# ViacheslavTimofeev/tpu_superresolution

Hardware: AMD Instinct MI355X
Metric: HR pixels/sec, SwinIR x4 train step, 64x64 LR, bs=32/GPU (higher is better)
Workload: dtype bf16; 1 GPU; BASELINE cfg3: SwinIR classical x4 (dim 180, 6x6 blocks, window 8) train step = fwd + L1 + bwd + clip 1.0 + AdamW, 64x64 LR patches -> 256x256 HR, random-init weights, drop_path 0.1; every step starts from the seeded weights and fresh AdamW state; batch_per_gpu=32, global_batch=32, parallelism=dp1

## Files before the change

include/srk.h:

```cpp
#ifndef SRK_H_
#define SRK_H_

#include <stddef.h>
#include <stdint.h>

#ifdef __cplusplus
extern "C" {
#endif

#define SRK_OK 0
#define SRK_E_SHAPE (-1)
#define SRK_E_NULL (-2)
#define SRK_E_UNSUPPORTED (-3)
#define SRK_E_LAUNCH (-4)
#define SRK_E_ALIGN (-5)
#define SRK_E_STATE (-6)

typedef void* srk_stream_t;

const char* srk_version(void);
const char* srk_last_error(void);

int srk_window_partition(const void* x, void* out, int B, int H, int W, int C, int ws, int elem_bytes, srk_stream_t stream);
int srk_window_reverse(const void* windows, void* out, int B, int H, int W, int C, int ws, int elem_bytes, srk_stream_t stream);
int srk_roll2d(const void* x, void* out, int B, int H, int W, int C, int sh, int sw, int elem_bytes, srk_stream_t stream);
int srk_pixel_shuffle(const void* x, void* out, int B, int C, int H, int W, int r, int elem_bytes, srk_stream_t stream);
int srk_shift_mask(float* mask, int H, int W, int ws, int shift, srk_stream_t stream);
int srk_relative_position_index(int64_t* out, int ws, srk_stream_t stream);

typedef struct {
  int H, W;
  int shift;
} srk_win_geom;

int srk_layernorm_fwd(const float* x, const float* gamma, const float* beta, uint16_t* y_bf16, float* y_f32,
                      float* mean, float* rstd, int rows, int C, int CP, const srk_win_geom* geom, srk_stream_t stream);
int srk_window_attention_fwd(const uint16_t* qkv, const float* bias_dense, uint16_t* out, int64_t B_, int nH,
                             const srk_win_geom* geom, srk_stream_t stream);
int srk_window_attention_bwd(const uint16_t* qkv, const float* bias_dense, const uint16_t* d_out, uint16_t* d_qkv,
                             float* d_table, void* slab, int64_t B_, int nH, float scale, const srk_win_geom* geom,
                             srk_stream_t stream);
size_t srk_window_attention_bwd_scratch(int64_t B_, int nH);
int srk_window_attention_bwd_fused(const uint16_t* xn, int lda, const uint16_t* w_qkv, const float* b_qkv, float scale,
                                   const uint16_t* d_x1, int ldg, const uint16_t* w_proj_t, const float* bias_dense, uint16_t* d_qkv,
                                   float* d_table, void* slab, int64_t B_, int nH, const srk_win_geom* geom, srk_stream_t stream);
size_t srk_window_attention_bwd_fused_scratch(int64_t B_, int nH);
int srk_rel_pos_bias_expand(const float* table, float* bias_dense, int nH, srk_stream_t stream);
int srk_linear_bf16(const uint16_t* a, const uint16_t* w, const float* bias, uint16_t* y, int M, int N, int K, srk_stream_t stream);
int srk_linear_wgrad_bf16(const uint16_t* y, const uint16_t* x, float* dw, float* db, int M, int N, int K, srk_stream_t stream);
typedef struct {
  const void* y; int ldy;
  const void* x; int ldx;
  float* dw; float* db;
  int N, K;
} srk_wgrad_problem;
int srk_linear_wgrad_multi_bf16(const srk_wgrad_problem* problems, int count, int M, srk_stream_t stream);
int srk_conv3x3_bf16(const uint16_t* x, const uint16_t* w, const float* bias, uint16_t* y, int B, int H, int W, int CinP, int N,
                     srk_stream_t stream);
int srk_conv3x3_wgrad_bf16(const uint16_t* y, const uint16_t* x, float* dw, float* db, int B, int H, int W, int CinP, int N,
                           srk_stream_t stream);
int srk_cast_f32_bf16(const float* x, uint16_t* y, int64_t n, srk_stream_t stream);
int srk_probe_trread(const uint16_t* in, uint16_t* out, srk_stream_t stream);

int srk_probe_begin(int family, int capacity);
int srk_probe_end(double* total_ms, double* flops, double* bytes, int* launches);

int srk_set_option(const char* name, int value);
int srk_get_option(const char* name, int* value);

int srk_l1_loss_fwd_bwd(const float* pred, const float* target, float* d_pred, float* loss, uint32_t* nonfinite,
                        int64_t n, float grad_scale, srk_stream_t stream);
#define SRK_LOSS_L1 0
#define SRK_LOSS_MSE 1
#define SRK_LOSS_CHARBONNIER 2
int64_t srk_pixel_loss_workspace(int64_t n);
int srk_pixel_loss_fwd_bwd(const float* pred, const float* target, float* d_pred, float* loss, uint32_t* nonfinite, int64_t n, int kind,
                           float eps, float grad_scale, int accumulate, void* workspace, srk_stream_t stream);
int64_t srk_ssim_loss_workspace(int B, int C, int H, int W);
int srk_ssim_loss_fwd_bwd(const float* x, const float* y, void* workspace, int B, int C, int H, int W, float data_range, float alpha,
                          float* d_x, int accumulate, float* ssim_mean, float* loss, srk_stream_t stream);
int64_t srk_wgrad_workspace_bytes(void);
int srk_set_wgrad_workspace(void* workspace, int64_t bytes);

int srk_paired_crop_u8(const uint8_t* pool, const int64_t* lr_desc, const int64_t* hr_desc, float* lr_out, float* hr_out, int B,
                       int lr_patch, int scale, srk_stream_t stream);
int srk_dihedral_f32(const float* in, float* out, const int32_t* ops, int op_all, int B, int C, int H, int W, float alpha,
                     int accumulate, srk_stream_t stream);
int64_t srk_batch_psnr_workspace(int64_t per_image, int B);
int srk_batch_psnr(const float* pred, const float* target, void* workspace, int B, int64_t per_image, float max_val, float* psnr,
                   float* psnr_sum, float* abs_sum, srk_stream_t stream);
int64_t srk_eval_psnr_workspace(int64_t per_image, int B);
int srk_eval_psnr(const float* x, const float* y, void* workspace, int B, int64_t per_image, float max_val, float* psnr, float* mean,
                  srk_stream_t stream);
int64_t srk_ssim_workspace(int B, int C, int H, int W);
int srk_ssim(const float* x, const float* y, void* workspace, int B, int C, int H, int W, float data_range, float* per_image, float* mean,
             srk_stream_t stream);
int srk_grad_sumsq(const float* grads, int64_t n, float* sumsq, srk_stream_t stream);
int srk_adamw_clip_step(float* params, const float* grads, float* exp_avg, float* exp_avg_sq, int64_t n,
                        const float* sumsq, float max_norm, float grad_div, float lr, float beta1, float beta2, float eps,
                        float weight_decay, int step, const int32_t* nonfinite, srk_stream_t stream);
int srk_adamw_clip_ema_step(float* params, const float* grads, float* exp_avg, float* exp_avg_sq, float* ema, int64_t n,
                            const float* sumsq, float max_norm, float grad_div, float lr, float beta1, float beta2, float eps,
                            float weight_decay, int step, float ema_decay, const int32_t* nonfinite, srk_stream_t stream);
int srk_multi_grad_sumsq(const float* const* grads, const int64_t* numel, int n_tensors, float* sumsq, srk_stream_t stream);
int srk_multi_adamw_clip_step(float* const* params, const float* const* grads, float* const* exp_avg, float* const* exp_avg_sq,
                              const int64_t* numel, int n_tensors, const float* sumsq, float max_norm, float grad_div, float lr,
                              float beta1, float beta2, float eps, float weight_decay, int step, const float* hyper,
                              const int32_t* nonfinite, srk_stream_t stream);
int srk_multi_adamw_clip_ema_step(float* const* params, const float* const* grads, float* const* exp_avg, float* const* exp_avg_sq,
                                  float* const* ema, const int64_t* numel, int n_tensors, const float* sumsq, float max_norm,
                                  float grad_div, float lr, float beta1, float beta2, float eps, float weight_decay, int step,
                                  float ema_decay, const float* hyper, const int32_t* nonfinite, srk_stream_t stream);
int srk_adamw_hyper(float lr, float beta1, float beta2, int step, float* out3);

enum { SRK_LD_ROWS = 0, SRK_LD_CONV3 = 1,
       SRK_LD_CONV3_PS = 2  };
enum { SRK_EP_BF16 = 0,
       SRK_EP_GELU = 3,
       SRK_EP_RES = 4,
       SRK_EP_LRELU = 6,
       SRK_EP_PS = 7,
       SRK_EP_IMG = 8,
       SRK_EP_PS_IMG = 9,
       SRK_EP_RES_BF16 = 10,
       SRK_EP_DGELU = 5,
       SRK_EP_DLRELU = 11,
       SRK_EP_F32_BF16 = 12,
       SRK_EP_LNBWD = 13,
       SRK_EP_MLP_FUSED = 100  };
typedef struct {
  int loader, epilogue;
  const void* A; int lda;
  const void* W;
// ... 219 lines not shown
```

tpu_superresolution_amd/_lib.py:

```python
from __future__ import annotations

import ctypes as C
import os
import re
from typing import List

HERE = os.path.dirname(os.path.abspath(__file__))
LIB_PATH = os.environ.get("SRK_LIB_PATH") or os.path.join(HERE, "libsrk.so")
HEADER_PATH = os.path.join(os.path.dirname(HERE), "include", "srk.h")

_lib = None


class SrkError(RuntimeError):
    def __init__(self, code: int, message: str):
        super().__init__(f"libsrk error {code}: {message}")
        self.code = code
        self.message = message


class SrkUnsupported(NotImplementedError):
    pass


class WinGeom(C.Structure):
    _fields_ = [("H", C.c_int), ("W", C.c_int), ("shift", C.c_int)]


class SwinIRConfig(C.Structure):
    _fields_ = [("img_size", C.c_int), ("in_chans", C.c_int), ("embed_dim", C.c_int), ("num_layers", C.c_int),
                ("depths", C.c_int * 16), ("num_heads", C.c_int * 16), ("window_size", C.c_int),
                ("hidden_dim", C.c_int), ("upscale", C.c_int), ("upsampler", C.c_int), ("img_range", C.c_float),
                ("mean", C.c_float * 3), ("qk_scale", C.c_float), ("resi_connection", C.c_int), ("ape", C.c_int), ("use_checkpoint", C.c_int)]


class GemmArgs(C.Structure):
    _fields_ = [("loader", C.c_int), ("epilogue", C.c_int), ("A", C.c_void_p), ("lda", C.c_int), ("W", C.c_void_p),
                ("M", C.c_int), ("N", C.c_int), ("K", C.c_int), ("B", C.c_int), ("H", C.c_int), ("Wd", C.c_int), ("CinP", C.c_int),
                ("r", C.c_int), ("Cs", C.c_int), ("bias", C.c_void_p), ("outf", C.c_void_p), ("outb", C.c_void_p),
                ("outb2", C.c_void_p), ("res", C.c_void_p), ("aux", C.c_void_p), ("ldo", C.c_int), ("scale", C.c_float),
                ("inv_range", C.c_float), ("mean", C.c_float * 4), ("Cimg", C.c_int), ("Hc", C.c_int), ("Wc", C.c_int),
                ("xn_out", C.c_void_p), ("xn_mean", C.c_void_p), ("xn_rstd", C.c_void_p), ("xn_gamma", C.c_void_p),
                ("xn_beta", C.c_void_p), ("xn_C", C.c_int), ("rowscale", C.c_void_p), ("rows_per_sample", C.c_int),
                ("ln_x", C.c_void_p), ("ln_mean", C.c_void_p), ("ln_rstd", C.c_void_p), ("ln_gamma", C.c_void_p), ("ln_dgamma", C.c_void_p),
                ("ln_dbeta", C.c_void_p), ("ln_C", C.c_int)]


class WgradProblem(C.Structure):
    _fields_ = [("y", C.c_void_p), ("ldy", C.c_int), ("x", C.c_void_p), ("ldx", C.c_int), ("dw", C.c_void_p), ("db", C.c_void_p),
                ("N", C.c_int), ("K", C.c_int)]


LD_ROWS, LD_CONV3, LD_CONV3_PS = 0, 1, 2
EP_BF16, EP_GELU, EP_RES, EP_LRELU, EP_PS, EP_IMG, EP_PS_IMG, EP_RES_BF16 = 0, 3, 4, 6, 7, 8, 9, 10
EP_DGELU, EP_DLRELU, EP_F32_BF16, EP_LNBWD = 5, 11, 12, 13

LOSS_L1, LOSS_MSE, LOSS_CHARBONNIER = 0, 1, 2
LOSS_KINDS = {"l1": LOSS_L1, "mse": LOSS_MSE, "charbonnier": LOSS_CHARBONNIER}

UPSAMPLER_PIXELSHUFFLE = 1
UPSAMPLER_PIXELSHUFFLEDIRECT = 2
UPSAMPLER_NEAREST_CONV = 3
UPSAMPLER_NONE = 4
UPSAMPLERS = {"pixelshuffle": UPSAMPLER_PIXELSHUFFLE, "pixelshuffledirect": UPSAMPLER_PIXELSHUFFLEDIRECT,
              "nearest+conv": UPSAMPLER_NEAREST_CONV, "": UPSAMPLER_NONE}
RESI = {"1conv": 0, "3conv": 1}

_vp, _i, _i64, _f, _sz = C.c_void_p, C.c_int, C.c_int64, C.c_float, C.c_size_t
_geom_p = C.POINTER(WinGeom)

_SIGNATURES = {
    "srk_version": (C.c_char_p, []),
    "srk_last_error": (C.c_char_p, []),
    "srk_window_partition": (_i, [_vp, _vp, _i, _i, _i, _i, _i, _i, _vp]),
    "srk_window_reverse": (_i, [_vp, _vp, _i, _i, _i, _i, _i, _i, _vp]),
    "srk_roll2d": (_i, [_vp, _vp, _i, _i, _i, _i, _i, _i, _i, _vp]),
    "srk_pixel_shuffle": (_i, [_vp, _vp, _i, _i, _i, _i, _i, _i, _vp]),
    "srk_shift_mask": (_i, [_vp, _i, _i, _i, _i, _vp]),
    "srk_relative_position_index": (_i, [_vp, _i, _vp]),
    "srk_layernorm_fwd": (_i, [_vp, _vp, _vp, _vp, _vp, _vp, _vp, _i, _i, _i, _geom_p, _vp]),
    "srk_window_attention_fwd": (_i, [_vp, _vp, _vp, _i64, _i, _geom_p, _vp]),
    "srk_window_attention_bwd": (_i, [_vp, _vp, _vp, _vp, _vp, _vp, _i64, _i, _f, _geom_p, _vp]),
    "srk_window_attention_bwd_scratch": (_sz, [_i64, _i]),
    "srk_window_attention_bwd_fused": (_i, [_vp, _i, _vp, _vp, _f, _vp, _i, _vp, _vp, _vp, _vp, _vp, _i64, _i, _geom_p, _vp]),
    "srk_window_attention_bwd_fused_scratch": (_sz, [_i64, _i]),
    "srk_rel_pos_bias_expand": (_i, [_vp, _vp, _i, _vp]),
    "srk_linear_bf16": (_i, [_vp, _vp, _vp, _vp, _i, _i, _i, _vp]),
    "srk_linear_wgrad_bf16": (_i, [_vp, _vp, _vp, _vp, _i, _i, _i, _vp]),
    "srk_conv3x3_bf16": (_i, [_vp, _vp, _vp, _vp, _i, _i, _i, _i, _i, _vp]),
    "srk_conv3x3_wgrad_bf16": (_i, [_vp, _vp, _vp, _vp, _i, _i, _i, _i, _i, _vp]),
    "srk_cast_f32_bf16": (_i, [_vp, _vp, _i64, _vp]),
    "srk_probe_trread": (_i, [_vp, _vp, _vp]),
    "srk_set_option": (_i, [C.c_char_p, _i]),
    "srk_probe_begin": (_i, [_i, _i]),
    "srk_probe_end": (_i, [C.POINTER(C.c_double), C.POINTER(C.c_double), C.POINTER(C.c_double), C.POINTER(_i)]),
    "srk_l1_loss_fwd_bwd": (_i, [_vp, _vp, _vp, _vp, _vp, _i64, _f, _vp]),
    "srk_pixel_loss_workspace": (_i64, [_i64]),
    "srk_pixel_loss_fwd_bwd": (_i, [_vp, _vp, _vp, _vp, _vp, _i64, _i, _f, _f, _i, _vp, _vp]),
    "srk_ssim_loss_workspace": (_i64, [_i, _i, _i, _i]),
    "srk_ssim_loss_fwd_bwd": (_i, [_vp, _vp, _vp, _i, _i, _i, _i, _f, _f, _vp, _i, _vp, _vp, _vp]),
    "srk_wgrad_workspace_bytes": (_i64, []),
    "srk_set_wgrad_workspace": (_i, [_vp, _i64]),
    "srk_paired_crop_u8": (_i, [_vp, _vp, _vp, _vp, _vp, _i, _i, _i, _vp]),
    "srk_dihedral_f32": (_i, [_vp, _vp, _vp, _i, _i, _i, _i, _i, _f, _i, _vp]),
    "srk_batch_psnr_workspace": (_i64, [_i64, _i]),
    "srk_batch_psnr": (_i, [_vp, _vp, _vp, _i, _i64, _f, _vp, _vp, _vp, _vp]),
    "srk_eval_psnr_workspace": (_i64, [_i64, _i]),
    "srk_eval_psnr": (_i, [_vp, _vp, _vp, _i, _i64, _f, _vp, _vp, _vp]),
    "srk_ssim_workspace": (_i64, [_i, _i, _i, _i]),
    "srk_ssim": (_i, [_vp, _vp, _vp, _i, _i, _i, _i, _f, _vp, _vp, _vp]),
    "srk_grad_sumsq": (_i, [_vp, _i64, _vp, _vp]),
    "srk_adamw_clip_step": (_i, [_vp, _vp, _vp, _vp, _i64, _vp, _f, _f, _f, _f, _f, _f, _f, _i, _vp, _vp]),
    "srk_adamw_clip_ema_step": (_i, [_vp, _vp, _vp, _vp, _vp, _i64, _vp, _f, _f, _f, _f, _f, _f, _f, _i, _f, _vp, _vp]),
    "srk_multi_grad_sumsq": (_i, [_vp, _vp, _i, _vp, _vp]),
    "srk_multi_adamw_clip_step": (_i, [_vp, _vp, _vp, _vp, _vp, _i, _vp, _f, _f, _f, _f, _f, _f, _f, _i, _vp, _vp, _vp]),
    "srk_multi_adamw_clip_ema_step": (_i, [_vp, _vp, _vp, _vp, _vp, _vp, _i, _vp, _f, _f, _f, _f, _f, _f, _f, _i, _f, _vp, _vp, _vp]),
    "srk_adamw_hyper": (_i, [_f, _f, _f, _i, C.POINTER(C.c_float * 3)]),
    "srk_gemm_ex": (_i, [C.POINTER(GemmArgs), _vp]),
    "srk_mlp_fused_fwd": (_i, [_vp, _vp, _vp, _vp, _vp, _vp, _vp, _vp, _vp, _vp, _vp, _vp, _vp, _i, _i, _vp]),
    "srk_img_prep": (_i, [_vp, _vp, _i, _i, _i, _i, _i, _i, _f, C.POINTER(C.c_float * 3), _vp]),
    "srk_cab_bwd_workspace": (_sz, [_i, _i, _i]),
    "srk_cab_bwd": (_i, [_vp, _vp, _vp, _vp, _vp, _vp, _vp, _vp, _f, _vp, _vp, _vp, _vp, _vp, _vp, _i, _i, _i, _i, _i, _vp]),
    "srk_win256_attention_bwd_scratch": (_sz, [_i, _i, _i, _i, _i, _i, _i]),
    "srk_win256_attention_bwd": (_i, [_vp, _i, _i, _vp, _i, _vp, _i, _vp, _vp, _vp, _i, _i, _i, _i, _i, _i, _f, _i, _vp]),
    "srk_layernorm_bwd": (_i, [_vp, _vp, _vp, _vp, _vp, _vp, _vp, _vp, _vp, _i, _i, _i, _i, _vp]),
    "srk_add_f32_bf16": (_i, [_vp, _vp, _vp, _i64, _vp]),
    "srk_add_bf16_into_f32": (_i, [_vp, _vp, _i64, _vp]),
    "srk_add_f32": (_i, [_vp, _vp, _vp, _i64, _vp]),
    "srk_img_grad_prep": (_i, [_vp, _vp, _i, _i, _i, _i, _i, _i, _i, _i, _f, _vp]),
    "srk_smallconv_wgrad": (_i, [_vp, _vp, _vp, _vp, _i, _i, _i, _i, _i, _i, _i, _vp]),
    "srk_smallconv_dgrad": (_i, [_vp, _vp, _vp, _i, _i, _i, _i, _i, _i, _i, _vp]),
    "srk_stem_wgrad": (_i, [_vp, _vp, _vp, _vp, _i, _i, _i, _i, _i, _i, _vp]),
    "srk_conv3x3_wgrad_ps_bf16": (_i, [_vp, _vp, _vp, _vp, _i, _i, _i, _i, _i, _i, _i, _vp]),
    "srk_mlp_fused_fwd_train": (_i, [_vp] * 15 + [_i, _vp, _i, _i, _vp]),
    "srk_rowscale_bf16": (_i, [_vp, _vp, _vp, _i64, _i, _i, _vp]),
    "srk_stem_conv": (_i, [_vp, _vp, _vp, _vp, _i, _i, _i, _i, _i, _i, _vp]),
    "srk_swin_block_fwd": (_i, [_vp] * 16 + [_f] + [_i] * 8 + [_vp]),
    "srk_win256_attention_fwd": (_i, [_vp, _i, _i, _vp, _i, _vp, _i, _i, _i, _i, _i, _i, _i, _i, _i, _f, _i, _vp]),
    "srk_win_small_attention_fwd": (_i, [_vp, _i, _i, _vp, _vp, _i, _i, _i, _i, _i, _i, _i, _f, _vp]),
    "srk_win_small_attention_bwd_scratch": (_sz, [_i, _i, _i, _i, _i]),
    "srk_win_small_attention_bwd": (_i, [_vp, _i, _i, _vp, _vp, _i, _vp, _vp, _vp, _i, _i, _i, _i, _i, _i, _f, _vp]),
    "srk_win_attention_fwd_padded": (_i, [_vp, _i, _i, _vp, _i, _vp, _i, _i, _i, _i, _i, _i, _i, _i, _i, _i, _i, _f, _i, _vp]),
    "srk_channel_gate_workspace": (_sz, [_i, _i, _i]),
    "srk_channel_gate": (_i, [_vp, _vp, _vp, _vp, _vp, _vp, _f, _vp, _i, _i, _i, _i, _i, _vp]),
    "srk_channel_gate_act": (_i, [_vp, _vp, _vp, _vp, _vp, _vp, _f, _vp, _i, _i, _i, _i, _i, _i, _vp]),
    "srk_dwconv3x3": (_i, [_vp, _i, _vp, _vp, _vp, _vp, _i, _vp, _i, _i, _i, _i, _i, _i, _vp]),
    "srk_dwconv3x3_bn_act": (_i, [_vp, _i, _vp, _vp, _vp, _vp, _vp, _i, _vp, _i, _i, _i, _i, _i, _vp]),
    "srk_dwconv3x3_bn_act_launches": (C.c_longlong, []),
    "srk_bn_frozen_coeffs": (_i, [_i, _i, _vp, _vp, _f, _vp, _vp, _vp, _vp, _vp]),
    "srk_bn_frozen_bwd_coeffs": (_i, [_vp, _i, _i, _i, _i, _vp, _vp, _vp]),
    "srk_channel_interaction_frozen_covered": (_i, [_i, _i, _i]),
    "srk_channel_interaction_frozen_fwd": (_i, [_vp, _i, _f, _vp, _vp, _vp, _vp, _vp, _f, _vp, _vp, _vp, _vp, _vp, _vp, _i, _i, _i, _i, _vp]),
    "srk_channel_interaction_frozen_bwd": (_i, [_vp, _vp, _i, _f, _vp, _vp, _vp, _vp, _vp, _f, _vp, _vp, _vp, _vp] + [_vp] * 7 + [_i, _i, _i, _i, _vp]),
    "srk_rowln_bf16": (_i, [_vp, _i, _vp, _vp, _vp, _i, _i64, _i, _i, _vp]),
    "srk_spatial_gate": (_i, [_vp, _i, _vp, _vp, _vp, _f, _i, _vp, _i64, _i, _vp]),
    "srk_spatial_gate_dev": (_i, [_vp, _i, _vp, _vp, _vp, _vp, _i, _vp, _i64, _i, _vp]),
    "srk_dual_gate_combine": (_i, [_vp, _vp, _vp, _vp, _vp, _i64, _i, _i, _i, _vp]),
    "srk_channel_attention_workspace": (_sz, [_i, _i, _i]),
    "srk_channel_attention_fwd": (_i, [_vp, _i, _i, _vp, _vp, _vp, _i, _i, _i, _i, _i, _vp]),
    "srk_linear_wgrad_multi_bf16": (_i, [C.POINTER(WgradProblem), _i, _i, _vp]),
    "srk_mlp_fused_bwd": (_i, [_vp, _vp, _vp, _vp, _vp, _vp, _vp, _vp, _vp, _vp, _vp, _vp, _i, _vp, _vp, _i, _i, _vp]),
    "srk_win_attention_bwd_padded_scratch": (_sz, [_i, _i, _i, _i, _i, _i]),
    "srk_win_attention_bwd_padded": (_i, [_vp, _i, _i, _vp, _vp, _i, _vp, _vp, _vp, _i, _i, _i, _i, _i, _i, _i, _i, _i, _i, _f, _vp]),
    "srk_bn_train_coeffs": (_i, [_vp, _i, _i, _i, _i, _f, _vp, _vp, _f, _vp, _vp, _vp, _f, _vp, _vp]),
    "srk_channel_interaction_covered": (_i, [_i, _i, _i]),
    "srk_channel_interaction_fwd": (_i, [_vp, _i, _f, _vp, _vp, _vp, _vp, _vp, _f, _vp, _vp, _vp, _vp, _f, _vp, _vp, _i, _i, _i, _i, _vp]),
    "srk_channel_interaction_bwd": (_i, [_vp, _vp, _i, _f, _vp, _vp, _vp, _vp, _vp, _f, _vp, _vp, _vp, _vp, _vp, _vp, _vp, _vp, _vp, _i, _i, _i, _i, _vp]),
    "srk_chan_attn_matrix_fwd": (_i, [_vp, _i, _vp, _vp, _vp, _i, _i, _i, _vp]),
# ... 85 lines not shown
```

tpu_superresolution_amd/csrc/api.hip:

```cpp
#include <stdarg.h>
#include <stdio.h>
#include <string.h>

#include "adamw.h"
#include "kernels.h"
#include "wgrad.h"

static thread_local char g_err[512] = "";

SrkOptTls& srk_opt_tls() {
  static thread_local SrkOptTls t = {};
  return t;
}

static SrkOpt** opt_table() {
  static SrkOpt* table[SRK_NUM_OPTS] = {};
  return table;
}

void srk_opt_register(SrkOpt* o) {
  if (o->id >= 0 && o->id < SRK_NUM_OPTS) opt_table()[o->id] = o;
}

void srk_opt_scope_begin(SrkOptTls* saved) {
// ... 118 lines not shown
  SRK_REQUIRE(B > 0 && C > 0 && H > 0 && W > 0 && r > 0, SRK_E_SHAPE, "pixel_shuffle: bad shape");
  return srk_launch_pixel_shuffle(x, out, B, C, H, W, r, elem_bytes, (hipStream_t)stream);
}

int srk_shift_mask(float* mask, int H, int W, int ws, int shift, srk_stream_t stream) {
  REQ_PTR(mask);
  SRK_REQUIRE(ws > 0 && H % ws == 0 && W % ws == 0 && shift >= 0 && shift < ws, SRK_E_SHAPE,
              "shift_mask: shift_size must in 0-window_size (H=%d W=%d ws=%d shift=%d)", H, W, ws, shift);
  return srk_launch_shift_mask(mask, H, W, ws, shift, (hipStream_t)stream);
}

int srk_relative_position_index(int64_t* out, int ws, srk_stream_t stream) {
  REQ_PTR(out);
  SRK_REQUIRE(ws > 0 && ws <= 64, SRK_E_SHAPE, "relative_position_index: bad ws %d", ws);
  return srk_launch_rel_pos_index((long long*)out, ws, (hipStream_t)stream);
}

int srk_layernorm_fwd(const float* x, const float* gamma, const float* beta, uint16_t* y_bf16, float* y_f32, float* mean,
                      float* rstd, int rows, int C, int CP, const srk_win_geom* geom, srk_stream_t stream) {
  REQ_PTR(x); REQ_PTR(gamma); REQ_PTR(beta); REQ_ALIGN(x);
  SRK_REQUIRE(rows > 0, SRK_E_SHAPE, "layernorm: rows=%d", rows);
  SRK_REQUIRE((mean == nullptr) == (rstd == nullptr), SRK_E_NULL, "layernorm: mean/rstd must both be given or both null");
  WinGeom g;
  if (geom) {
    int rc = make_geom(geom, &g, "layernorm");
    if (rc) return rc;
    SRK_REQUIRE(rows % (g.H * g.W) == 0, SRK_E_SHAPE, "layernorm: rows %d not a multiple of H*W", rows);
  }
  return srk_launch_ln_fwd(x, gamma, beta, y_bf16, y_f32, mean, rstd, rows, C, CP, geom ? &g : nullptr, (hipStream_t)stream);
}

int srk_window_attention_fwd(const uint16_t* qkv, const float* bias_dense, uint16_t* out, int64_t B_, int nH,
                             const srk_win_geom* geom, srk_stream_t stream) {
  REQ_PTR(qkv); REQ_PTR(bias_dense); REQ_PTR(out); REQ_PTR(geom); REQ_ALIGN(qkv); REQ_ALIGN(out); REQ_ALIGN(bias_dense);
  WinGeom g;
  int rc = make_geom(geom, &g, "window_attention_fwd");
  if (rc) return rc;
  SRK_REQUIRE(B_ > 0 && B_ % g.nW == 0 && nH > 0 && nH <= 64, SRK_E_SHAPE, "window_attention_fwd: B_=%lld nW=%d nH=%d",
              (long long)B_, g.nW, nH);
  return srk_launch_attn_fwd(qkv, bias_dense, out, B_, nH, g, (hipStream_t)stream);
}

size_t srk_window_attention_bwd_scratch(int64_t B_, int nH) {
  return (size_t)srk_attn_bwd_slabs(B_, nH, nullptr) * nH * 4096 * sizeof(float);
}

int srk_window_attention_bwd(const uint16_t* qkv, const float* bias_dense, const uint16_t* d_out, uint16_t* d_qkv,
                             float* d_table, void* slab, int64_t B_, int nH, float scale, const srk_win_geom* geom,
                             srk_stream_t stream) {
  REQ_PTR(qkv); REQ_PTR(bias_dense); REQ_PTR(d_out); REQ_PTR(d_qkv); REQ_PTR(d_table); REQ_PTR(slab); REQ_PTR(geom);
  REQ_ALIGN(qkv); REQ_ALIGN(d_out); REQ_ALIGN(d_qkv); REQ_ALIGN(slab);
  WinGeom g;
  int rc = make_geom(geom, &g, "window_attention_bwd");
  if (rc) return rc;
  SRK_REQUIRE(B_ > 0 && B_ % g.nW == 0 && nH > 0 && nH <= 64, SRK_E_SHAPE, "window_attention_bwd: B_=%lld nW=%d nH=%d",
              (long long)B_, g.nW, nH);
  return srk_launch_attn_bwd(qkv, bias_dense, d_out, d_qkv, (float*)slab, d_table, B_, nH, g, scale, (hipStream_t)stream);
}

size_t srk_window_attention_bwd_fused_scratch(int64_t B_, int nH) {
  return (size_t)srk_qkv_attn_bwd_slabs(B_, nH, nH * 32, 192) * nH * 4096 * sizeof(float);
}

int srk_window_attention_bwd_fused(const uint16_t* xn, int lda, const uint16_t* w_qkv, const float* b_qkv, float scale,
                                   const uint16_t* d_x1, int ldg, const uint16_t* w_proj_t, const float* bias_dense, uint16_t* d_qkv,
                                   float* d_table, void* slab, int64_t B_, int nH, const srk_win_geom* geom, srk_stream_t stream) {
  REQ_PTR(xn); REQ_PTR(w_qkv); REQ_PTR(d_x1); REQ_PTR(w_proj_t); REQ_PTR(bias_dense); REQ_PTR(d_qkv); REQ_PTR(d_table); REQ_PTR(slab);
  REQ_PTR(geom); REQ_ALIGN(xn); REQ_ALIGN(w_qkv); REQ_ALIGN(d_x1); REQ_ALIGN(w_proj_t); REQ_ALIGN(d_qkv); REQ_ALIGN(slab);
  WinGeom g;
  int rc = make_geom(geom, &g, "window_attention_bwd_fused");
  if (rc) return rc;
  SRK_REQUIRE(B_ > 0 && B_ % g.nW == 0, SRK_E_SHAPE, "window_attention_bwd_fused: B_=%lld nW=%d", (long long)B_, g.nW);
  const int nslab = srk_qkv_attn_bwd_slabs(B_, nH, nH * 32, 192);
  SRK_REQUIRE(nslab > 0, SRK_E_UNSUPPORTED,
              "window_attention_bwd_fused: covers 6 heads x 32, K = 192 and at least one window per CU (got nH=%d B_=%lld)", nH,
              (long long)B_);
  rc = srk_launch_qkv_attn_bwd(xn, lda, w_qkv, b_qkv, scale, d_x1, ldg, w_proj_t, bias_dense, d_qkv, (float*)slab, B_, nH, nH * 32, 192, g,
                               (hipStream_t)stream);
  SRK_REQUIRE(rc != SRK_NOT_COVERED, SRK_E_UNSUPPORTED, "window_attention_bwd_fused: the kernel cannot run on this build / shape");
  if (rc) return rc;
  return srk_launch_rpb_reduce((const float*)slab, d_table, nslab, nH, (hipStream_t)stream);
}

int srk_rel_pos_bias_expand(const float* table, float* bias_dense, int nH, srk_stream_t stream) {
  REQ_PTR(table); REQ_PTR(bias_dense);
  return srk_launch_rpb_expand(table, bias_dense, nH, (hipStream_t)stream);
}

int srk_linear_bf16(const uint16_t* a, const uint16_t* w, const float* bias, uint16_t* y, int M, int N, int K, srk_stream_t stream) {
  REQ_PTR(a); REQ_PTR(w); REQ_PTR(y); REQ_ALIGN(a); REQ_ALIGN(w); REQ_ALIGN(y);
  GemmParams p = {};
  p.A = a; p.lda = K; p.Wt = w; p.M = M; p.N = N; p.K = K; p.bias = bias; p.outb = y; p.ldo = N;
  return srk_launch_gemm(LD_ROWS, EP_BF16, p, (hipStream_t)stream);
}

int srk_linear_wgrad_bf16(const uint16_t* y, const uint16_t* x, float* dw, float* db, int M, int N, int K, srk_stream_t stream) {
  REQ_PTR(y); REQ_PTR(x); REQ_PTR(dw); REQ_ALIGN(y); REQ_ALIGN(x);
  WgradParams p = {};
  p.Y = y; p.ldy = N; p.X = x; p.ldx = K; p.M = M; p.N = N; p.K = K; p.dW = dw; p.ldw = K; p.db = db;
  return srk_launch_wgrad(p, (hipStream_t)stream);
}

int srk_linear_wgrad_multi_bf16(const srk_wgrad_problem* problems, int count, int M, srk_stream_t stream) {
  REQ_PTR(problems);
  SRK_REQUIRE(count >= 1 && count <= 4 && M > 0, SRK_E_SHAPE, "linear_wgrad_multi: count=%d (1..4), M=%d", count, M);
  WgradParams ps[4] = {};
  for (int i = 0; i < count; ++i) {
    const srk_wgrad_problem& q = problems[i];
    REQ_PTR(q.y); REQ_PTR(q.x); REQ_PTR(q.dw); REQ_ALIGN(q.y); REQ_ALIGN(q.x);
    SRK_REQUIRE(q.N > 0 && q.K > 0 && q.N % 64 == 0 && q.K % 64 == 0, SRK_E_SHAPE, "linear_wgrad_multi: problem %d: N=%d K=%d (multiples of 64)", i,
                q.N, q.K);
    SRK_REQUIRE((q.ldy <= 0 || q.ldy >= q.N) && (q.ldx <= 0 || q.ldx >= q.K), SRK_E_SHAPE, "linear_wgrad_multi: problem %d: ldy=%d < N or ldx=%d < K",
                i, q.ldy, q.ldx);
    SRK_REQUIRE((q.ldy <= 0 || q.ldy % 8 == 0) && (q.ldx <= 0 || q.ldx % 8 == 0), SRK_E_ALIGN,
                "linear_wgrad_multi: problem %d: ldy=%d / ldx=%d must be multiples of 8 elements", i, q.ldy, q.ldx);
    ps[i].Y = static_cast<const bf16_t*>(q.y); ps[i].ldy = q.ldy > 0 ? q.ldy : q.N;
    ps[i].X = static_cast<const bf16_t*>(q.x); ps[i].ldx = q.ldx > 0 ? q.ldx : q.K;
    ps[i].M = M; ps[i].N = q.N; ps[i].K = q.K; ps[i].dW = q.dw; ps[i].ldw = q.K; ps[i].db = q.db;
  }
  return srk_launch_wgrad_multi(ps, count, (hipStream_t)stream);
}

int srk_conv3x3_bf16(const uint16_t* x, const uint16_t* w, const float* bias, uint16_t* y, int B, int H, int W, int CinP, int N,
                     srk_stream_t stream) {
  REQ_PTR(x); REQ_PTR(w); REQ_PTR(y); REQ_ALIGN(x); REQ_ALIGN(w); REQ_ALIGN(y);
  GemmParams p = {};
  p.A = x; p.Wt = w; p.M = B * H * W; p.N = N; p.K = 9 * CinP; p.B = B; p.H = H; p.W = W; p.CinP = CinP;
  p.bias = bias; p.outb = y; p.ldo = N;
  return srk_launch_gemm(LD_CONV3, EP_BF16, p, (hipStream_t)stream);
}

int srk_conv3x3_wgrad_bf16(const uint16_t* y, const uint16_t* x, float* dw, float* db, int B, int H, int W, int CinP, int N,
                           srk_stream_t stream) {
  REQ_PTR(y); REQ_PTR(x); REQ_PTR(dw); REQ_ALIGN(y); REQ_ALIGN(x);
  SRK_REQUIRE(B > 0 && H > 0 && W > 0 && (long long)B * H * W < (1ll << 31), SRK_E_SHAPE, "conv3x3_wgrad: B=%d H=%d W=%d", B, H, W);
  WgradParams p = {};
  p.Y = y; p.ldy = N; p.X = x; p.ldx = CinP; p.M = B * H * W; p.N = N; p.K = CinP; p.dW = dw; p.ldw = 9 * CinP; p.db = db;
  p.conv = 1; p.B = B; p.H = H; p.W = W; p.r = 1;
  return srk_launch_wgrad(p, (hipStream_t)stream);
}

int srk_cast_f32_bf16(const float* x, uint16_t* y, int64_t n, srk_stream_t stream) {
  REQ_PTR(x); REQ_PTR(y);
  return srk_launch_cast_f32_bf16(x, y, n, (hipStream_t)stream);
}

int srk_probe_begin(int family, int capacity) {
  SRK_REQUIRE(!g_probe.active, SRK_E_STATE, "probe_begin: a probe is already active");
  SRK_REQUIRE(family >= 1 && family <= 7 && capacity > 0 && capacity <= (1 << 20), SRK_E_SHAPE, "probe_begin: bad arguments");
  while ((int)g_probe.ev0.size() < capacity) {
    hipEvent_t a, b;
    if (hipEventCreate(&a) != hipSuccess || hipEventCreate(&b) != hipSuccess) {
      srk_set_error("probe_begin: hipEventCreate failed");
      return SRK_E_LAUNCH;
    }
    g_probe.ev0.push_back(a);
    g_probe.ev1.push_back(b);
  }
  g_probe.family = family;
  g_probe.count = 0;
  g_probe.seen = 0;
  g_probe.flops = 0.0;
  g_probe.bytes = 0.0;
  g_probe.active = true;
  return SRK_OK;
}

int srk_probe_end(double* total_ms, double* flops, double* bytes, int* launches) {
  SRK_REQUIRE(g_probe.active, SRK_E_STATE, "probe_end: no active probe");
  g_probe.active = false;
  double ms = 0.0;
  for (size_t i = 0; i < g_probe.count; ++i) {
    float t = 0.f;
    if (hipEventSynchronize(g_probe.ev1[i]) != hipSuccess || hipEventElapsedTime(&t, g_probe.ev0[i], g_probe.ev1[i]) != hipSuccess) {
      srk_set_error("probe_end: event query failed");
      return SRK_E_LAUNCH;
    }
    ms += t;
  }
  if (total_ms) *total_ms = ms;
  if (flops) *flops = g_probe.flops;
  if (bytes) *bytes = g_probe.bytes;
  if (launches) *launches = (int)g_probe.count;
  return SRK_OK;
}

namespace {

int tune_get(int which) {
  int v[4];
  srk_gemm_stream_tune_get(&v[0], &v[1], &v[2], &v[3]);
  return v[which];
}
int tune_set(int which, int value) {
  int v[4];
  srk_gemm_stream_tune_get(&v[0], &v[1], &v[2], &v[3]);
  v[which] = value;
  srk_gemm_stream_tune(v[0], v[1], v[2], v[3]);
  return SRK_OK;
}
int wtune_get(int which) {
  int rows, nt;
  srk_wgrad_stream_tune_get(&rows, &nt);
  return which == 0 ? rows : nt;
}

struct OptEntry {
  const char* name;
  int (*get)();
  int (*set)(int);
};

const OptEntry kOptions[] = {
    {"gemm_stream", [] { return srk_gemm_stream_enabled(); }, [](int v) { srk_gemm_stream_enable(v); return (int)SRK_OK; }},
    {"attn_bwd_fused", [] { return srk_attn_bwd_fused_enabled(); }, [](int v) { srk_attn_bwd_fused_enable(v); return (int)SRK_OK; }},
    {"attn_fused", [] { return srk_attn_fused_mode(); }, [](int v) { srk_attn_fused_enable(v); return (int)SRK_OK; }},
    {"wgrad_stream_w8", [] { return srk_wgrad_w8_enabled(); }, [](int v) { srk_wgrad_w8_enable(v); return (int)SRK_OK; }},
    {"block_light", [] { return srk_block_light_enabled(); }, [](int v) { srk_block_light_enable(v); return (int)SRK_OK; }},
    {"mlp_bwd_fused", [] { return srk_mlp_bwd_fused_enabled(); }, [](int v) { srk_mlp_bwd_fused_enable(v); return (int)SRK_OK; }},
    {"mlp_dgelu_store", [] { return srk_mlp_dgelu_store_enabled(); }, [](int v) { srk_mlp_dgelu_store_enable(v); return (int)SRK_OK; }},
    {"mlp_fused", [] { return srk_mlp_fused_enabled(); }, [](int v) { srk_mlp_fused_enable(v); return (int)SRK_OK; }},
    {"wgrad_stream", [] { return srk_wgrad_stream_enabled(); }, [](int v) { srk_wgrad_stream_enable(v); return (int)SRK_OK; }},
    {"conv_wgrad_taps", [] { return srk_conv_wgrad_taps_mode(); }, [](int v) { srk_conv_wgrad_taps_enable(v); return (int)SRK_OK; }},
    {"conv_wgrad_roll", [] { return srk_conv_wgrad_roll_enabled(); }, [](int v) { srk_conv_wgrad_roll_enable(v); return (int)SRK_OK; }},
    {"wgrad_partials", [] { return srk_wgrad_partials_enabled(); }, [](int v) { srk_wgrad_partials_enable(v); return (int)SRK_OK; }},
    {"wgrad_stream_rows", [] { return wtune_get(0); },
     [](int v) {
       SRK_REQUIRE(v == 32 || v == 64, SRK_E_SHAPE, "wgrad_stream_rows: 32/64");
       srk_wgrad_stream_tune(v, -1);
       return (int)SRK_OK;
     }},
    {"wgrad_stream_nt", [] { return wtune_get(1); }, [](int v) { srk_wgrad_stream_tune(0, v != 0); return (int)SRK_OK; }},
    {"gemm_stream_bm", [] { return tune_get(0); },
     [](int v) {
       SRK_REQUIRE(v == 0 || v == 16 || v == 32 || v == 64, SRK_E_SHAPE, "gemm_stream_bm: 0/16/32/64");
       return tune_set(0, v);
     }},
    {"gemm_stream_ks2", [] { return tune_get(1); }, [](int v) { return tune_set(1, v < 0 ? -1 : (v != 0)); }},
    {"gemm_stream_split", [] { return tune_get(2); }, [](int v) { return tune_set(2, v < 0 ? -1 : (v != 0)); }},
    {"gemm_stream_nb", [] { return tune_get(3); },
     [](int v) {
       SRK_REQUIRE(v == 0 || v == 4 || v == 8, SRK_E_SHAPE, "gemm_stream_nb: 0/4/8");
       return tune_set(3, v);
     }},
    {"probe_stride", [] { return g_probe.stride; },
     [](int v) {
       SRK_REQUIRE(v >= 1 && v <= 1024, SRK_E_SHAPE, "probe_stride: 1..1024");
       g_probe.stride = v;
       return (int)SRK_OK;
     }},
};

const OptEntry* find_option(const char* name) {
  for (const OptEntry& e : kOptions)
    if (strcmp(name, e.name) == 0) return &e;
  return nullptr;
}

}

int srk_set_option(const char* name, int value) {
  REQ_PTR(name);
  const OptEntry* e = find_option(name);
  if (!e) {
    srk_set_error("srk_set_option: unknown option '%s'", name);
    return SRK_E_UNSUPPORTED;
  }
  return e->set(value);
}

int srk_get_option(const char* name, int* value) {
  REQ_PTR(name); REQ_PTR(value);
  const OptEntry* e = find_option(name);
  if (!e) {
    srk_set_error("srk_get_option: unknown option '%s'", name);
    return SRK_E_UNSUPPORTED;
  }
  *value = e->get();
  return SRK_OK;
}

int srk_probe_trread(const uint16_t* in, uint16_t* out, srk_stream_t stream) {
  REQ_PTR(in); REQ_PTR(out);
  return srk_launch_probe_trread(in, out, (hipStream_t)stream);
}

int srk_l1_loss_fwd_bwd(const float* pred, const float* target, float* d_pred, float* loss, uint32_t* nonfinite, int64_t n,
                        float grad_scale, srk_stream_t stream) {
  REQ_PTR(pred); REQ_PTR(target); REQ_PTR(loss); REQ_PTR(nonfinite);
  SRK_REQUIRE(n > 0, SRK_E_SHAPE, "l1_loss: n=%lld", (long long)n);
  return srk_launch_l1_loss(pred, target, d_pred, loss, nonfinite, n, grad_scale, (hipStream_t)stream);
}

int64_t srk_wgrad_workspace_bytes(void) { return (int64_t)WS_WORKSPACE_BYTES; }

int srk_set_wgrad_workspace(void* workspace, int64_t bytes) {
  SRK_REQUIRE(bytes >= 0 && (workspace != nullptr || bytes == 0), SRK_E_SHAPE, "set_wgrad_workspace: null pointer with %lld bytes",
              (long long)bytes);
// ... 131 lines not shown
```

tpu_superresolution_amd/csrc/attn_bwd_fused.hip:

```cpp
#include "kernels.h"

namespace {

constexpr int H_K = 192, H_CA = 192, H_NH = 6;
constexpr int H_SLOT = 64 * H_K * 2;
constexpr int H_TILE = 64 * 32;
constexpr int H_PT = 64 * 64;
constexpr int H_TAB = 225;
constexpr int H_PAIR = 2 * H_SLOT;
constexpr int OFF_S = 0;
constexpr int OFF_T = 2 * H_PAIR;
constexpr int OFF_TAB = OFF_T + 12 * H_TILE * 2;
constexpr int OFF_PB = OFF_TAB + 2704;
constexpr int H_LDS = OFF_PB + 10 * 32 * 4;
static_assert(6 * H_PT * 2 == H_PAIR, "P / dS tiles of a head triple fill a row slot exactly");

#ifndef SRK_ABF_ISSUE_AT
#define SRK_ABF_ISSUE_AT 1
#endif
#ifdef SRK_PROBE_ABF
__device__ unsigned long long g_abf_probe[12 * 16 * 8];
#define ABF_MARK(k) do { if (blockIdx.x == 0 && lane == 0 && t < 16) g_abf_probe[(wave * 16 + t) * 8 + (k)] = __builtin_amdgcn_s_memrealtime(); } while (0)
extern "C" int srk_debug_abf_probe(void* host) { return (int)hipMemcpyFromSymbol(host, HIP_SYMBOL(g_abf_probe), sizeof(g_abf_probe)); }
#else
#define ABF_MARK(k) do {} while (0)
#endif

struct BwdFusedParams {
  const bf16_t* xn;
  int lda;
  const bf16_t* g;
  int ldg;
  const bf16_t* Wqkv;
  const float* bqkv;
  float scale;
  const bf16_t* WprojT;
  const float* biasd;
  bf16_t* dqkv;
  float* slab;
  long long B_;
  WinGeom geom;
};

__device__ __forceinline__ int tf(int r) { return ((((r >> 2) ^ (r >> 3)) & 1) << 1) | (((r >> 3) ^ (r >> 1)) & 1); }
__device__ __forceinline__ int ps(int r) { return (((r >> 3) & 1) << 2) | (((r >> 1) & 1) << 1) | ((r >> 2) & 1); }

__device__ __forceinline__ bf16x8_t h_cat4(bf16x4_t lo, bf16x4_t hi) {
  return bf16x8_t{lo[0], lo[1], lo[2], lo[3], hi[0], hi[1], hi[2], hi[3]};
}

__device__ __forceinline__ bf16x8_t tile_tr(const bf16_t* tile, int rb0, int rb1, int dt, int r16) {
  const int q = r16 >> 2, c = 2 * dt + ((r16 & 3) >> 1), in = (r16 & 1) << 2;
  const int ra = rb0 + q, rb = rb1 + q;
  return h_cat4(lds_tr_read(tile + ra * 32 + ((c ^ tf(ra)) << 3) + in), lds_tr_read(tile + rb * 32 + ((c ^ tf(rb)) << 3) + in));
}
__device__ __forceinline__ bf16x8_t ptile_tr(const bf16_t* tile, int rb0, int rb1, int jt, int r16) {
  const int q = r16 >> 2, c = 2 * jt + ((r16 & 3) >> 1), in = (r16 & 1) << 2;
  const int ra = rb0 + q, rb = rb1 + q;
  return h_cat4(lds_tr_read(tile + ra * 64 + ((c ^ ps(ra)) << 3) + in), lds_tr_read(tile + rb * 64 + ((c ^ ps(rb)) << 3) + in));
}

__global__ __launch_bounds__(768) void qkv_attn_bwd_kernel(const BwdFusedParams p, int ngrp) {
  extern __shared__ __attribute__((aligned(16))) unsigned char smem[];
  const unsigned smem_base = (unsigned)(size_t)smem;
  const int tid = threadIdx.x, lane = tid & 63;
  const int wave = __builtin_amdgcn_readfirstlane(tid >> 6);
  const int r16 = lane & 15, g = lane >> 4;
  const int id = blockIdx.x, xcd = id & 7, slot = id >> 3;
  const int tr = slot & 1, grp = slot >> 1;
  const int gidx = grp * 8 + xcd;
  const long long first = gidx, stride = 8LL * ngrp;
  const long long nwin = first < p.B_ ? (p.B_ - first + stride - 1) / stride : 0;
  const int hl = wave >> 2, it = wave & 3;
  const int head = 3 * tr + hl;

  f32x4_t dbias[4];
#pragma unroll
  for (int jt = 0; jt < 4; ++jt) dbias[jt] = f32x4_t{0.f, 0.f, 0.f, 0.f};

  if (nwin > 0) {
    bf16_t* tiles = reinterpret_cast<bf16_t*>(smem + OFF_T);
    float* tab = reinterpret_cast<float*>(smem + OFF_TAB);
    for (int i = tid; i < 3 * H_TAB; i += 768) {
      const int hh = i / H_TAB, t = i - hh * H_TAB;
      const int dy = t / 15 - 7, dx = t - (t / 15) * 15 - 7;
      const int qi = (dy > 0 ? dy : 0) * 8 + (dx > 0 ? dx : 0), kj = (dy < 0 ? -dy : 0) * 8 + (dx < 0 ? -dx : 0);
      tab[i] = p.biasd[(3 * tr + hh) * 4096 + qi * 64 + kj];
    }

    bf16x8_t wf[2][6];
    {
      const bf16_t* wbase = it < 3 ? p.Wqkv + (long long)(it * H_CA + head * 32) * H_K : p.WprojT + (long long)(head * 32) * H_K;
#pragma unroll
      for (int j = 0; j < 2; ++j)
#pragma unroll
        for (int s = 0; s < 6; ++s) wf[j][s] = *reinterpret_cast<const bf16x8_t*>(wbase + (16 * j + r16) * H_K + s * 32 + g * 8);
    }
    float* pbs = reinterpret_cast<float*>(smem + OFF_PB);
    for (int i = tid; i < 9 * 32; i += 768) {
      const int tl = i >> 5, hh = tl / 3, which = tl - 3 * hh;
      pbs[i] = p.bqkv ? p.bqkv[which * H_CA + (3 * tr + hh) * 32 + (i & 31)] : 0.f;
    }
    for (int i = tid; i < 32; i += 768) pbs[9 * 32 + i] = 0.f;
    const float* pbw = pbs + (it < 3 ? hl * 3 + it : 9) * 32 + 4 * g;
    const float sc = it == 0 ? p.scale : 1.0f;

    const bool dma_g = wave >= 6;
    const bf16_t* dsrc = dma_g ? p.g : p.xn;
    const long long dld = dma_g ? p.ldg : p.lda;
    const int piece0 = dma_g ? 4 * (wave - 6) : 4 * wave;
    const unsigned ddst = smem_base + OFF_S + (dma_g ? H_SLOT : 0) + piece0 * 1024;
    auto issue = [&](long long b_, int slot) {
      const bf16_t* base = dsrc + b_ * 64 * dld;
#pragma unroll
      for (int i = 0; i < 4; ++i) {
        int q = (piece0 + i) * 64 + lane;
        asm volatile("" : "+v"(q));
        const int row = (q * 2731) >> 16, pos = q - row * 24;
        srk_glds16<false>(base + row * (int)dld + ((pos ^ (row & 7)) << 3), __builtin_amdgcn_readfirstlane(ddst + slot * H_PAIR + i * 1024));
      }
    };
#pragma unroll
    for (int j = 0; j < 2; ++j) {
#pragma unroll
      for (int s = 0; s < 6; ++s) asm volatile("" ::"v"(wf[j][s]));
    }
    issue(first, 0);

    const int tfr = tf(r16), psr = ps(r16);
    bf16_t* mytile = tiles + (hl * 4 + it) * H_TILE;
    const bf16_t* Qs = tiles + (hl * 4 + 0) * H_TILE;
    const bf16_t* Ks = tiles + (hl * 4 + 1) * H_TILE;
    const bf16_t* Vs = tiles + (hl * 4 + 2) * H_TILE;
    const bf16_t* Os = tiles + (hl * 4 + 3) * H_TILE;
    const float* th = tab + hl * H_TAB + ((2 * it + (r16 >> 3)) - (g >> 1) + 7) * 15 + ((r16 & 7) - 4 * (g & 1) + 7) - 93;
    const int ldq = 3 * H_CA;
    const int scol = ((g & 1) << 4) | ((g >> 1) << 3);
    auto store8 = [&](bf16_t* dst, uint2 x, uint2 y) {
      const auto s0 = __builtin_amdgcn_permlane16_swap(x.x, y.x, false, false);
      const auto s1 = __builtin_amdgcn_permlane16_swap(x.y, y.y, false, false);
      *reinterpret_cast<uint4*>(dst) = make_uint4(s0[0], s1[0], s0[1], s1[1]);
    };

    for (long long t = 0; t < nwin; ++t) {
      const long long b_ = first + t * stride;
      if (t == 0) srk_wait_vmcnt<0>();
// ... 92 lines not shown
#pragma unroll
          for (int e = 0; e < 4; ++e) s[jt][e] = __builtin_amdgcn_exp2f(tt[e]);
          a4 += s[jt];
        }
        const float inv = __builtin_amdgcn_rcpf(xrow_sum4((a4[0] + a4[1]) + (a4[2] + a4[3])));
        float dl = 0.f;
#pragma unroll
        for (int jt = 0; jt < 4; ++jt)
#pragma unroll
          for (int e = 0; e < 4; ++e) {
            s[jt][e] *= inv;
            dl += s[jt][e] * dp[jt][e];
          }
        dl = xrow_sum4(dl);
        uint2 dsp[4];
#pragma unroll
        for (int jt = 0; jt < 4; ++jt) {
#pragma unroll
          for (int e = 0; e < 4; ++e) {
            dp[jt][e] = s[jt][e] * (dp[jt][e] - dl);
            dbias[jt][e] += dp[jt][e];
          }
          dsp[jt] = pack_bf4(dp[jt][0], dp[jt][1], dp[jt][2], dp[jt][3]);
          const int po = (16 * it + r16) * 64 + (((2 * jt + (g >> 1)) ^ psr) << 3) + 4 * (g & 1);
          *reinterpret_cast<uint2*>(Pb + po) = pack_bf4(s[jt][0], s[jt][1], s[jt][2], s[jt][3]);
          *reinterpret_cast<uint2*>(Db + po) = dsp[jt];
        }
        f32x4_t aq[2] = {f32x4_t{0.f, 0.f, 0.f, 0.f}, f32x4_t{0.f, 0.f, 0.f, 0.f}};
#pragma unroll
        for (int ss = 0; ss < 2; ++ss) {
          const bf16x8_t dsf = __builtin_bit_cast(bf16x8_t, make_uint4(dsp[2 * ss].x, dsp[2 * ss].y, dsp[2 * ss + 1].x, dsp[2 * ss + 1].y));
#pragma unroll
          for (int dt = 0; dt < 2; ++dt)
            aq[dt] = __builtin_amdgcn_mfma_f32_16x16x32_bf16(tile_tr(Ks, 32 * ss + 4 * g, 32 * ss + 16 + 4 * g, dt, r16), dsf, aq[dt], 0, 0, 0);
        }
        bf16_t* row = p.dqkv + (b_ * 64 + 16 * it + r16) * ldq + head * 32 + scol;
        store8(row, pack_bf4(aq[0][0] * p.scale, aq[0][1] * p.scale, aq[0][2] * p.scale, aq[0][3] * p.scale),
               pack_bf4(aq[1][0] * p.scale, aq[1][1] * p.scale, aq[1][2] * p.scale, aq[1][3] * p.scale));
      }
      ABF_MARK(4);
      srk_lds_barrier();
      ABF_MARK(5);
      if (SRK_ABF_ISSUE_AT == 2 && t + 1 < nwin) issue(b_ + stride, cur ^ 1);

      {
        f32x4_t av[2], ak[2];
#pragma unroll
        for (int dt = 0; dt < 2; ++dt) av[dt] = ak[dt] = f32x4_t{0.f, 0.f, 0.f, 0.f};
        bf16x8_t pf[2], df[2], otf[2][2], qtf[2][2];
#pragma unroll
        for (int ss = 0; ss < 2; ++ss) {
          const int rb0 = 32 * ss + 8 * g, rb1 = rb0 + 4;
          pf[ss] = ptile_tr(Pb, rb0, rb1, it, r16);
          df[ss] = ptile_tr(Db, rb0, rb1, it, r16);
#pragma unroll
          for (int dt = 0; dt < 2; ++dt) {
            otf[ss][dt] = tile_tr(Os, rb0, rb1, dt, r16);
            qtf[ss][dt] = tile_tr(Qs, rb0, rb1, dt, r16);
          }
        }
        __builtin_amdgcn_sched_barrier(0);
#pragma unroll
        for (int ss = 0; ss < 2; ++ss)
#pragma unroll
          for (int dt = 0; dt < 2; ++dt) {
            av[dt] = __builtin_amdgcn_mfma_f32_16x16x32_bf16(otf[ss][dt], pf[ss], av[dt], 0, 0, 0);
            ak[dt] = __builtin_amdgcn_mfma_f32_16x16x32_bf16(qtf[ss][dt], df[ss], ak[dt], 0, 0, 0);
          }
        bf16_t* row = p.dqkv + (b_ * 64 + 16 * it + r16) * ldq + head * 32 + scol;
        store8(row + H_CA, pack_bf4(ak[0][0], ak[0][1], ak[0][2], ak[0][3]), pack_bf4(ak[1][0], ak[1][1], ak[1][2], ak[1][3]));
        store8(row + 2 * H_CA, pack_bf4(av[0][0], av[0][1], av[0][2], av[0][3]), pack_bf4(av[1][0], av[1][1], av[1][2], av[1][3]));
      }
      ABF_MARK(6);
    }
  }
  int lane2;
  asm volatile("v_mbcnt_lo_u32_b32 %0, -1, 0\n\tv_mbcnt_hi_u32_b32 %0, -1, %0" : "=v"(lane2));
  float* slab = p.slab + (((long long)gidx * H_NH + head) * 64 + 16 * it + (lane2 & 15)) * 64 + 4 * (lane2 >> 4);
#pragma unroll
  for (int jt = 0; jt < 4; ++jt)
    *reinterpret_cast<float4*>(slab + 16 * jt) = make_float4(dbias[jt][0], dbias[jt][1], dbias[jt][2], dbias[jt][3]);
}

SrkOpt g_attn_bwd_fused{OPT_ATTN_BWD_FUSED, 1};

}

void srk_attn_bwd_fused_enable(int on) { g_attn_bwd_fused = on ? 1 : 0; }
int srk_attn_bwd_fused_enabled() { return g_attn_bwd_fused; }

static int abf_cus() { return srk_device_cus(); }

int srk_qkv_attn_bwd_slabs(long long B_, int nH, int CA, int K) {
  if (!g_attn_bwd_fused || nH != H_NH || CA != H_CA || K != H_K) return 0;
  const int cus = abf_cus();
  if (cus < 16 || B_ < cus) return 0;
  return 8 * (cus / 16);
}

int srk_launch_qkv_attn_bwd(const bf16_t* xn, int lda, const bf16_t* Wqkv, const float* bqkv, float scale, const bf16_t* g, int ldg,
                            const bf16_t* WprojT, const float* biasd, bf16_t* dqkv, float* slab, long long B_, int nH, int CA, int K,
                            WinGeom geom, hipStream_t stream) {
  const int nslab = srk_qkv_attn_bwd_slabs(B_, nH, CA, K);
  if (nslab == 0 || lda % 8 != 0 || ldg % 8 != 0 || B_ * 64 * (long long)(lda > ldg ? lda : ldg) >= (1LL << 31)) return SRK_NOT_COVERED;
  static SrkPerDevice<int> configured_pd; int& configured = configured_pd.here();
  if (!configured) {
    const void* fn = reinterpret_cast<const void*>(&qkv_attn_bwd_kernel);
    hipFuncAttributes attr;
    configured = -1;
#ifdef SRK_PROBE_ABF
    attr.localSizeBytes = 0;
    if (hipFuncSetAttribute(fn, hipFuncAttributeMaxDynamicSharedMemorySize, H_LDS) == hipSuccess) configured = 1;
#endif
    if (configured < 0 && hipFuncGetAttributes(&attr, fn) == hipSuccess && attr.localSizeBytes == 0 &&
        hipFuncSetAttribute(fn, hipFuncAttributeMaxDynamicSharedMemorySize, H_LDS) == hipSuccess)
      configured = 1;
  }
  if (configured < 0) return SRK_NOT_COVERED;
  BwdFusedParams bp;
  bp.xn = xn; bp.lda = lda; bp.g = g; bp.ldg = ldg; bp.Wqkv = Wqkv; bp.bqkv = bqkv; bp.scale = scale; bp.WprojT = WprojT;
  bp.biasd = biasd; bp.dqkv = dqkv; bp.slab = slab; bp.B_ = B_; bp.geom = geom;
  const int ngrp = nslab / 8;
  srk_probe_pre(FAM_ATTN_BWD, stream, 0.0);
  hipLaunchKernelGGL(qkv_attn_bwd_kernel, dim3(16 * ngrp), dim3(768), H_LDS, stream, bp, ngrp);
  srk_probe_post(FAM_ATTN_BWD, stream);
  return srk_check_launch("qkv+attention backward");
}
```

tpu_superresolution_amd/csrc/common.h:

```cpp
#pragma once
#include <hip/hip_runtime.h>
#include <stdint.h>

#include "../../include/srk.h"

typedef unsigned short bf16_t;
typedef __attribute__((ext_vector_type(8))) short bf16x8_t;
typedef __attribute__((ext_vector_type(4))) short bf16x4_t;
typedef __attribute__((ext_vector_type(4))) float f32x4_t;

#define SRK_WAVE 64

void srk_set_error(const char* fmt, ...);
int srk_check_launch(const char* what);

constexpr int SRK_MAX_DEVICES = 64;
int srk_current_device();
int srk_device_cus();
enum SrkOptId {
  OPT_MLP_FUSED, OPT_MLP_BWD_FUSED, OPT_GEMM_STREAM, OPT_TUNE_BM, OPT_TUNE_KS2, OPT_TUNE_SPLIT, OPT_TUNE_NB, OPT_ATTN_BWD_FUSED,
  OPT_ATTN_FUSED, OPT_BLOCK_LIGHT, OPT_TAPS_ENABLED, OPT_TAPS_DMA, OPT_WGRAD_STREAM, OPT_WGRAD_ROWS, OPT_WGRAD_NT, OPT_WGRAD_W8,
  OPT_WGRAD_PARTIALS, OPT_MLP_DGELU_STORE, OPT_TAPS_ROLL, SRK_NUM_OPTS
};
struct SrkOptTls {
  int v[SRK_NUM_OPTS];
  unsigned on;
};
SrkOptTls& srk_opt_tls();
struct SrkOpt;
void srk_opt_register(SrkOpt* o);
void srk_opt_scope_begin(SrkOptTls* saved);
void srk_opt_scope_end(const SrkOptTls& saved);
struct SrkOpt {
  int id;
  int value;
  SrkOpt(int id_, int v) : id(id_), value(v) { srk_opt_register(this); }
  operator int() const {
    const SrkOptTls& t = srk_opt_tls();
    return ((t.on >> id) & 1u) ? t.v[id] : value;
  }
  SrkOpt& operator=(int v) {
    SrkOptTls& t = srk_opt_tls();
    if ((t.on >> id) & 1u) t.v[id] = v;
    else value = v;
    return *this;
  }
  SrkOpt(const SrkOpt&) = delete;
  SrkOpt& operator=(const SrkOpt&) = delete;
};

template <class T>
struct SrkPerDevice {
  T v[SRK_MAX_DEVICES] = {};
  T& here() { return v[srk_current_device()]; }
};

enum { FAM_GEMM_LINEAR = 1, FAM_GEMM_CONV = 2, FAM_WGRAD_LINEAR = 3, FAM_WGRAD_CONV = 4, FAM_ATTN_FWD = 5, FAM_ATTN_BWD = 6,
       FAM_LN = 7 };
void srk_probe_pre(int family, hipStream_t stream, double flops, double bytes = 0.0);
void srk_probe_post(int family, hipStream_t stream);

#define SRK_REQUIRE(cond, code, ...)      \
  do {                                    \
    if (!(cond)) {                        \
      srk_set_error(__VA_ARGS__);         \
      return (code);                      \
    }                                     \
  } while (0)

__device__ __forceinline__ float bf2f(bf16_t v) { return __uint_as_float(((unsigned)v) << 16); }

__device__ __forceinline__ bf16_t f2bf(float f) {
  __bf16 b = (__bf16)f;
  return __builtin_bit_cast(unsigned short, b);
}

typedef __bf16 srk_bf16x2_t __attribute__((ext_vector_type(2)));
typedef float srk_f32x2_t __attribute__((ext_vector_type(2)));
__device__ __forceinline__ unsigned pack_bf2(float lo, float hi) {
  return __builtin_bit_cast(unsigned, __builtin_convertvector(srk_f32x2_t{lo, hi}, srk_bf16x2_t));
}

__device__ __forceinline__ uint2 pack_bf4(float a, float b, float c, float d) {
  return make_uint2(pack_bf2(a, b), pack_bf2(c, d));
}

__device__ __forceinline__ void unpack_bf2(unsigned u, float& lo, float& hi) {
  lo = __uint_as_float(u << 16);
  hi = __uint_as_float(u & 0xffff0000u);
}

__device__ __forceinline__ float erf_fast(float x) {
  const float ax = fabsf(x);
  const float t = __builtin_amdgcn_rcpf(fmaf(0.3275911f, ax, 1.0f));
  float p = fmaf(1.061405429f, t, -1.453152027f);
  p = fmaf(p, t, 1.421413741f);
  p = fmaf(p, t, -0.284496736f);
  p = fmaf(p, t, 0.254829592f);
  const float r = 1.0f - p * t * __expf(-ax * ax);
  return copysignf(r, x);
}
__device__ __forceinline__ float gelu_f(float x) { return 0.5f * x * (1.0f + erf_fast(x * 0.70710678118654752f)); }

__device__ __forceinline__ float dgelu_shared_exp(float x) {
  const float z = x * 0.70710678118654752f;
// ... 164 lines not shown
```

tpu_superresolution_amd/csrc/kernels.h:

```cpp
#pragma once
#include "common.h"
#include "gemm.h"
#include "pack.h"
#include "wgrad.h"

int srk_launch_qkv_attn_fwd(const bf16_t* xn, int lda, const bf16_t* Wt, const float* bias, float scale, bf16_t* qkv, const float* biasd,
                            bf16_t* ao, long long B_, int nH, int CA, int K, WinGeom geom, hipStream_t stream);
void srk_attn_fused_enable(int on);
int srk_attn_fused_mode();
void srk_block_light_enable(int on);
int srk_block_light_enabled();
int srk_launch_swin_block_light(const float* x, float* y, bf16_t* yb, const float* n1w, const float* n1b, const float* n2w, const float* n2b,
                                const bf16_t* Wqkv, const bf16_t* Wproj, const bf16_t* W1, const bf16_t* W2, const float* bqkv,
                                const float* bproj, const float* b1, const float* b2, const float* biasd, float scale, int C, int CP, int HP,
                                int nH, int dh, int HID, long long B_, WinGeom geom, hipStream_t stream);
int srk_launch_attn_fwd(const bf16_t* qkv, const float* biasd, bf16_t* ao, long long B_, int nH, WinGeom geom, hipStream_t stream);
int srk_attn_bwd_slabs(long long B_, int nH, int* wpw_out);
int srk_launch_attn_bwd(const bf16_t* qkv, const float* biasd, const bf16_t* dao, bf16_t* dqkv, float* dbias_slab,
                        float* dtable, long long B_, int nH, WinGeom geom, float scale, hipStream_t stream);
int srk_launch_rpb_expand(const float* table, float* biasd, int nH, hipStream_t stream);
void srk_attn_bwd_fused_enable(int on);
int srk_attn_bwd_fused_enabled();
int srk_qkv_attn_bwd_slabs(long long B_, int nH, int CA, int K);
int srk_launch_qkv_attn_bwd(const bf16_t* xn, int lda, const bf16_t* Wqkv, const float* bqkv, float scale, const bf16_t* g, int ldg,
                            const bf16_t* WprojT, const float* biasd, bf16_t* dqkv, float* slab, long long B_, int nH, int CA, int K,
                            WinGeom geom, hipStream_t stream);

int srk_launch_ln_fwd(const float* x, const float* gamma, const float* beta, bf16_t* yb, float* yf, float* mean,
                      float* rstd, int rows, int C, int CP, const WinGeom* geom, hipStream_t stream);
int srk_launch_ln_bwd(const bf16_t* dyb, const float* x, const float* mean, const float* rstd, const float* gamma,
                      float* gx, bf16_t* gxb, float* dgamma, float* dbeta, int rows, int C, int CP, const WinGeom* geom,
                      int dy_by_m, int stats_by_m, int out_by_m, int accumulate, const float* rowscale, int rows_per_sample,
                      hipStream_t stream);

int srk_launch_window_partition(const void* x, void* out, int B, int H, int W, int C, int ws, int elem_bytes, int reverse, hipStream_t stream);
int srk_launch_roll2d(const void* x, void* out, int B, int H, int W, int C, int sh, int sw, int elem_bytes, hipStream_t stream);
int srk_launch_pixel_shuffle(const void* x, void* out, int B, int C, int H, int W, int r, int elem_bytes, hipStream_t stream);
int srk_launch_shift_mask(float* mask, int H, int W, int ws, int shift, hipStream_t stream);
int srk_launch_rel_pos_index(long long* out, int ws, hipStream_t stream);
int srk_launch_img_prep(const float* x, float* out, int B, int Cimg, int H0, int W0, int H, int W, float range, const float* mean, hipStream_t stream);
int srk_launch_stem_conv(const float* in, const float* wgt, const float* bias, float* out, int B, int H, int W, int Cin, int C, int CP, hipStream_t stream);
int srk_launch_stem_wgrad(const float* in, const float* gy, float* dW, float* db, int B, int H, int W, int Cin, int C, int CP, hipStream_t stream);
int srk_launch_img_grad_prep(const float* dpred, float* gy, int B, int Cimg, int Hc, int Wc, int H, int W, int r, int CoP, float inv_range, hipStream_t stream);
int srk_launch_smallconv_dgrad(const float* gy, const float* wgt, bf16_t* dx, int B, int H, int W, int Cin, int CinP, int Co, int CoP, hipStream_t stream);
int srk_launch_smallconv_wgrad(const bf16_t* x, const float* gy, float* dW, float* db, int B, int H, int W, int Cin, int CinP, int Co, int CoP, hipStream_t stream);
inline int srk_batch_psnr_chunks(long long per_image) {
  const long long c = (per_image + 8191) / 8192;
  return (int)(c < 1 ? 1 : (c > 64 ? 64 : c));
}
int srk_launch_crop_u8(const unsigned char* pool, const long long* desc, float* out, int B, int patch, hipStream_t stream);
int srk_launch_dihedral_f32(const float* in, float* out, const int* ops, int op_all, int B, int C, int H, int W, float alpha,
                            int accumulate, hipStream_t stream);
int srk_launch_batch_psnr(const float* pred, const float* target, float* partial, int B, long long per_image, float max_val,
                          float* psnr, float* psnr_sum, float* abs_sum, hipStream_t stream);
int srk_launch_zero_f32(float* p, long long n, hipStream_t stream);
int srk_launch_add_f32_bf16(float* a, const float* b, bf16_t* ab, long long n, hipStream_t stream);
int srk_launch_add_bf16_into_f32(float* a, const bf16_t* b, long long n, hipStream_t stream);
int srk_launch_cast_f32_bf16(const float* a, bf16_t* out, long long n, hipStream_t stream);
int srk_launch_ape_add(float* x, const float* ape, int B, int L, int C, int CP, hipStream_t stream);
int srk_launch_ape_grad(const float* gx, float* dape, int B, int L, int C, int CP, hipStream_t stream);
int srk_launch_dlrelu_bf16(bf16_t* g, const bf16_t* act, float slope, long long n, hipStream_t stream);
int srk_launch_nn2x_bf16(const bf16_t* in, bf16_t* out, int B, int h, int w, int C, hipStream_t stream);
int srk_launch_nn2x_sum_dlrelu(const bf16_t* g, const bf16_t* act, bf16_t* out, int B, int h, int w, int C, float slope, hipStream_t stream);
int srk_launch_nchw_tokens(const float* src, float* dst, int B, int C, int CP, int HW, int to_tokens, hipStream_t stream);
int srk_launch_l1_loss(const float* pred, const float* target, float* dpred, float* loss_sum, unsigned* nonfinite, long long n, float grad_scale, hipStream_t stream);
inline int srk_pixel_loss_blocks(long long n) {
  const long long b = (n + 255) / 256;
  return (int)(b < 1 ? 1 : (b > 2048 ? 2048 : b));
}
int srk_launch_pixel_loss(const float* pred, const float* target, float* dpred, float* loss, unsigned* nonfinite, long long n, int kind,
                          float eps, float grad_scale, int accumulate, float* partial, hipStream_t stream);
int srk_launch_ssim_loss(const float* x, const float* y, float* partial, int B, int C, int H, int W, float data_range, float alpha, float* d_x,
                         int accumulate, float* ssim_mean, float* loss, hipStream_t stream);
int srk_launch_sumsq(const float* g, long long n, float* out, hipStream_t stream);
int srk_launch_adamw(float* p, const float* g, float* m, float* v, long long n, const float* sumsq, const int* nonfinite, float max_norm, float grad_div, float lr, float beta1, float beta2, float eps, float wd, int step, hipStream_t stream);
int srk_launch_adamw_ema(float* p, const float* g, float* m, float* v, float* ema, long long n, const float* sumsq, const int* nonfinite, float max_norm, float grad_div, float lr, float beta1, float beta2, float eps, float wd, int step, float ema_decay, hipStream_t stream);
int srk_launch_multi_sumsq(const float* const* grads, const long long* numel, int n_tensors, float* out, hipStream_t stream);
int srk_launch_multi_adamw(float* const* p, const float* const* g, float* const* m, float* const* v, const long long* numel, int n_tensors, const float* sumsq, const int* nonfinite, const float* hyper, float max_norm, float grad_div, float lr, float beta1, float beta2, float eps, float wd, int step, hipStream_t stream);
int srk_launch_multi_adamw_ema(float* const* p, const float* const* g, float* const* m, float* const* v, float* const* e, const long long* numel, int n_tensors, const float* sumsq, const int* nonfinite, const float* hyper, float max_norm, float grad_div, float lr, float beta1, float beta2, float eps, float wd, int step, float ema_decay, hipStream_t stream);
int srk_launch_probe_trread(const bf16_t* in, bf16_t* out, hipStream_t stream);
int srk_launch_win256_attn_fwd(const bf16_t* qkv, int ldq, int CA, const float* bias, int table_rows, bf16_t* out, int ldo, int B, int H, int W, int wh, int ww, int sy, int sx, int nH, float scale, int overlap, hipStream_t stream);
int srk_launch_win_attn_fwd_padded(const bf16_t* qkv, int ldq, int CA, const float* bias, int table_rows, bf16_t* out, int ldo, int B, int H, int W, int Hp, int Wp, int wh, int ww, int sy, int sx, int nH, float scale, int overlap, hipStream_t stream);
int srk_launch_chan_gram(const bf16_t* x, int ldx, const bf16_t* y, int ldy, float* partial, int B, int N, int nH, hipStream_t stream);
```

tpu_superresolution_amd/csrc/swinir.hip:

```cpp
#include <string.h>

#include <map>
#include <string>
#include <vector>

#include "kernels.h"
#include "wgrad.h"

namespace {

struct ParamEntry {
  std::string name;
  long long off, numel;
  int ndim;
  long long shape[4];
};

struct BlockW {
  long long n1w, n1b, rpb, qkvw, qkvb, projw, projb, n2w, n2b, fc1w, fc1b, fc2w, fc2b;
  long long Wqkv, WqkvT, Wproj, WprojT, Wfc1, Wfc1T, Wfc2, Wfc2T;
  long long bqkv, bproj, bfc1, bfc2, biasd;
  int nH, dh, CA, shift;
  float scale;
};

struct ConvW {
  long long w, b;
  long long Wc, WcT;
  long long bc;
  int Cin, CinP, Cout, NP, r, Cs;
};

struct ResiW {
  int three = 0;
  ConvW c;
  ConvW c0, c2;
  long long w1 = 0, b1 = 0, W1 = 0, W1T = 0, b1s = 0;
  int C4 = 0;
};

struct ResiAct {
  size_t a1 = 0, a2 = 0;
};

struct BlockAct {
  size_t x_in, xn1w, mean1, rstd1, qkv, ao, x1, xn2, mean2, rstd2, u, h, x_out;
};

struct Workspace {
  int B = 0, H0 = 0, W0 = 0, H = 0, W = 0, training = 0;
  int attn_recompute = 0;
  int ckpt = 0;
  int u_is_dgelu = 0;
  size_t ck_x = 0;
  int opt_sig = 0;
  long long T = 0;
  size_t img4, f0, x0, mean_pe, rstd_pe;
  std::vector<BlockAct> blk;
  std::vector<size_t> layer_in, layer_xb, layer_out;
  size_t meanf, rstdf, xnf, fb, t1;
  std::vector<size_t> up;
  std::vector<ResiAct> resi;
  std::vector<size_t> nc_u, nc_a;
  size_t nc_hr = 0;
  size_t gx, gxb, gx2, gxb2, gxbw, du, dxn, dao, dqkv, slab, wgpart, gyimg, gt1, gfb, gfb32, gstage_w, gstage_side;
  size_t g3a = 0, g3b = 0;
  size_t ncgA = 0, ncgB = 0, ncgU = 0;
  std::vector<size_t> gup;
  size_t total = 0;
  std::map<std::string, std::pair<size_t, size_t>> names;
};

}

struct srk_swinir_plan {
  srk_swinir_config cfg;
  int C, CP, HID, HP, L, nblk, Cimg;
  int nstage, stage_r;
  bool no_shift;
  std::vector<ParamEntry> params;
  long long param_floats = 0;
  std::vector<std::pair<std::string, int>> options;
  std::vector<BlockW> blocks;
  std::vector<int> layer_first_blk;
  std::vector<ResiW> layer_conv;
  ResiW conv_after_body;
  ConvW conv_before_up, conv_last, up_direct, conv_hr;
  std::vector<ConvW> up_convs;
  long long p_conv_first_w, p_conv_first_b, p_pe_w, p_pe_b, p_norm_w, p_norm_b;
  long long p_ape = -1;
  std::vector<PackDesc> descs;
  std::vector<int> group_desc_begin, group_blocks;
  std::vector<long long> group_param_begin;
  long long packed_elems = 0, side_floats = 0;
  const PackDesc* d_descs = nullptr;
  Workspace ws;
};

namespace {

long long add_param(srk_swinir_plan* p, const std::string& name, std::initializer_list<long long> shape) {
  ParamEntry e;
  e.name = name;
  e.ndim = (int)shape.size();
  e.numel = 1;
  int i = 0;
  for (long long s : shape) {
    e.shape[i++] = s;
    e.numel *= s;
  }
  for (; i < 4; ++i) e.shape[i] = 1;
  e.off = p->param_floats;
  p->param_floats += (e.numel + 63) / 64 * 64;
  p->params.push_back(e);
  return e.off;
}

long long alloc_packed(srk_swinir_plan* p, long long elems) {
  const long long off = p->packed_elems;
  p->packed_elems += (elems + 127) / 128 * 128;
  return off;
}
long long alloc_side(srk_swinir_plan* p, long long floats) {
  const long long off = p->side_floats;
  p->side_floats += (floats + 63) / 64 * 64;
  return off;
}

PackDesc base_desc(int kind, long long src, long long dst, int NP, int KP) {
  PackDesc d;
  memset(&d, 0, sizeof(d));
  d.kind = kind;
  d.src = src;
  d.dst = dst;
  d.NP = NP;
  d.KP = KP;
  d.r = 1;
  d.Cs = 64;
  d.CinP = 64;
  return d;
}

void push_desc(srk_swinir_plan* p, const PackDesc& d) { p->descs.push_back(d); }

void add_linear(srk_swinir_plan* p, long long src, long long dst, long long dstT, int NP, int KP, int Nreal, int Kreal, int nmap,
                int kmap, int nH, int dh) {
  PackDesc d = base_desc(PK_LINEAR, src, dst, NP, KP);
  d.Nreal = Nreal; d.Kreal = Kreal; d.nmap = nmap; d.kmap = kmap; d.nH = nH; d.dh = dh; d.CA = nH * 32;
// ... 151 lines not shown
    const int first = p->layer_first_blk[l], depth = p->cfg.depths[l];
    for (int j = 0; j < depth; ++j) {
      const int bi = first + j;
      BlockAct& ba = w.blk[bi];
      const std::string pre = "blk" + std::to_string(bi) + ".";
      const BlockW& bw = p->blocks[bi];
      ba.x_in = cur;
      if (training) {
        ba.xn1w = a.get(pre + "xn1w", T * CP * 2);
        ba.mean1 = a.get(pre + "mean1", T * 4);
        ba.rstd1 = a.get(pre + "rstd1", T * 4);
        ba.qkv = w.attn_recompute ? 0 : a.get(pre + "qkv", T * 3 * bw.CA * 2);
        ba.ao = w.ckpt ? ck_ao : a.get(pre + "ao", T * bw.CA * 2);
        ba.x1 = a.get(pre + "x1", T * CP * 4);
        ba.xn2 = a.get(pre + "xn2", T * CP * 2);
        ba.mean2 = a.get(pre + "mean2", T * 4);
        ba.rstd2 = a.get(pre + "rstd2", T * 4);
        ba.u = w.ckpt ? ck_u : a.get(pre + "u", T * HP * 2);
        ba.h = w.ckpt ? ck_h : a.get(pre + "h", T * HP * 2);
        ba.x_out = a.get(pre + "x_out", T * CP * 4);
      } else {
        const size_t xin = ba.x_in;
        ba = shared;
        ba.x_in = xin;
        ba.x1 = pingP;
        ba.x_out = pingQ;
      }
      cur = ba.x_out;
    }
    if (p->cfg.resi_connection == SRK_RESI_3CONV) {
      const std::string pre = training ? "layer" + std::to_string(l) + "." : "shared.";
      w.resi[l].a1 = (training || l == 0) ? a.get(pre + "resi_a1", T * 64 * 2) : w.resi[0].a1;
      w.resi[l].a2 = (training || l == 0) ? a.get(pre + "resi_a2", T * 64 * 2) : w.resi[0].a2;
    }
    w.layer_xb[l] = training ? a.get("layer" + std::to_string(l) + ".xb", T * CP * 2) : shared_xb;
    w.layer_out[l] = training ? a.get("layer" + std::to_string(l) + ".out", T * CP * 4) : w.layer_in[l];
    cur = w.layer_out[l];
  }
  w.meanf = a.get("meanf", T * 4);
  w.rstdf = a.get("rstdf", T * 4);
  w.xnf = a.get("xnf", T * CP * 2);
  w.fb = a.get("fb", T * CP * 2);
  if (p->cfg.resi_connection == SRK_RESI_3CONV) {
    w.resi[p->L].a1 = (training || p->L == 0) ? a.get("tail.resi_a1", T * 64 * 2) : w.resi[0].a1;
    w.resi[p->L].a2 = (training || p->L == 0) ? a.get("tail.resi_a2", T * 64 * 2) : w.resi[0].a2;
  }
  w.t1 = 0;
  size_t out_px = T;
  if (p->cfg.upsampler == SRK_UPSAMPLER_PIXELSHUFFLE) {
    w.t1 = a.get("t1", T * 64 * 2);
    size_t px = T;
    for (int k = 0; k < p->nstage; ++k) {
      px *= (size_t)p->stage_r * p->stage_r;
      w.up.push_back(a.get("up" + std::to_string(k), px * 64 * 2));
    }
    out_px = px;
  } else if (p->cfg.upsampler == SRK_UPSAMPLER_NEAREST_CONV) {
    w.t1 = a.get("t1", T * 64 * 2);
    size_t px = T;
    for (int k = 0; k < p->nstage; ++k) {
      px *= 4;
      w.nc_u.push_back(a.get("nc_u" + std::to_string(k), px * 64 * 2));
      w.nc_a.push_back(a.get("nc_a" + std::to_string(k), px * 64 * 2));
    }
    w.nc_hr = a.get("nc_hr", px * 64 * 2);
    out_px = px;
  }
  if (training) {
    w.gx = a.get("gx", T * CP * 4);
    w.gxb = a.get("gxb", T * CP * 2);
    w.gx2 = a.get("gx2", T * CP * 4);
    w.gxb2 = a.get("gxb2", T * CP * 2);
    w.gxbw = a.get("gxbw", T * CP * 2);
    w.du = a.get("du", T * HP * 2);
    w.dxn = a.get("dxn", T * CP * 2);
    w.dao = a.get("dao", T * maxCA * 2);
    w.dqkv = a.get("dqkv", T * 3 * maxCA * 2);
    int maxH = 1;
    for (const BlockW& b : p->blocks) maxH = b.nH > maxH ? b.nH : maxH;
    size_t nslab = (size_t)srk_attn_bwd_slabs(w.T / 64, 1, nullptr);
    if (w.attn_recompute) nslab = (size_t)srk_qkv_attn_bwd_slabs(w.T / 64, p->blocks[0].nH, p->blocks[0].CA, p->CP);
    w.slab = a.get("slab", nslab * maxH * 4096 * 4);
    w.wgpart = a.get("wgpart", WS_WORKSPACE_BYTES);
    w.gfb = a.get("gfb", T * CP * 2);
    w.gfb32 = a.get("gfb32", T * CP * 4);
    if (p->cfg.resi_connection == SRK_RESI_3CONV) {
      w.g3a = a.get("g3a", T * 64 * 2);
      w.g3b = a.get("g3b", T * 64 * 2);
    }
    if (p->cfg.upsampler == SRK_UPSAMPLER_NEAREST_CONV) {
      w.gt1 = a.get("gt1", T * 64 * 2);
      w.ncgA = a.get("ncgA", out_px * 64 * 2);
      w.ncgB = a.get("ncgB", out_px * 64 * 2);
      w.ncgU = a.get("ncgU", out_px * 64 * 2);
      w.gyimg = a.get("gyimg", out_px * 4 * 4);
    } else if (p->cfg.upsampler == SRK_UPSAMPLER_PIXELSHUFFLE) {
      w.gt1 = a.get("gt1", T * 64 * 2);
      size_t px = T;
      for (int k = 0; k < p->nstage; ++k) {
        px *= (size_t)p->stage_r * p->stage_r;
        w.gup.push_back(a.get("gup" + std::to_string(k), px * 64 * 2));
      }
      w.gyimg = a.get("gyimg", px * 4 * 4);
    } else {
      w.gyimg = a.get("gyimg", T * 16 * 4);
    }
    w.gstage_w = a.get("gstage_w", (size_t)p->packed_elems * 4);
    w.gstage_side = a.get("gstage_side", (size_t)p->side_floats * 4);
  }
  w.total = a.off;
}

struct Ctx {
  srk_swinir_plan* p;
  const float* params;
  const bf16_t* packed;
  const float* side;
  unsigned char* ws;
  hipStream_t stream;
  template <typename T>
  T* at(size_t off) const { return reinterpret_cast<T*>(ws + off); }
};

inline const float* side_of(const srk_swinir_plan* p, const void* packed) {
  return reinterpret_cast<const float*>(reinterpret_cast<const unsigned char*>(packed) + (size_t)p->packed_elems * 2);
}

WinGeom make_wgeom(int H, int W, int shift) {
  WinGeom g;
  g.H = H; g.W = W; g.nWw = W / 8; g.nW = (H / 8) * (W / 8); g.shift = shift;
  return g;
}

#define RUN(expr)          \
  do {                     \
    int rc__ = (expr);     \
    if (rc__) return rc__; \
  } while (0)

int run_conv(const Ctx& c, const ConvW& cw, int loader, int ep, const bf16_t* in, int B, int H, int W, GemmParams extra) {
  GemmParams g = extra;
  g.A = in;
  g.Wt = c.packed + cw.Wc;
  g.M = B * H * W;
  g.N = cw.NP;
  g.K = 9 * cw.CinP;
  g.B = B; g.H = H; g.W = W; g.CinP = cw.CinP;
  g.bias = c.side + cw.bc;
  g.flops = 2.0 * g.M * cw.Cout * cw.Cin * 9;
  if (g.ldo == 0) g.ldo = cw.NP;
  return srk_launch_gemm(loader, ep, g, c.stream);
}

}

extern "C" {

int srk_swinir_plan_create(const srk_swinir_config* cfg, srk_swinir_plan** out) {
  SRK_REQUIRE(cfg && out, SRK_E_NULL, "plan_create: null argument");
  SRK_REQUIRE(cfg->window_size == 8, SRK_E_UNSUPPORTED, "HIP path supports window_size == 8 only (got %d)", cfg->window_size);
  SRK_REQUIRE(cfg->img_size >= 8, SRK_E_UNSUPPORTED, "HIP path needs img_size >= window_size (got %d)", cfg->img_size);
  SRK_REQUIRE(cfg->in_chans == 1 || cfg->in_chans == 3, SRK_E_UNSUPPORTED, "in_chans must be 1 or 3 (got %d)", cfg->in_chans);
  SRK_REQUIRE(cfg->embed_dim > 0 && cfg->embed_dim <= 256, SRK_E_UNSUPPORTED, "embed_dim must be <= 256 (got %d)", cfg->embed_dim);
  SRK_REQUIRE(cfg->num_layers > 0 && cfg->num_layers <= 16, SRK_E_UNSUPPORTED, "num_layers must be 1..16");
  SRK_REQUIRE(cfg->hidden_dim > 0 && cfg->hidden_dim <= 1024, SRK_E_UNSUPPORTED, "hidden_dim must be <= 1024");
  SRK_REQUIRE(cfg->upsampler >= SRK_UPSAMPLER_PIXELSHUFFLE && cfg->upsampler <= SRK_UPSAMPLER_NONE, SRK_E_UNSUPPORTED,
// ... 711 lines not shown
      RUN(unpack_group(c, p->L + 1, grads));
    } else if (seg <= p->L) {
      const int l = p->L - seg;
      const int first = p->layer_first_blk[l], depth = p->cfg.depths[l];
      {
        const int last = first + depth - 1;
        GemmParams g = {};
        g.outf = c.at<float>(w.gx2); g.outb = c.at<bf16_t>(w.gxb2);
        g.rowscale = drop_scale ? drop_scale + ((size_t)last * 2 + 1) * B : nullptr; g.rows_per_sample = HW;
        RUN(resi_backward(c, p->layer_conv[l], w.resi[l], c.at<bf16_t>(w.gxb), c.at<bf16_t>(w.layer_xb[l]), EP_F32_BF16, g, B, H, W));
      }
      bool skip_folded = false;
      for (int j = depth - 1; j >= 0; --j) {
        const int bi = first + j;
        const BlockW& bw = p->blocks[bi];
        const BlockAct& ba = w.blk[bi];
        const WinGeom geom = make_wgeom(H, W, bw.shift);
        const float* ds_attn = drop_scale ? drop_scale + ((size_t)bi * 2 + 0) * B : nullptr;
        const float* ds_prev_mlp = (drop_scale && j > 0) ? drop_scale + ((size_t)(bi - 1) * 2 + 1) * B : nullptr;
        if (w.ckpt) {
          GemmParams g1 = {};
          g1.A = c.at<bf16_t>(ba.xn2); g1.lda = CP; g1.Wt = c.packed + bw.Wfc1; g1.M = T; g1.N = HP; g1.K = CP;
          g1.bias = c.side + bw.bfc1; g1.outb = c.at<bf16_t>(ba.u); g1.outb2 = c.at<bf16_t>(ba.h); g1.ldo = HP; g1.flops = fl_mlp;
          g1.bytes = (double)T * (2.0 * C + 4.0 * p->HID) + 2.0 * C * p->HID;
          RUN(srk_launch_gemm(LD_ROWS, EP_GELU, g1, st));
          const int rc_f = srk_launch_qkv_attn_fwd(c.at<bf16_t>(ba.xn1w), CP, c.packed + bw.Wqkv, c.side + bw.bqkv, bw.scale, nullptr,
                                                   c.side + bw.biasd, c.at<bf16_t>(ba.ao), T / 64, bw.nH, bw.CA, CP, geom, st);
          if (rc_f == SRK_NOT_COVERED) RUN(srk_launch_attn_fwd(c.at<bf16_t>(ba.qkv), c.side + bw.biasd, c.at<bf16_t>(ba.ao), T / 64, bw.nH, geom, st));
          else RUN(rc_f);
        }
        int rc_mlpb = SRK_NOT_COVERED;
        if (fuse_ln) {
          GemmParams g = {};
          g.A = c.at<bf16_t>(w.gxb2); g.lda = CP; g.Wt = c.packed + bw.Wfc2T; g.K = CP; g.HP = HP; g.aux = c.at<bf16_t>(ba.u);
          g.u_out = c.at<bf16_t>(w.du); g.W2 = c.packed + bw.Wfc1T; g.M = T; g.N = CP; g.ldo = CP;
          g.outf = c.at<float>(w.gx2); g.outb = c.at<bf16_t>(w.gxbw); g.geom = geom; g.rowscale = ds_attn; g.rows_per_sample = HW;
          g.ln_x = c.at<float>(ba.x1); g.ln_mean = c.at<float>(ba.mean2); g.ln_rstd = c.at<float>(ba.rstd2);
          g.ln_gamma = params + bw.n2w; g.ln_dgamma = grads + bw.n2w; g.ln_dbeta = grads + bw.n2b; g.ln_C = C;
          g.ln_rows_window = 0; g.ln_stats_by_m = 0; g.ln_out_window = 1;
          g.flops = 2.0 * fl_mlp;
          g.bytes = (double)T * (2.0 * C + 2.0 * p->HID + 2.0 * p->HID + 4.0 * C + 8.0 * C + 2.0 * C) + 4.0 * C * p->HID;
          g.u_dgelu = w.u_is_dgelu && !w.ckpt;
          rc_mlpb = srk_launch_mlp_fused_bwd(g, st);
          if (rc_mlpb != SRK_NOT_COVERED) RUN(rc_mlpb);
        }
        if (rc_mlpb == SRK_NOT_COVERED && w.u_is_dgelu && !w.ckpt) {
          srk_set_error("train step: the forward stored gelu'(u) for the fused MLP backward, which is not available now "
                        "(mlp_bwd_fused / gemm_stream changed between forward and backward?)");
          return SRK_E_UNSUPPORTED;
        }
        if (rc_mlpb == SRK_NOT_COVERED) {
          GemmParams g = {};
          g.A = c.at<bf16_t>(w.gxb2); g.lda = CP; g.Wt = c.packed + bw.Wfc2T; g.M = T; g.N = HP; g.K = CP;
          g.outb = c.at<bf16_t>(w.du); g.aux = c.at<bf16_t>(ba.u); g.ldo = HP; g.flops = fl_mlp;
          g.bytes = (double)T * (2.0 * C + 2.0 * p->HID + 2.0 * p->HID) + 2.0 * C * p->HID;
          RUN(srk_launch_gemm(LD_ROWS, EP_DGELU, g, st));
        }
        WgradParams wq[4];
        wq[0] = lin_wgrad(c, c.at<bf16_t>(w.gxb2), CP, c.at<bf16_t>(ba.h), HP, T, bw.Wfc2, bw.bfc2, fl_mlp);
        if (rc_mlpb == SRK_NOT_COVERED) {
          GemmParams g = {};
          g.A = c.at<bf16_t>(w.du); g.lda = HP; g.Wt = c.packed + bw.Wfc1T; g.M = T; g.N = CP; g.K = HP;
          g.ldo = CP; g.flops = fl_mlp;
          g.bytes = (double)T * (2.0 * p->HID + 4.0 * C + 8.0 * C + 2.0 * C) + 2.0 * C * p->HID;
          if (fuse_ln) {
            g.outf = c.at<float>(w.gx2); g.outb = c.at<bf16_t>(w.gxbw); g.geom = geom; g.rowscale = ds_attn; g.rows_per_sample = HW;
            g.ln_x = c.at<float>(ba.x1); g.ln_mean = c.at<float>(ba.mean2); g.ln_rstd = c.at<float>(ba.rstd2);
            g.ln_gamma = params + bw.n2w; g.ln_dgamma = grads + bw.n2w; g.ln_dbeta = grads + bw.n2b; g.ln_C = C;
            g.ln_rows_window = 0; g.ln_stats_by_m = 0; g.ln_out_window = 1;
            RUN(srk_launch_gemm(LD_ROWS, EP_LNBWD, g, st));
          } else {
            g.outb = c.at<bf16_t>(w.dxn);
            RUN(srk_launch_gemm(LD_ROWS, EP_BF16, g, st));
          }
        }
        wq[1] = lin_wgrad(c, c.at<bf16_t>(w.du), HP, c.at<bf16_t>(ba.xn2), CP, T, bw.Wfc1, bw.bfc1, fl_mlp);
        if (!fuse_ln && rc_mlpb == SRK_NOT_COVERED) {
          RUN(srk_launch_ln_bwd(c.at<bf16_t>(w.dxn), c.at<float>(ba.x1), c.at<float>(ba.mean2), c.at<float>(ba.rstd2),
                                params + bw.n2w, c.at<float>(w.gx2), c.at<bf16_t>(w.gxbw), grads + bw.n2w, grads + bw.n2b, T, C, CP,
                                &geom, 0, 0, 1, 1, ds_attn, HW, st));
        }
        wq[2] = lin_wgrad(c, c.at<bf16_t>(w.gxbw), CP, c.at<bf16_t>(ba.ao), bw.CA, T, bw.Wproj, bw.bproj, fl_proj);
        int nslab;
        if (w.attn_recompute) {
          const int rc_abf = srk_launch_qkv_attn_bwd(c.at<bf16_t>(ba.xn1w), CP, c.packed + bw.Wqkv, c.side + bw.bqkv, bw.scale,
                                                     c.at<bf16_t>(w.gxbw), CP, c.packed + bw.WprojT, c.side + bw.biasd,
                                                     c.at<bf16_t>(w.dqkv), c.at<float>(w.slab), T / 64, bw.nH, bw.CA, CP, geom, st);
          SRK_REQUIRE(rc_abf != SRK_NOT_COVERED, SRK_E_STATE, "backward: the re-projecting attention backward cannot run but the "
                      "forward stored no q/k/v (option attn_bwd_fused changed between forward and backward?)");
          RUN(rc_abf);
          nslab = srk_qkv_attn_bwd_slabs(T / 64, bw.nH, bw.CA, CP);
        } else {
          {
            GemmParams g = {};
            g.A = c.at<bf16_t>(w.gxbw); g.lda = CP; g.Wt = c.packed + bw.WprojT; g.M = T; g.N = bw.CA; g.K = CP;
            g.outb = c.at<bf16_t>(w.dao); g.ldo = bw.CA; g.flops = fl_proj; g.bytes = (double)T * 4.0 * C + 2.0 * C * C;
            RUN(srk_launch_gemm(LD_ROWS, EP_BF16, g, st));
          }
          RUN(srk_launch_attn_bwd(c.at<bf16_t>(ba.qkv), c.side + bw.biasd, c.at<bf16_t>(w.dao), c.at<bf16_t>(w.dqkv),
                                  c.at<float>(w.slab), nullptr, T / 64, bw.nH, geom, bw.scale, st));
          nslab = srk_attn_bwd_slabs(T / 64, bw.nH, nullptr);
        }
        const RpbJob rpb = {c.at<float>(w.slab), grads + bw.rpb, nslab, bw.nH};
        wq[3] = lin_wgrad(c, c.at<bf16_t>(w.dqkv), 3 * bw.CA, c.at<bf16_t>(ba.xn1w), CP, T, bw.Wqkv, bw.bqkv, fl_qkv);
        RUN(srk_launch_wgrad_multi_rpb(wq, 4, &rpb, st));
        {
          GemmParams g = {};
          g.A = c.at<bf16_t>(w.dqkv); g.lda = 3 * bw.CA; g.Wt = c.packed + bw.WqkvT; g.M = T; g.N = CP; g.K = 3 * bw.CA;
          g.ldo = CP; g.flops = fl_qkv;
          g.bytes = (double)T * (6.0 * C + 4.0 * C + 8.0 * C + 2.0 * C) + 6.0 * C * C;
          if (fuse_ln) {
            g.outf = c.at<float>(w.gx2); g.outb = c.at<bf16_t>(j > 0 ? w.gxb2 : w.gxb); g.geom = geom; g.rowscale = j > 0 ? ds_prev_mlp : nullptr;
            g.rows_per_sample = HW;
            g.ln_skip = j > 0 ? nullptr : c.at<float>(w.gx);
            skip_folded = j == 0;
            g.ln_x = c.at<float>(ba.x_in); g.ln_mean = c.at<float>(ba.mean1); g.ln_rstd = c.at<float>(ba.rstd1);
            g.ln_gamma = params + bw.n1w; g.ln_dgamma = grads + bw.n1w; g.ln_dbeta = grads + bw.n1b; g.ln_C = C;
            g.ln_rows_window = 1; g.ln_stats_by_m = 1; g.ln_out_window = 0;
            RUN(srk_launch_gemm(LD_ROWS, EP_LNBWD, g, st));
          } else {
            g.outb = c.at<bf16_t>(w.dxn);
            RUN(srk_launch_gemm(LD_ROWS, EP_BF16, g, st));
            RUN(srk_launch_ln_bwd(c.at<bf16_t>(w.dxn), c.at<float>(ba.x_in), c.at<float>(ba.mean1), c.at<float>(ba.rstd1),
                                  params + bw.n1w, c.at<float>(w.gx2), c.at<bf16_t>(w.gxb2), grads + bw.n1w, grads + bw.n1b, T, C, CP,
                                  &geom, 1, 1, 0, 1, ds_prev_mlp, HW, st));
          }
        }
      }
      if (!skip_folded) RUN(srk_launch_add_f32_bf16(c.at<float>(w.gx), c.at<float>(w.gx2), c.at<bf16_t>(w.gxb), (long long)T * CP, st));
      RUN(unpack_group(c, l + 1, grads));
    } else {
      if (p->p_ape >= 0)
        RUN(srk_launch_ape_grad(c.at<float>(w.gx), grads + p->p_ape, B, p->cfg.img_size * p->cfg.img_size, C, CP, st));
      RUN(srk_launch_ln_bwd(c.at<bf16_t>(w.gxb), c.at<float>(w.f0), c.at<float>(w.mean_pe), c.at<float>(w.rstd_pe),
                            params + p->p_pe_w, c.at<float>(w.gx2), nullptr, grads + p->p_pe_w, grads + p->p_pe_b, T, C, CP, nullptr, 0,
                            0, 0, 0, nullptr, HW, st));
      RUN(srk_launch_add_bf16_into_f32(c.at<float>(w.gx2), c.at<bf16_t>(w.gfb), (long long)T * CP, st));
      RUN(srk_launch_stem_wgrad(c.at<float>(w.img4), c.at<float>(w.gx2), grads + p->p_conv_first_w, grads + p->p_conv_first_b, B, H, W,
                                p->Cimg, C, CP, st));
      RUN(unpack_group(c, 0, grads));
    }
  }
  return SRK_OK;
}

}
```

tpu_superresolution_amd/csrc/wgrad.h:

```cpp
#pragma once
#include "common.h"

struct WgradParams {
  const bf16_t* Y;
  int ldy;
  const bf16_t* X;
  int ldx;
  int M, N, K;
  float* dW;
  int ldw;
  float* db;
  int m_per;
  int conv;
  int B, H, W;
  double flops;
  double bytes;
  int r, Cs;
};

struct RpbJob {
  const float* slab;
  float* dtable;
  int nslab, nH;
};

struct WgradMulti {
  int nprob;
  int m_per;
  int tile_begin[5];
  float* partial;
  int nsplit;
  int w8;
  RpbJob rpb;
  WgradParams p[4];
};

__device__ __forceinline__ void rpb_reduce_block(const float* __restrict__ slab, float* __restrict__ dtable, int nslab, int nH, int i,
                                                 int h, float (*part)[64]) {
  const int lane = threadIdx.x & 63, wave = threadIdx.x >> 6;
  float a8[8] = {0.f, 0.f, 0.f, 0.f, 0.f, 0.f, 0.f, 0.f};
  const long long sstride = (long long)nH * 4096;
  const float* base = slab + ((long long)h * 64 + i) * 64 + lane;
  int sidx = wave;
  for (; sidx + 28 < nslab; sidx += 32) {
#pragma unroll
    for (int u = 0; u < 8; ++u) a8[u] += base[(sidx + 4 * u) * sstride];
  }
  for (; sidx < nslab; sidx += 4) a8[0] += base[sidx * sstride];
  part[wave][lane] = ((a8[0] + a8[1]) + (a8[2] + a8[3])) + ((a8[4] + a8[5]) + (a8[6] + a8[7]));
  __syncthreads();
  if (wave == 0) {
    const float v = part[0][lane] + part[1][lane] + part[2][lane] + part[3][lane];
    const int t = ((i >> 3) - (lane >> 3) + 7) * 15 + ((i & 7) - (lane & 7) + 7);
    atomicAdd(dtable + t * nH + h, v);
  }
}

constexpr int WS_SLAB_VEC = 9216;
constexpr size_t WS_WORKSPACE_BYTES = (size_t)256 * WS_SLAB_VEC * 16;
float* srk_wgrad_scratch(hipStream_t stream, size_t bytes);
void srk_wgrad_bind_workspace(void* ptr, size_t bytes, void** prev_ptr, size_t* prev_bytes);
void srk_wgrad_partials_enable(int on);
void srk_wgrad_w8_enable(int on);
void srk_wgrad_stream_tune(int rows, int nt);
int srk_wgrad_partials_enabled();
int srk_wgrad_stream_enabled();
int srk_wgrad_w8_enabled();
void srk_wgrad_stream_tune_get(int* rows, int* nt);

int srk_launch_wgrad(const WgradParams& p, hipStream_t stream);

#define SRK_WGRAD_NOT_COVERED 1
int srk_launch_conv_wgrad_taps(const WgradParams& p, hipStream_t stream);
void srk_conv_wgrad_taps_enable(int on);
int srk_conv_wgrad_taps_mode();
void srk_conv_wgrad_roll_enable(int on);
int srk_conv_wgrad_roll_enabled();
int srk_launch_smallconv_wgrad_mfma(const bf16_t* x, const float* gy, float* dW, float* db, int B, int H, int W, int Cin, int CinP, int Co,
                                    int CoP, hipStream_t stream);
int srk_launch_imghead_dgrad_mfma(const float* gy, const float* wgt, bf16_t* dx, int B, int H, int W, int Cin, int CinP, int Co, int CoP,
                                  hipStream_t stream);
void srk_wgrad_stream_enable(int on);
int srk_launch_wgrad_multi(const WgradParams* ps, int nprob, hipStream_t stream);
int srk_launch_wgrad_multi_rpb(const WgradParams* ps, int nprob, const RpbJob* rpb, hipStream_t stream);
int srk_launch_rpb_reduce(const float* slab, float* dtable, int nslab, int nH, hipStream_t stream);
```

tpu_superresolution_amd/csrc/wgrad.hip:

```cpp
#include "wgrad.h"

namespace {

template <int TA, int TB, bool CONV>
__global__ __launch_bounds__(256) void wgrad_kernel(const WgradMulti mp) {
  const int ntiles = mp.tile_begin[mp.nprob];
  const int logical = xcd_remap(blockIdx.x, gridDim.x);
  const int bsplit = logical / ntiles, btile = logical - bsplit * ntiles;
  int pi = 0;
  while (pi + 1 < mp.nprob && btile >= mp.tile_begin[pi + 1]) ++pi;
  const WgradParams& p = mp.p[pi];
  constexpr int TN = 64 * TA, TK = 64 * TB;
  constexpr int SY = TN + 16, SX = TK + 16;
  constexpr int PY = (64 * TN / 8) / 256;
  constexpr int PX = (64 * TK / 8) / 256;
  extern __shared__ __attribute__((aligned(16))) unsigned char smem[];
  bf16_t* Ys = reinterpret_cast<bf16_t*>(smem);
  bf16_t* Xs = Ys + 2 * 64 * SY;

  const int tid = threadIdx.x, lane = tid & 63, wave = tid >> 6;
  const int r16 = lane & 15, g = lane >> 4;
  const int wn = wave >> 1, wk = wave & 1;
  const int ntn = p.N / TN, ntk = p.K / TK;
  int bx = btile - mp.tile_begin[pi];
  const int tn = bx % ntn; bx /= ntn;
  const int tk = bx % ntk; bx /= ntk;
  const int tap = bx;
  const int n0 = tn * TN, k0 = tk * TK;
  const int dy = CONV ? tap / 3 - 1 : 0, dx = CONV ? tap % 3 - 1 : 0;
  const int m_begin = bsplit * mp.m_per;
  const int m_end = min(p.M, m_begin + mp.m_per);
  const int nchunk = (m_end - m_begin + 63) / 64;
  if (nchunk <= 0) return;

  uint4 ry[PY], rx[PX];
  auto load_stage = [&](int ch) {
    const int mb = m_begin + ch * 64;
#pragma unroll
    for (int t = 0; t < PY; ++t) {
      const int pid = tid + 256 * t;
      const int row = pid / (TN / 8), c8 = pid % (TN / 8);
      const int m = mb + row;
      uint4 v = make_uint4(0, 0, 0, 0);
      if (m < m_end) {
        if (CONV && p.r > 1) {
          const int hw = p.H * p.W;
          const int b = m / hw, rem = m - b * hw;
          const int y = rem / p.W, x = rem - y * p.W;
          const int nn = n0 + c8 * 8;
          const int ij = nn / p.Cs, c = nn - ij * p.Cs;
          const int si = ij / p.r, sj = ij - si * p.r;
          v = *reinterpret_cast<const uint4*>(
              p.Y + (((long long)(b * p.H * p.r + y * p.r + si)) * (p.W * p.r) + x * p.r + sj) * p.Cs + c);
        } else {
          v = *reinterpret_cast<const uint4*>(p.Y + (long long)m * p.ldy + n0 + c8 * 8);
        }
      }
      ry[t] = v;
    }
#pragma unroll
    for (int t = 0; t < PX; ++t) {
      const int pid = tid + 256 * t;
      const int row = pid / (TK / 8), c8 = pid % (TK / 8);
      const int m = mb + row;
      uint4 v = make_uint4(0, 0, 0, 0);
      if (m < m_end) {
        if (CONV) {
          const int hw = p.H * p.W;
          const int b = m / hw, rem = m - b * hw;
          const int y = rem / p.W + dy, x = rem % p.W + dx;
          if ((unsigned)y < (unsigned)p.H && (unsigned)x < (unsigned)p.W)
            v = *reinterpret_cast<const uint4*>(p.X + ((long long)(b * p.H + y) * p.W + x) * p.ldx + k0 + c8 * 8);
        } else {
          v = *reinterpret_cast<const uint4*>(p.X + (long long)m * p.ldx + k0 + c8 * 8);
        }
      }
      rx[t] = v;
    }
  };
  auto store_stage = [&](int buf) {
    bf16_t* ys = Ys + buf * 64 * SY;
    bf16_t* xs = Xs + buf * 64 * SX;
#pragma unroll
    for (int t = 0; t < PY; ++t) {
      const int pid = tid + 256 * t;
      *reinterpret_cast<uint4*>(ys + (pid / (TN / 8)) * SY + (pid % (TN / 8)) * 8) = ry[t];
    }
#pragma unroll
    for (int t = 0; t < PX; ++t) {
      const int pid = tid + 256 * t;
      *reinterpret_cast<uint4*>(xs + (pid / (TK / 8)) * SX + (pid % (TK / 8)) * 8) = rx[t];
    }
  };

  constexpr int NTW = 2 * TA, KTW = 2 * TB;
  f32x4_t acc[NTW][KTW], accb[NTW];
#pragma unroll
  for (int i = 0; i < NTW; ++i) {
    accb[i] = f32x4_t{0.f, 0.f, 0.f, 0.f};
#pragma unroll
    for (int j = 0; j < KTW; ++j) acc[i][j] = f32x4_t{0.f, 0.f, 0.f, 0.f};
  }
  const bool do_bias = p.db != nullptr && tk == 0 && wk == 0 && tap == 0;
  const bf16x8_t ones = bf16x8_t{0x3F80, 0x3F80, 0x3F80, 0x3F80, 0x3F80, 0x3F80, 0x3F80, 0x3F80};

  load_stage(0);
  store_stage(0);
  __syncthreads();
  for (int ch = 0; ch < nchunk; ++ch) {
    const int buf = ch & 1;
    if (ch + 1 < nchunk) load_stage(ch + 1);
    const bf16_t* ys = Ys + buf * 64 * SY;
    const bf16_t* xs = Xs + buf * 64 * SX;
#pragma unroll
    for (int ks = 0; ks < 2; ++ks) {
      bf16x8_t yf[NTW], xf[KTW];
#pragma unroll
      for (int i = 0; i < NTW; ++i) {
        const int c0 = wn * (32 * TA) + 16 * i;
        const bf16x4_t lo = lds_tr_read(tr_addr(ys, SY, 32 * ks + 4 * g, c0, lane));
        const bf16x4_t hi = lds_tr_read(tr_addr(ys, SY, 32 * ks + 16 + 4 * g, c0, lane));
        yf[i] = bf16x8_t{lo[0], lo[1], lo[2], lo[3], hi[0], hi[1], hi[2], hi[3]};
      }
#pragma unroll
      for (int j = 0; j < KTW; ++j) {
        const int c0 = wk * (32 * TB) + 16 * j;
        const bf16x4_t lo = lds_tr_read(tr_addr(xs, SX, 32 * ks + 4 * g, c0, lane));
        const bf16x4_t hi = lds_tr_read(tr_addr(xs, SX, 32 * ks + 16 + 4 * g, c0, lane));
        xf[j] = bf16x8_t{lo[0], lo[1], lo[2], lo[3], hi[0], hi[1], hi[2], hi[3]};
      }
#pragma unroll
      for (int i = 0; i < NTW; ++i)
#pragma unroll
        for (int j = 0; j < KTW; ++j)
          acc[i][j] = __builtin_amdgcn_mfma_f32_16x16x32_bf16(yf[i], xf[j], acc[i][j], 0, 0, 0);
      if (do_bias) {
#pragma unroll
        for (int i = 0; i < NTW; ++i) accb[i] = __builtin_amdgcn_mfma_f32_16x16x32_bf16(yf[i], ones, accb[i], 0, 0, 0);
      }
    }
    if (ch + 1 < nchunk) store_stage(buf ^ 1);
    __syncthreads();
  }

  const long long koff = CONV ? (long long)tap * p.K : 0;
#pragma unroll
  for (int i = 0; i < NTW; ++i) {
    const int n = n0 + wn * (32 * TA) + 16 * i + 4 * g;
#pragma unroll
    for (int j = 0; j < KTW; ++j) {
      const int k = k0 + wk * (32 * TB) + 16 * j + r16;
#pragma unroll
      for (int e = 0; e < 4; ++e) atomicAdd(p.dW + (long long)(n + e) * p.ldw + koff + k, acc[i][j][e]);
    }
    if (do_bias && r16 == 0) {
#pragma unroll
      for (int e = 0; e < 4; ++e) atomicAdd(p.db + n + e, accb[i][e]);
    }
  }
}

constexpr int WS_LDS_BYTES = 147456;

__device__ __forceinline__ const bf16_t* tr_addr_swz(const bf16_t* tile, int rbase, int c0, int lane) {
  const int ll = lane & 15;
  const int row = rbase + (ll >> 2);
  return tile + row * 192 + (((c0 >> 4) ^ ((row >> 1) & 3)) << 4) + ((ll & 3) << 2);
}

template <int ROWS, bool NT, bool W8>
__global__ __launch_bounds__(W8 ? 512 : 256) void wgrad_stream_kernel(const WgradMulti mp) {
  constexpr int FI = W8 ? 3 : 6;
  constexpr int STAGE_ELEMS = 2 * ROWS * 192;
  constexpr int RING = WS_LDS_BYTES / (STAGE_ELEMS * 2);
  constexpr int NI = ROWS * 24 / 256;
  constexpr int AHEAD = RING - 1;
  const int ntiles = mp.tile_begin[mp.nprob];
  const int logical = xcd_remap(blockIdx.x, gridDim.x);
  const int bsplit = logical / ntiles, btile = logical - bsplit * ntiles;
  int pi = 0;
  while (pi + 1 < mp.nprob && btile >= mp.tile_begin[pi + 1]) ++pi;
  const WgradParams& p = mp.p[pi];
  extern __shared__ __attribute__((aligned(16))) unsigned char smem[];
  bf16_t* ring = reinterpret_cast<bf16_t*>(smem);
  const unsigned ring_base = (unsigned)(size_t)smem;

  const int tid = threadIdx.x, lane = tid & 63;
  const int wave = __builtin_amdgcn_readfirstlane(tid >> 6);
  const int r16 = lane & 15, g = lane >> 4;
  const int wn = wave >> 1, wk = wave & 1;
  const bool loader = wave < 4;
  const int ntn = p.N / 192;
  const int bx = btile - mp.tile_begin[pi];
  const int tn = bx % ntn, tk = bx / ntn;
  const int n0 = tn * 192, k0 = tk * 192;
  const int m_begin = bsplit * mp.m_per;
  const int m_end = min(p.M, m_begin + mp.m_per);
  const int nchunk = (m_end - m_begin) / ROWS;
  if (nchunk <= 0) return;

  int yoff[NI], xoff[NI];
#pragma unroll
  for (int i = 0; i < NI; ++i) {
    const int q = (wave & 3) * (NI * 64) + i * 64 + lane;
    const int row = q / 24, pos = q - row * 24;
    const int c = (((pos >> 1) ^ ((row >> 1) & 3)) << 1) | (pos & 1);
    yoff[i] = row * p.ldy + n0 + c * 8;
    xoff[i] = row * p.ldx + k0 + c * 8;
  }
  auto issue = [&](int ch) {
    if (!loader) return;
    const int m0 = m_begin + ch * ROWS;
    const bf16_t* yb = p.Y + (long long)m0 * p.ldy;
    const bf16_t* xb = p.X + (long long)m0 * p.ldx;
    const unsigned dst = ring_base + (unsigned)((ch % RING) * STAGE_ELEMS * 2);
#pragma unroll
    for (int i = 0; i < NI; ++i)
      srk_glds16<NT>(yb + yoff[i], __builtin_amdgcn_readfirstlane(dst + (wave * (NI * 64) + i * 64) * 16));
#pragma unroll
    for (int i = 0; i < NI; ++i)
      srk_glds16<NT>(xb + xoff[i], __builtin_amdgcn_readfirstlane(dst + ROWS * 192 * 2 + (wave * (NI * 64) + i * 64) * 16));
  };

  f32x4_t acc[FI][6], accb[FI];
#pragma unroll
  for (int i = 0; i < FI; ++i) {
    accb[i] = f32x4_t{0.f, 0.f, 0.f, 0.f};
#pragma unroll
    for (int j = 0; j < 6; ++j) acc[i][j] = f32x4_t{0.f, 0.f, 0.f, 0.f};
  }
  const bool do_bias = p.db != nullptr && tk == 0 && wk == 0;
  const bf16x8_t ones = bf16x8_t{0x3F80, 0x3F80, 0x3F80, 0x3F80, 0x3F80, 0x3F80, 0x3F80, 0x3F80};

  for (int c = 0; c < AHEAD && c < nchunk; ++c) issue(c);
  for (int ch = 0; ch < nchunk; ++ch) {
    if (ch + AHEAD - 1 < nchunk) {
      srk_wait_vmcnt<2 * NI * (AHEAD - 1)>();
    } else {
      srk_wait_vmcnt<0>();
    }
    srk_lds_barrier();
    if (ch + AHEAD < nchunk) issue(ch + AHEAD);
    const bf16_t* ys = ring + (ch % RING) * STAGE_ELEMS;
    const bf16_t* xs = ys + ROWS * 192;
#pragma unroll
    for (int ks = 0; ks < ROWS / 32; ++ks) {
      bf16x8_t yf[FI], xf[6];
#pragma unroll
      for (int i = 0; i < FI; ++i) {
        const int c0 = wn * (16 * FI) + 16 * i;
        const bf16x4_t lo = lds_tr_read(tr_addr_swz(ys, 32 * ks + 4 * g, c0, lane));
        const bf16x4_t hi = lds_tr_read(tr_addr_swz(ys, 32 * ks + 16 + 4 * g, c0, lane));
        yf[i] = bf16x8_t{lo[0], lo[1], lo[2], lo[3], hi[0], hi[1], hi[2], hi[3]};
      }
#pragma unroll
      for (int j = 0; j < 6; ++j) {
        const int c0 = wk * 96 + 16 * j;
        const bf16x4_t lo = lds_tr_read(tr_addr_swz(xs, 32 * ks + 4 * g, c0, lane));
        const bf16x4_t hi = lds_tr_read(tr_addr_swz(xs, 32 * ks + 16 + 4 * g, c0, lane));
        xf[j] = bf16x8_t{lo[0], lo[1], lo[2], lo[3], hi[0], hi[1], hi[2], hi[3]};
      }
#pragma unroll
      for (int i = 0; i < FI; ++i)
#pragma unroll
        for (int j = 0; j < 6; ++j) acc[i][j] = __builtin_amdgcn_mfma_f32_16x16x32_bf16(yf[i], xf[j], acc[i][j], 0, 0, 0);
      if (do_bias) {
#pragma unroll
        for (int i = 0; i < FI; ++i) accb[i] = __builtin_amdgcn_mfma_f32_16x16x32_bf16(yf[i], ones, accb[i], 0, 0, 0);
      }
    }
  }

  if (mp.partial != nullptr) {
    f32x4_t* slab = reinterpret_cast<f32x4_t*>(mp.partial) + (((size_t)btile * 144 + wave * (FI * 6)) * mp.nsplit + bsplit) * 64 + lane;
#pragma unroll
    for (int i = 0; i < FI; ++i)
#pragma unroll
      for (int j = 0; j < 6; ++j) slab[(size_t)(i * 6 + j) * mp.nsplit * 64] = acc[i][j];
  }
#pragma unroll
  for (int i = 0; i < FI; ++i) {
    const int n = n0 + wn * (16 * FI) + 16 * i + 4 * g;
    if (mp.partial == nullptr) {
#pragma unroll
      for (int j = 0; j < 6; ++j) {
        const int k = k0 + wk * 96 + 16 * j + r16;
#pragma unroll
        for (int e = 0; e < 4; ++e) atomicAdd(p.dW + (long long)(n + e) * p.ldw + k, acc[i][j][e]);
      }
    }
    if (do_bias && r16 == 0) {
#pragma unroll
      for (int e = 0; e < 4; ++e) atomicAdd(p.db + n + e, accb[i][e]);
    }
  }
}

__global__ __launch_bounds__(256) void wgrad_reduce_kernel(const WgradMulti mp) {
  if ((int)blockIdx.x >= 36 * mp.tile_begin[mp.nprob]) {
    __shared__ float part[4][64];
    const int b = blockIdx.x - 36 * mp.tile_begin[mp.nprob];
    rpb_reduce_block(mp.rpb.slab, mp.rpb.dtable, mp.rpb.nslab, mp.rpb.nH, b & 63, b >> 6, part);
    return;
  }
  const int btile = blockIdx.x / 36;
  const int q = (blockIdx.x - btile * 36) * 256 + threadIdx.x;
  int pi = 0;
  while (pi + 1 < mp.nprob && btile >= mp.tile_begin[pi + 1]) ++pi;
  const WgradParams& p = mp.p[pi];
  const int ntn = p.N / 192;
  const int bx = btile - mp.tile_begin[pi];
  const int tn = bx % ntn, tk = bx / ntn;
  const f32x4_t* src = reinterpret_cast<const f32x4_t*>(mp.partial) + ((size_t)btile * 144 + (q >> 6)) * mp.nsplit * 64 + (q & 63);
  f32x4_t sum = f32x4_t{0.f, 0.f, 0.f, 0.f};
  int s = 0;
  for (; s + 8 <= mp.nsplit; s += 8) {
    f32x4_t v[8];
#pragma unroll
    for (int u = 0; u < 8; ++u) v[u] = src[(s + u) * 64];
#pragma unroll
    for (int u = 0; u < 8; ++u) sum += v[u];
  }
  for (; s < mp.nsplit; ++s) sum += src[s * 64];
  const int lane = q & 63, t = q >> 6;
  const int fi = mp.w8 ? 3 : 6;
  const int j = t % 6, i = (t / 6) % fi, wave = t / (6 * fi);
  const int wn = wave >> 1, wk = wave & 1, r16 = lane & 15, g = lane >> 4;
  const int n = tn * 192 + wn * (16 * fi) + 16 * i + 4 * g;
  const int k = tk * 192 + wk * 96 + 16 * j + r16;
#pragma unroll
  for (int e = 0; e < 4; ++e) atomicAdd(p.dW + (long long)(n + e) * p.ldw + k, sum[e]);
}

thread_local const RpbJob* t_rpb = nullptr;
thread_local bool t_rpb_done = false;

SrkOpt g_wgrad_stream{OPT_WGRAD_STREAM, 1};
SrkOpt g_wgrad_rows{OPT_WGRAD_ROWS, 32};
SrkOpt g_wgrad_nt{OPT_WGRAD_NT, 1};
#ifndef SRK_WGRAD_W8_DEFAULT
#define SRK_WGRAD_W8_DEFAULT 1
#endif
SrkOpt g_wgrad_w8{OPT_WGRAD_W8, SRK_WGRAD_W8_DEFAULT};
SrkOpt g_wgrad_partials{OPT_WGRAD_PARTIALS, 1};

template <int TA, int TB, bool CONV>
int launch(const WgradParams* ps, int nprob, hipStream_t stream) {
  constexpr size_t lds = (size_t)2 * 64 * ((64 * TA + 16) + (64 * TB + 16)) * sizeof(bf16_t);
  static SrkPerDevice<bool> configured_pd; bool& configured = configured_pd.here();
  if (!configured) {
    if (hipFuncSetAttribute(reinterpret_cast<const void*>(&wgrad_kernel<TA, TB, CONV>),
                            hipFuncAttributeMaxDynamicSharedMemorySize, (int)lds) != hipSuccess) {
      srk_set_error("wgrad: cannot reserve %zu bytes of LDS", lds);
      return SRK_E_LAUNCH;
    }
    configured = true;
  }
  WgradMulti mp;
  mp.nprob = nprob;
  mp.partial = nullptr;
  mp.nsplit = 0;
  mp.rpb = RpbJob{nullptr, nullptr, 0, 0};
  mp.w8 = 0;
  int tiles = 0;
  double flops = 0.0, bytes = 0.0;
  for (int i = 0; i < nprob; ++i) {
    mp.p[i] = ps[i];
    mp.tile_begin[i] = tiles;
    tiles += (ps[i].N / (64 * TA)) * (ps[i].K / (64 * TB)) * (CONV ? 9 : 1);
    flops += ps[i].flops;
    bytes += ps[i].bytes;
  }
  mp.tile_begin[nprob] = tiles;
  const int M = ps[0].M;
  int splits = 256 / tiles;
  if (splits < 1) splits = 1;
  int m_per = round_up(cdiv(M, splits), 64);
  if (m_per < 256) m_per = 256;
  mp.m_per = m_per;
  splits = cdiv(M, m_per);
  const int fam = CONV ? FAM_WGRAD_CONV : FAM_WGRAD_LINEAR;
  if constexpr (TA == 3 && TB == 3 && !CONV) {
    bool ok = g_wgrad_stream && M % 64 == 0;
    for (int i = 0; i < nprob; ++i) ok = ok && ps[i].ldy % 8 == 0 && ps[i].ldx % 8 == 0;
    if (ok) {
      constexpr int slds = WS_LDS_BYTES;
      using KernelFn = void (*)(const WgradMulti);
      static const KernelFn fns[8] = {&wgrad_stream_kernel<64, false, false>, &wgrad_stream_kernel<64, true, false>,
                                      &wgrad_stream_kernel<32, false, false>, &wgrad_stream_kernel<32, true, false>,
                                      &wgrad_stream_kernel<64, false, true>,  &wgrad_stream_kernel<64, true, true>,
                                      &wgrad_stream_kernel<32, false, true>,  &wgrad_stream_kernel<32, true, true>};
      static SrkPerDevice<bool> sconf_pd; bool& sconf = sconf_pd.here();
      if (!sconf) {
        for (KernelFn f : fns)
          if (hipFuncSetAttribute(reinterpret_cast<const void*>(f), hipFuncAttributeMaxDynamicSharedMemorySize, slds) != hipSuccess) {
            srk_set_error("wgrad(stream): cannot reserve %d bytes of LDS", slds);
            return SRK_E_LAUNCH;
          }
        sconf = true;
      }
      const KernelFn fn = fns[(g_wgrad_w8 ? 4 : 0) + (g_wgrad_rows == 32 ? 2 : 0) + (g_wgrad_nt ? 1 : 0)];
      mp.nsplit = splits;
      mp.w8 = g_wgrad_w8;
      mp.partial = g_wgrad_partials && splits > 1 ? srk_wgrad_scratch(stream, (size_t)tiles * splits * WS_SLAB_VEC * 16) : nullptr;
      srk_probe_pre(fam, stream, flops, bytes);
      hipLaunchKernelGGL(fn, dim3(tiles * splits), dim3(g_wgrad_w8 ? 512 : 256), slds, stream, mp);
      if (mp.partial) {
        int extra = 0;
        if (t_rpb && t_rpb->slab) {
          mp.rpb = *t_rpb;
          extra = 64 * t_rpb->nH;
          t_rpb_done = true;
        }
        hipLaunchKernelGGL(wgrad_reduce_kernel, dim3(tiles * 36 + extra), dim3(256), 0, stream, mp);
      }
      srk_probe_post(fam, stream);
      return srk_check_launch("wgrad(stream)");
    }
  }
  srk_probe_pre(fam, stream, flops, bytes);
  hipLaunchKernelGGL((wgrad_kernel<TA, TB, CONV>), dim3(tiles * splits), dim3(256), lds, stream, mp);
  srk_probe_post(fam, stream);
  return srk_check_launch("wgrad");
}

inline void tile_class(const WgradParams& p, int& a, int& b) {
  a = p.N % 192 == 0 ? 3 : (p.N % 128 == 0 ? 2 : 1);
  b = p.K % 192 == 0 ? 3 : (p.K % 128 == 0 ? 2 : 1);
}

template <bool CONV>
int dispatch(const WgradParams* ps, int nprob, hipStream_t stream) {
  int a, b;
  tile_class(ps[0], a, b);
#define WCASE(A, B) \
  if (a == A && b == B) return launch<A, B, CONV>(ps, nprob, stream);
  WCASE(3, 3) WCASE(3, 1) WCASE(1, 3) WCASE(2, 2) WCASE(2, 1) WCASE(1, 2) WCASE(1, 1) WCASE(3, 2) WCASE(2, 3)
#undef WCASE
  srk_set_error("wgrad: no tile for N=%d K=%d", ps[0].N, ps[0].K);
  return SRK_E_UNSUPPORTED;
}

int validate(const WgradParams& p) {
  SRK_REQUIRE(p.M > 0 && p.N % 64 == 0 && p.K % 64 == 0, SRK_E_SHAPE, "wgrad: bad M/N/K %d/%d/%d", p.M, p.N, p.K);
  SRK_REQUIRE(p.Y && p.X && p.dW, SRK_E_NULL, "wgrad: null operand");
  if (p.conv) {
    SRK_REQUIRE(p.M == p.B * p.H * p.W, SRK_E_SHAPE, "wgrad(conv): M != B*H*W");
    if (p.r > 1) SRK_REQUIRE(p.Cs % 8 == 0 && p.N == p.r * p.r * p.Cs, SRK_E_SHAPE, "wgrad(conv,ps): bad Cs");
  }
  return SRK_OK;
}

}

void srk_wgrad_stream_enable(int on) { g_wgrad_stream = on ? 1 : 0; }
void srk_wgrad_partials_enable(int on) { g_wgrad_partials = on ? 1 : 0; }
void srk_wgrad_w8_enable(int on) { g_wgrad_w8 = on ? 1 : 0; }
void srk_wgrad_stream_tune(int rows, int nt) {
  if (rows == 32 || rows == 64) g_wgrad_rows = rows;
  if (nt >= 0) g_wgrad_nt = nt ? 1 : 0;
}
int srk_wgrad_partials_enabled() { return g_wgrad_partials; }
int srk_wgrad_stream_enabled() { return g_wgrad_stream; }
int srk_wgrad_w8_enabled() { return g_wgrad_w8; }
void srk_wgrad_stream_tune_get(int* rows, int* nt) { *rows = g_wgrad_rows; *nt = g_wgrad_nt; }

namespace {
thread_local float* t_wgrad_ws = nullptr;
thread_local size_t t_wgrad_ws_bytes = 0;
}
void srk_wgrad_bind_workspace(void* ptr, size_t bytes, void** prev_ptr, size_t* prev_bytes) {
  if (prev_ptr) *prev_ptr = t_wgrad_ws;
  if (prev_bytes) *prev_bytes = t_wgrad_ws_bytes;
  t_wgrad_ws = static_cast<float*>(ptr);
  t_wgrad_ws_bytes = ptr ? bytes : 0;
}
float* srk_wgrad_scratch(hipStream_t, size_t bytes) { return bytes <= t_wgrad_ws_bytes ? t_wgrad_ws : nullptr; }

int srk_launch_wgrad(const WgradParams& p, hipStream_t stream) {
  int rc = validate(p);
  if (rc) return rc;
  if (p.conv) {
    rc = srk_launch_conv_wgrad_taps(p, stream);
    if (rc != SRK_WGRAD_NOT_COVERED) return rc;
  }
  return p.conv ? dispatch<true>(&p, 1, stream) : dispatch<false>(&p, 1, stream);
}

int srk_launch_wgrad_multi_rpb(const WgradParams* ps, int nprob, const RpbJob* rpb, hipStream_t stream) {
  t_rpb = rpb;
  t_rpb_done = false;
  int rc = srk_launch_wgrad_multi(ps, nprob, stream);
  t_rpb = nullptr;
  if (rc == SRK_OK && rpb && rpb->slab && !t_rpb_done) rc = srk_launch_rpb_reduce(rpb->slab, rpb->dtable, rpb->nslab, rpb->nH, stream);
  return rc;
}

int srk_launch_wgrad_multi(const WgradParams* ps, int nprob, hipStream_t stream) {
  SRK_REQUIRE(nprob >= 1 && nprob <= 4, SRK_E_SHAPE, "wgrad_multi: nprob=%d", nprob);
  bool same = true;
  int a0, b0;
  tile_class(ps[0], a0, b0);
  for (int i = 0; i < nprob; ++i) {
    int rc = validate(ps[i]);
    if (rc) return rc;
    int a, b;
    tile_class(ps[i], a, b);
    same = same && a == a0 && b == b0 && ps[i].M == ps[0].M && !ps[i].conv;
  }
  if (same) return dispatch<false>(ps, nprob, stream);
  for (int i = 0; i < nprob; ++i) {
    int rc = srk_launch_wgrad(ps[i], stream);
    if (rc) return rc;
  }
  return SRK_OK;
}
```

tpu_superresolution_amd/ops.py:

```python
from __future__ import annotations

import ctypes as C
from typing import Optional, Tuple

import threading

import torch

from . import _lib
from ._lib import WinGeom, check, lib


def _stream() -> int:
    return torch.cuda.current_stream().cuda_stream


def _p(t: Optional[torch.Tensor]) -> Optional[int]:
    if t is None:
        return None
    if not t.is_cuda:
        raise RuntimeError("libsrk operates on GPU tensors only (got a CPU tensor); there is no CPU fallback")
    if t.device.index != torch.cuda.current_device():
        raise RuntimeError(f"tensor on {t.device} but the current device is cuda:{torch.cuda.current_device()}; "
                           "libsrk ops launch on the current device (torch.cuda.set_device / one process per GPU)")
# ... 142 lines not shown

def linear_bf16(a: torch.Tensor, w: torch.Tensor, bias: Optional[torch.Tensor]) -> torch.Tensor:
    M, K = a.shape
    N = w.shape[0]
    y = torch.empty((M, N), dtype=torch.bfloat16, device=a.device)
    check(lib().srk_linear_bf16(_p(a), _p(w), _p(bias), _p(y), M, N, K, _stream()))
    return y


_WGRAD_WS = {}


def _bind_wgrad_workspace(device: torch.device) -> None:
    key = (device.index if device.index is not None else torch.cuda.current_device())
    ws = _WGRAD_WS.get(key)
    if ws is None:
        ws = _WGRAD_WS[key] = torch.empty(int(lib().srk_wgrad_workspace_bytes()), dtype=torch.uint8, device=device)
    check(lib().srk_set_wgrad_workspace(_p(ws), ws.numel()))


def linear_wgrad_bf16(y: torch.Tensor, x: torch.Tensor, with_bias: bool = True):
    M, N = y.shape
    K = x.shape[1]
    dw = torch.zeros((N, K), dtype=torch.float32, device=y.device)
    db = torch.zeros((N,), dtype=torch.float32, device=y.device) if with_bias else None
    _bind_wgrad_workspace(y.device)
    check(lib().srk_linear_wgrad_bf16(_p(y), _p(x), _p(dw), _p(db), M, N, K, _stream()))
    return dw, db


class ZeroArena:

    def __init__(self):
        self.need = 0
        self.buf = None
        self.off = 0

    def begin(self, device) -> None:
        want = max(self.need, self.off)
        self.need = want
        self.buf = torch.zeros(want, dtype=torch.float32, device=device) if want > 0 else None
        self.off = 0

    def zeros(self, shape, device) -> torch.Tensor:
        shape = tuple(shape) if not isinstance(shape, int) else (shape,)
        n = 1
        for d in shape:
            n *= int(d)
        n_al = (n + 63) // 64 * 64
        o = self.off
        self.off += n_al
        if self.buf is not None and self.buf.device == device and o + n_al <= self.buf.numel():
            return self.buf[o:o + n].view(shape)
        return torch.zeros(shape, dtype=torch.float32, device=device)


_ARENA = threading.local()


def zeros_f32(shape, device) -> torch.Tensor:
    ar = getattr(_ARENA, "cur", None)
    if ar is None:
        return torch.zeros(shape, dtype=torch.float32, device=device)
    return ar.zeros(shape, device)


class arena_scope:

    def __init__(self, arena: "ZeroArena", device):
        self.arena, self.device = arena, device

    def __enter__(self):
        self.prev = getattr(_ARENA, "cur", None)
        self.arena.begin(self.device)
        _ARENA.cur = self.arena
        return self.arena

    def __exit__(self, *exc):
        _ARENA.cur = self.prev
        self.arena.need = max(self.arena.need, self.arena.off)
        return False


def linear_wgrad_multi_bf16(pairs):
    from ._lib import WgradProblem
    assert 1 <= len(pairs) <= 4
    M = pairs[0][0].shape[0]
    dev = pairs[0][0].device
    arr = (WgradProblem * len(pairs))()
    outs = []
    for i, (y, x) in enumerate(pairs):
        assert y.shape[0] == M and x.shape[0] == M and y.stride(1) == 1 and x.stride(1) == 1
        N, K = y.shape[1], x.shape[1]
        dw = zeros_f32((N, K), dev)
        db = zeros_f32((N,), dev)
        arr[i].y, arr[i].ldy, arr[i].x, arr[i].ldx = y.data_ptr(), y.stride(0), x.data_ptr(), x.stride(0)
        arr[i].dw, arr[i].db, arr[i].N, arr[i].K = dw.data_ptr(), db.data_ptr(), N, K
        outs.append((dw, db))
    _bind_wgrad_workspace(dev)
    check(lib().srk_linear_wgrad_multi_bf16(arr, len(pairs), M, _stream()))
    return outs


def conv3x3_bf16(x: torch.Tensor, w: torch.Tensor, bias: Optional[torch.Tensor]) -> torch.Tensor:
    B, H, W, CinP = x.shape
    N = w.shape[0]
    y = torch.empty((B, H, W, N), dtype=torch.bfloat16, device=x.device)
    check(lib().srk_conv3x3_bf16(_p(x), _p(w), _p(bias), _p(y), B, H, W, CinP, N, _stream()))
    return y


def conv3x3_wgrad_bf16(dy: torch.Tensor, x: torch.Tensor):
    B, H, W, N = dy.shape
    CinP = x.shape[-1]
    dw = torch.zeros((N, 9 * CinP), dtype=torch.float32, device=x.device)
    db = torch.zeros((N,), dtype=torch.float32, device=x.device)
    _bind_wgrad_workspace(x.device)
    check(lib().srk_conv3x3_wgrad_bf16(_p(dy), _p(x), _p(dw), _p(db), B, H, W, CinP, N, _stream()))
    return dw, db


def probe_trread(tile: torch.Tensor) -> torch.Tensor:
    out = torch.empty((64, 8), dtype=torch.int16, device=tile.device)
    check(lib().srk_probe_trread(_p(tile), _p(out), _stream()))
    return out


def batch_psnr(pred: torch.Tensor, target: torch.Tensor, max_val: float = 1.0, psnr_sum: Optional[torch.Tensor] = None,
               abs_sum: Optional[torch.Tensor] = None) -> torch.Tensor:
    assert pred.shape == target.shape and pred.dtype == torch.float32 and target.dtype == torch.float32
    pred, target = pred.contiguous(), target.contiguous()
    B = pred.shape[0]
    per_image = pred.numel() // B
    ws = torch.empty(int(lib().srk_batch_psnr_workspace(per_image, B)), dtype=torch.uint8, device=pred.device)
    out = torch.empty(B, dtype=torch.float32, device=pred.device)
    check(lib().srk_batch_psnr(_p(pred), _p(target), _p(ws), B, per_image, float(max_val), _p(out), _p(psnr_sum), _p(abs_sum), _stream()))
    return out


def eval_psnr(x: torch.Tensor, y: torch.Tensor, max_val: float = 1.0):
    assert x.shape == y.shape and x.dtype == torch.float32 and y.dtype == torch.float32
    x, y = x.contiguous(), y.contiguous()
    B = x.shape[0]
    per_image = x.numel() // B
    ws = torch.empty(int(lib().srk_eval_psnr_workspace(per_image, B)), dtype=torch.uint8, device=x.device)
    per, mean = torch.empty(B, dtype=torch.float32, device=x.device), torch.empty(1, dtype=torch.float32, device=x.device)
    check(lib().srk_eval_psnr(_p(x), _p(y), _p(ws), B, per_image, float(max_val), _p(per), _p(mean), _stream()))
    return per, mean


def ssim(x: torch.Tensor, y: torch.Tensor, data_range: float = 1.0):
    assert x.shape == y.shape and x.ndim == 4 and x.dtype == torch.float32 and y.dtype == torch.float32
    x, y = x.contiguous(), y.contiguous()
    B, Cc, H, W = x.shape
    ws = torch.empty(max(4, int(lib().srk_ssim_workspace(B, Cc, H, W))), dtype=torch.uint8, device=x.device)
    per, mean = torch.empty(B, dtype=torch.float32, device=x.device), torch.empty(1, dtype=torch.float32, device=x.device)
    check(lib().srk_ssim(_p(x), _p(y), _p(ws), B, Cc, H, W, float(data_range), _p(per), _p(mean), _stream()))
    return per, mean


class TensorTable:

    def __init__(self, n: int):
        self.n = int(n)
        self.numel = (C.c_int64 * self.n)()
        self.ptrs = {}

    def set(self, role: str, tensors, first: bool = False) -> None:
        if len(tensors) != self.n:
            raise ValueError(f"multi-tensor optimizer: {len(tensors)} {role} tensors for a table of {self.n}")
        arr = self.ptrs.get(role)
        if arr is None:
            arr = self.ptrs[role] = (C.c_void_p * self.n)()
        cur, numel, f32 = None, self.numel, torch.float32
        for i, t in enumerate(tensors):
            if t.dtype is not f32:
                raise TypeError(f"multi-tensor optimizer: {role}[{i}] must be float32 (got {t.dtype})")
            if cur is None and t.is_cuda:
                cur = torch.cuda.current_device()
            if not t.is_cuda or t.device.index != cur or not t.is_contiguous():
                _p(t)
            arr[i] = t.data_ptr()
            if first:
                numel[i] = t.numel()
# ... 105 lines not shown
```

Before: 75.75 million HR pixels/s.

## Run weight-gradient GEMMs on idle CUs inside the attention backward kernel

Adds a combined kernel in which the first workgroups run the fused qkv+attention backward role and the remaining workgroups, on CUs the attention grid leaves idle, stream independent weight-gradient problems (proj, MLP) into split partials. The remaining wgrad problems and the relative-position-bias reduction then run in a follow-up multi-wgrad launch that also folds the ridden partials. This targets the underfilled device during attention backward, where only 16*groups workgroups occupy CUs. The cost is a new workspace, more complex dispatch, and a risk of bandwidth or LDS contention slowing the attention role.

After: 76.45 million HR pixels/s, median of 6. No clear change (+0.9%).

```diff
diff --git a/include/srk.h b/include/srk.h
--- a/include/srk.h
+++ b/include/srk.h
@@ -45,10 +45,18 @@
                                    const uint16_t* d_x1, int ldg, const uint16_t* w_proj_t, const float* bias_dense, uint16_t* d_qkv,
                                    float* d_table, void* slab, int64_t B_, int nH, const srk_win_geom* geom, srk_stream_t stream);
 size_t srk_window_attention_bwd_fused_scratch(int64_t B_, int nH);
+struct srk_wgrad_problem_s;
+size_t srk_window_attention_bwd_ride_scratch(int64_t B_, int nH);
+int64_t srk_window_attention_bwd_ride_workspace_bytes(void);
+int srk_window_attention_bwd_ride(const uint16_t* xn, int lda, const uint16_t* w_qkv, const float* b_qkv, float scale,
+                                  const uint16_t* d_x1, int ldg, const uint16_t* w_proj_t, const float* bias_dense, uint16_t* d_qkv,
+                                  float* d_table, void* slab, int64_t B_, int nH, const srk_win_geom* geom,
+                                  const struct srk_wgrad_problem_s* problems, int count, int nride, int M, void* ride_ws,
+                                  int64_t ride_ws_bytes, int phases, srk_stream_t stream);
 int srk_rel_pos_bias_expand(const float* table, float* bias_dense, int nH, srk_stream_t stream);
 int srk_linear_bf16(const uint16_t* a, const uint16_t* w, const float* bias, uint16_t* y, int M, int N, int K, srk_stream_t stream);
 int srk_linear_wgrad_bf16(const uint16_t* y, const uint16_t* x, float* dw, float* db, int M, int N, int K, srk_stream_t stream);
-typedef struct {
+typedef struct srk_wgrad_problem_s {
   const void* y; int ldy;
   const void* x; int ldx;
   float* dw; float* db;
diff --git a/tpu_superresolution_amd/_lib.py b/tpu_superresolution_amd/_lib.py
--- a/tpu_superresolution_amd/_lib.py
+++ b/tpu_superresolution_amd/_lib.py
@@ -84,6 +84,10 @@
     "srk_window_attention_bwd_scratch": (_sz, [_i64, _i]),
     "srk_window_attention_bwd_fused": (_i, [_vp, _i, _vp, _vp, _f, _vp, _i, _vp, _vp, _vp, _vp, _vp, _i64, _i, _geom_p, _vp]),
     "srk_window_attention_bwd_fused_scratch": (_sz, [_i64, _i]),
+    "srk_window_attention_bwd_ride": (_i, [_vp, _i, _vp, _vp, _f, _vp, _i, _vp, _vp, _vp, _vp, _vp, _i64, _i, _geom_p, C.POINTER(WgradProblem), _i,
+                                           _i, _i, _vp, _i64, _i, _vp]),
+    "srk_window_attention_bwd_ride_scratch": (_sz, [_i64, _i]),
+    "srk_window_attention_bwd_ride_workspace_bytes": (_i64, []),
     "srk_rel_pos_bias_expand": (_i, [_vp, _vp, _i, _vp]),
     "srk_linear_bf16": (_i, [_vp, _vp, _vp, _vp, _i, _i, _i, _vp]),
     "srk_linear_wgrad_bf16": (_i, [_vp, _vp, _vp, _vp, _i, _i, _i, _vp]),
diff --git a/tpu_superresolution_amd/csrc/api.hip b/tpu_superresolution_amd/csrc/api.hip
--- a/tpu_superresolution_amd/csrc/api.hip
+++ b/tpu_superresolution_amd/csrc/api.hip
@@ -224,6 +224,59 @@
   return srk_launch_rpb_reduce((const float*)slab, d_table, nslab, nH, (hipStream_t)stream);
 }
 
+size_t srk_window_attention_bwd_ride_scratch(int64_t B_, int nH) {
+  return (size_t)srk_qkv_attn_bwd_ride_slabs(B_, nH, nH * 32, 192) * nH * 4096 * sizeof(float);
+}
+
+int64_t srk_window_attention_bwd_ride_workspace_bytes(void) { return (int64_t)RIDE_WORKSPACE_BYTES; }
+
+int srk_window_attention_bwd_ride(const uint16_t* xn, int lda, const uint16_t* w_qkv, const float* b_qkv, float scale,
+                                  const uint16_t* d_x1, int ldg, const uint16_t* w_proj_t, const float* bias_dense, uint16_t* d_qkv,
+                                  float* d_table, void* slab, int64_t B_, int nH, const srk_win_geom* geom,
+                                  const srk_wgrad_problem* problems, int count, int nride, int M, void* ride_ws, int64_t ride_ws_bytes,
+                                  int phases, srk_stream_t stream) {
+  REQ_PTR(xn); REQ_PTR(w_qkv); REQ_PTR(d_x1); REQ_PTR(w_proj_t); REQ_PTR(bias_dense); REQ_PTR(d_qkv); REQ_PTR(d_table); REQ_PTR(slab);
+  REQ_PTR(geom); REQ_PTR(problems); REQ_PTR(ride_ws);
+  REQ_ALIGN(xn); REQ_ALIGN(w_qkv); REQ_ALIGN(d_x1); REQ_ALIGN(w_proj_t); REQ_ALIGN(d_qkv); REQ_ALIGN(slab); REQ_ALIGN(ride_ws);
+  WinGeom g;
+  int rc = make_geom(geom, &g, "window_attention_bwd_ride");
+  if (rc) return rc;
+  SRK_REQUIRE(B_ > 0 && B_ % g.nW == 0, SRK_E_SHAPE, "window_attention_bwd_ride: B_=%lld nW=%d", (long long)B_, g.nW);
+  SRK_REQUIRE(count >= 2 && count <= 4 && nride >= 1 && nride <= 3 && nride < count && M > 0 && phases >= 1 && phases <= 3 && ride_ws_bytes > 0,
+              SRK_E_SHAPE, "window_attention_bwd_ride: count=%d nride=%d M=%d phases=%d", count, nride, M, phases);
+  WgradParams ps[4] = {};
+  for (int i = 0; i < count; ++i) {
+    const srk_wgrad_problem& q = problems[i];
+    REQ_PTR(q.y); REQ_PTR(q.x); REQ_PTR(q.dw); REQ_ALIGN(q.y); REQ_ALIGN(q.x);
+    SRK_REQUIRE(q.N > 0 && q.K > 0 && (q.ldy <= 0 || q.ldy >= q.N) && (q.ldx <= 0 || q.ldx >= q.K), SRK_E_SHAPE,
+                "window_attention_bwd_ride: problem %d: N=%d K=%d ldy=%d ldx=%d", i, q.N, q.K, q.ldy, q.ldx);
+    ps[i].Y = static_cast<const bf16_t*>(q.y); ps[i].ldy = q.ldy > 0 ? q.ldy : q.N;
+    ps[i].X = static_cast<const bf16_t*>(q.x); ps[i].ldx = q.ldx > 0 ? q.ldx : q.K;
+    ps[i].M = M; ps[i].N = q.N; ps[i].K = q.K; ps[i].dW = q.dw; ps[i].ldw = q.K; ps[i].db = q.db;
+  }
+  const int nslab = srk_qkv_attn_bwd_ride_slabs(B_, nH, nH * 32, 192);
+  SRK_REQUIRE(nslab > 0 && srk_wgrad_ride_applies(ps, count) && srk_wgrad_w8_enabled(), SRK_E_UNSUPPORTED,
+              "window_attention_bwd_ride: needs 6 heads x 32, K = 192, at least one window per CU, fewer than #CUs attention "
+              "workgroups, and problems the streaming weight-gradient kernel with split partials covers (nH=%d B_=%lld)", nH, (long long)B_);
+  WgradMulti ridden;
+  if (phases & 1) {
+    rc = srk_launch_qkv_attn_bwd_ride(xn, lda, w_qkv, b_qkv, scale, d_x1, ldg, w_proj_t, bias_dense, d_qkv, (float*)slab, B_, nH, nH * 32, 192,
+                                      g, ps, nride, (float*)ride_ws, (size_t)ride_ws_bytes, &ridden, (hipStream_t)stream);
+    SRK_REQUIRE(rc != SRK_NOT_COVERED, SRK_E_UNSUPPORTED, "window_attention_bwd_ride: the kernel cannot run on this build / shape / workspace");
+    if (rc) return rc;
+  } else {
+    const size_t need = srk_wgrad_ride_plan(ps, nride, srk_device_cus() - 2 * nslab, &ridden);
+    SRK_REQUIRE(need > 0 && need <= (size_t)ride_ws_bytes, SRK_E_UNSUPPORTED, "window_attention_bwd_ride: workspace of %lld bytes",
+                (long long)ride_ws_bytes);
+    ridden.partial = (float*)ride_ws;
+  }
+  if (phases & 2) {
+    const RpbJob rpb = {(const float*)slab, d_table, nslab, nH};
+    rc = srk_launch_wgrad_multi_ridden(ps + nride, count - nride, ridden, &rpb, (hipStream_t)stream);
+  }
+  return rc;
+}
+
 int srk_rel_pos_bias_expand(const float* table, float* bias_dense, int nH, srk_stream_t stream) {
   REQ_PTR(table); REQ_PTR(bias_dense);
   return srk_launch_rpb_expand(table, bias_dense, nH, (hipStream_t)stream);
@@ -356,6 +409,14 @@
 const OptEntry kOptions[] = {
     {"gemm_stream", [] { return srk_gemm_stream_enabled(); }, [](int v) { srk_gemm_stream_enable(v); return (int)SRK_OK; }},
     {"attn_bwd_fused", [] { return srk_attn_bwd_fused_enabled(); }, [](int v) { srk_attn_bwd_fused_enable(v); return (int)SRK_OK; }},
+    {"attn_bwd_ride", [] { return srk_attn_bwd_ride_option(0); }, [](int v) { srk_attn_bwd_ride_set_option(0, v != 0); return (int)SRK_OK; }},
+    {"attn_bwd_ride_groups", [] { return srk_attn_bwd_ride_option(1); },
+     [](int v) {
+       SRK_REQUIRE(v >= 1 && v <= 64, SRK_E_SHAPE, "attn_bwd_ride_groups: 1..64");
+       srk_attn_bwd_ride_set_option(1, v);
+       return (int)SRK_OK;
+     }},
+    {"attn_bwd_ride_set", [] { return srk_attn_bwd_ride_option(2); }, [](int v) { srk_attn_bwd_ride_set_option(2, v != 0); return (int)SRK_OK; }},
     {"attn_fused", [] { return srk_attn_fused_mode(); }, [](int v) { srk_attn_fused_enable(v); return (int)SRK_OK; }},
     {"wgrad_stream_w8", [] { return srk_wgrad_w8_enabled(); }, [](int v) { srk_wgrad_w8_enable(v); return (int)SRK_OK; }},
     {"block_light", [] { return srk_block_light_enabled(); }, [](int v) { srk_block_light_enable(v); return (int)SRK_OK; }},
diff --git a/tpu_superresolution_amd/csrc/attn_bwd_fused.hip b/tpu_superresolution_amd/csrc/attn_bwd_fused.hip
--- a/tpu_superresolution_amd/csrc/attn_bwd_fused.hip
+++ b/tpu_superresolution_amd/csrc/attn_bwd_fused.hip
@@ -1,4 +1,5 @@
 #include "kernels.h"
+#include "wgrad_stream.h"
 
 namespace {
 
@@ -60,8 +61,7 @@
   return h_cat4(lds_tr_read(tile + ra * 64 + ((c ^ ps(ra)) << 3) + in), lds_tr_read(tile + rb * 64 + ((c ^ ps(rb)) << 3) + in));
 }
 
-__global__ __launch_bounds__(768) void qkv_attn_bwd_kernel(const BwdFusedParams p, int ngrp) {
-  extern __shared__ __attribute__((aligned(16))) unsigned char smem[];
+__device__ __forceinline__ void qkv_attn_bwd_role(const BwdFusedParams& p, int ngrp, unsigned char* smem) {
   const unsigned smem_base = (unsigned)(size_t)smem;
   const int tid = threadIdx.x, lane = tid & 63;
   const int wave = __builtin_amdgcn_readfirstlane(tid >> 6);
@@ -320,12 +320,38 @@
     *reinterpret_cast<float4*>(slab + 16 * jt) = make_float4(dbias[jt][0], dbias[jt][1], dbias[jt][2], dbias[jt][3]);
 }
 
+__global__ __launch_bounds__(768) void qkv_attn_bwd_kernel(const BwdFusedParams p, int ngrp) {
+  extern __shared__ __attribute__((aligned(16))) unsigned char smem[];
+  qkv_attn_bwd_role(p, ngrp, smem);
+}
+
+template <int ROWS, bool NT>
+__global__ __launch_bounds__(768) void qkv_attn_bwd_ride_kernel(const BwdFusedParams p, int ngrp, const WgradMulti mp) {
+  extern __shared__ __attribute__((aligned(16))) unsigned char smem[];
+  const int nattn = 16 * ngrp;
+  if ((int)blockIdx.x < nattn) {
+    qkv_attn_bwd_role(p, ngrp, smem);
+  } else {
+    if (threadIdx.x >= 512) return;
+    wgrad_stream_role<ROWS, NT, true>(mp, (int)blockIdx.x - nattn, (int)gridDim.x - nattn, smem);
+  }
+}
+static_assert(WS_LDS_BYTES <= H_LDS, "the rider's ring fits the attention role's LDS");
+
 SrkOpt g_attn_bwd_fused{OPT_ATTN_BWD_FUSED, 1};
+#ifndef SRK_ATTN_BWD_RIDE_DEFAULT
+#define SRK_ATTN_BWD_RIDE_DEFAULT 1
+#endif
+SrkOpt g_attn_bwd_ride{OPT_ATTN_BWD_RIDE, SRK_ATTN_BWD_RIDE_DEFAULT};
+SrkOpt g_attn_bwd_ride_groups{OPT_ATTN_BWD_RIDE_GROUPS, 10};
+SrkOpt g_attn_bwd_ride_set{OPT_ATTN_BWD_RIDE_SET, 0};
 
 }
 
 void srk_attn_bwd_fused_enable(int on) { g_attn_bwd_fused = on ? 1 : 0; }
 int srk_attn_bwd_fused_enabled() { return g_attn_bwd_fused; }
+void srk_attn_bwd_ride_set_option(int which, int v) { (which == 0 ? g_attn_bwd_ride : which == 1 ? g_attn_bwd_ride_groups : g_attn_bwd_ride_set) = v; }
+int srk_attn_bwd_ride_option(int which) { return which == 0 ? g_attn_bwd_ride : which == 1 ? g_attn_bwd_ride_groups : g_attn_bwd_ride_set; }
 
 static int abf_cus() { return srk_device_cus(); }
 
@@ -364,3 +390,47 @@
   srk_probe_post(FAM_ATTN_BWD, stream);
   return srk_check_launch("qkv+attention backward");
 }
+
+int srk_qkv_attn_bwd_ride_slabs(long long B_, int nH, int CA, int K) {
+  if (!g_attn_bwd_ride || srk_qkv_attn_bwd_slabs(B_, nH, CA, K) == 0) return 0;
+  const int ngrp = g_attn_bwd_ride_groups;
+  if (ngrp < 1 || 16 * ngrp >= abf_cus() || B_ < 8LL * ngrp) return 0;
+  return 8 * ngrp;
+}
+
+int srk_launch_qkv_attn_bwd_ride(const bf16_t* xn, int lda, const bf16_t* Wqkv, const float* bqkv, float scale, const bf16_t* g, int ldg,
+                                 const bf16_t* WprojT, const float* biasd, bf16_t* dqkv, float* slab, long long B_, int nH, int CA, int K,
+                                 WinGeom geom, const WgradParams* ride, int nride, float* ride_partial, size_t ride_partial_bytes,
+                                 WgradMulti* ridden, hipStream_t stream) {
+  const int nslab = srk_qkv_attn_bwd_ride_slabs(B_, nH, CA, K);
+  if (nslab == 0 || lda % 8 != 0 || ldg % 8 != 0 || B_ * 64 * (long long)(lda > ldg ? lda : ldg) >= (1LL << 31)) return SRK_NOT_COVERED;
+  if (nride < 1 || nride > 3 || !ride_partial || !srk_wgrad_ride_applies(ride, nride) || !srk_wgrad_w8_enabled()) return SRK_NOT_COVERED;
+  const int ngrp = nslab / 8, riders = abf_cus() - 16 * ngrp;
+  const size_t need = srk_wgrad_ride_plan(ride, nride, riders, ridden);
+  if (need == 0 || need > ride_partial_bytes) return SRK_NOT_COVERED;
+  int rows, nt;
+  srk_wgrad_stream_tune_get(&rows, &nt);
+  using RideFn = void (*)(const BwdFusedParams, int, const WgradMulti);
+  static const RideFn fns[4] = {&qkv_attn_bwd_ride_kernel<64, false>, &qkv_attn_bwd_ride_kernel<64, true>,
+                                &qkv_attn_bwd_ride_kernel<32, false>, &qkv_attn_bwd_ride_kernel<32, true>};
+  const int which = (rows == 32 ? 2 : 0) + (nt ? 1 : 0);
+  struct Conf { int v[4]; };
+  static SrkPerDevice<Conf> conf_pd; int& configured = conf_pd.here().v[which];
+  if (!configured) {
+    const void* fn = reinterpret_cast<const void*>(fns[which]);
+    hipFuncAttributes attr;
+    configured = -1;
+    if (hipFuncGetAttributes(&attr, fn) == hipSuccess && attr.localSizeBytes == 0 &&
+        hipFuncSetAttribute(fn, hipFuncAttributeMaxDynamicSharedMemorySize, H_LDS) == hipSuccess)
+      configured = 1;
+  }
+  if (configured < 0) return SRK_NOT_COVERED;
+  ridden->partial = ride_partial;
+  BwdFusedParams bp;
+  bp.xn = xn; bp.lda = lda; bp.g = g; bp.ldg = ldg; bp.Wqkv = Wqkv; bp.bqkv = bqkv; bp.scale = scale; bp.WprojT = WprojT;
+  bp.biasd = biasd; bp.dqkv = dqkv; bp.slab = slab; bp.B_ = B_; bp.geom = geom;
+  srk_probe_pre(FAM_ATTN_BWD, stream, 0.0);
+  hipLaunchKernelGGL(fns[which], dim3(16 * ngrp + riders), dim3(768), H_LDS, stream, bp, ngrp, *ridden);
+  srk_probe_post(FAM_ATTN_BWD, stream);
+  return srk_check_launch("qkv+attention backward with riding weight gradients");
+}
diff --git a/tpu_superresolution_amd/csrc/common.h b/tpu_superresolution_amd/csrc/common.h
--- a/tpu_superresolution_amd/csrc/common.h
+++ b/tpu_superresolution_amd/csrc/common.h
@@ -20,7 +20,8 @@
 enum SrkOptId {
   OPT_MLP_FUSED, OPT_MLP_BWD_FUSED, OPT_GEMM_STREAM, OPT_TUNE_BM, OPT_TUNE_KS2, OPT_TUNE_SPLIT, OPT_TUNE_NB, OPT_ATTN_BWD_FUSED,
   OPT_ATTN_FUSED, OPT_BLOCK_LIGHT, OPT_TAPS_ENABLED, OPT_TAPS_DMA, OPT_WGRAD_STREAM, OPT_WGRAD_ROWS, OPT_WGRAD_NT, OPT_WGRAD_W8,
-  OPT_WGRAD_PARTIALS, OPT_MLP_DGELU_STORE, OPT_TAPS_ROLL, SRK_NUM_OPTS
+  OPT_WGRAD_PARTIALS, OPT_MLP_DGELU_STORE, OPT_TAPS_ROLL, OPT_ATTN_BWD_RIDE, OPT_ATTN_BWD_RIDE_GROUPS,
+  OPT_ATTN_BWD_RIDE_SET, SRK_NUM_OPTS
 };
 struct SrkOptTls {
   int v[SRK_NUM_OPTS];
diff --git a/tpu_superresolution_amd/csrc/kernels.h b/tpu_superresolution_amd/csrc/kernels.h
--- a/tpu_superresolution_amd/csrc/kernels.h
+++ b/tpu_superresolution_amd/csrc/kernels.h
@@ -25,6 +25,13 @@
 int srk_launch_qkv_attn_bwd(const bf16_t* xn, int lda, const bf16_t* Wqkv, const float* bqkv, float scale, const bf16_t* g, int ldg,
                             const bf16_t* WprojT, const float* biasd, bf16_t* dqkv, float* slab, long long B_, int nH, int CA, int K,
                             WinGeom geom, hipStream_t stream);
+void srk_attn_bwd_ride_set_option(int which, int v);
+int srk_attn_bwd_ride_option(int which);
+int srk_qkv_attn_bwd_ride_slabs(long long B_, int nH, int CA, int K);
+int srk_launch_qkv_attn_bwd_ride(const bf16_t* xn, int lda, const bf16_t* Wqkv, const float* bqkv, float scale, const bf16_t* g, int ldg,
+                                 const bf16_t* WprojT, const float* biasd, bf16_t* dqkv, float* slab, long long B_, int nH, int CA, int K,
+                                 WinGeom geom, const WgradParams* ride, int nride, float* ride_partial, size_t ride_partial_bytes,
+                                 WgradMulti* ridden, hipStream_t stream);
 
 int srk_launch_ln_fwd(const float* x, const float* gamma, const float* beta, bf16_t* yb, float* yf, float* mean,
                       float* rstd, int rows, int C, int CP, const WinGeom* geom, hipStream_t stream);
diff --git a/tpu_superresolution_amd/csrc/swinir.hip b/tpu_superresolution_amd/csrc/swinir.hip
--- a/tpu_superresolution_amd/csrc/swinir.hip
+++ b/tpu_superresolution_amd/csrc/swinir.hip
@@ -63,7 +63,7 @@
   std::vector<ResiAct> resi;
   std::vector<size_t> nc_u, nc_a;
   size_t nc_hr = 0;
-  size_t gx, gxb, gx2, gxb2, gxbw, du, dxn, dao, dqkv, slab, wgpart, gyimg, gt1, gfb, gfb32, gstage_w, gstage_side;
+  size_t gx, gxb, gx2, gxb2, gxbw, du, dxn, dao, dqkv, slab, wgpart, ridepart, gyimg, gt1, gfb, gfb32, gstage_w, gstage_side;
   size_t g3a = 0, g3b = 0;
   size_t ncgA = 0, ncgB = 0, ncgU = 0;
   std::vector<size_t> gup;
@@ -381,6 +381,7 @@
     if (w.attn_recompute) nslab = (size_t)srk_qkv_attn_bwd_slabs(w.T / 64, p->blocks[0].nH, p->blocks[0].CA, p->CP);
     w.slab = a.get("slab", nslab * maxH * 4096 * 4);
     w.wgpart = a.get("wgpart", WS_WORKSPACE_BYTES);
+    w.ridepart = a.get("ridepart", RIDE_WORKSPACE_BYTES);
     w.gfb = a.get("gfb", T * CP * 2);
     w.gfb32 = a.get("gfb32", T * CP * 4);
     if (p->cfg.resi_connection == SRK_RESI_3CONV) {
@@ -1258,7 +1259,19 @@
         }
         wq[2] = lin_wgrad(c, c.at<bf16_t>(w.gxbw), CP, c.at<bf16_t>(ba.ao), bw.CA, T, bw.Wproj, bw.bproj, fl_proj);
         int nslab;
-        if (w.attn_recompute) {
+        wq[3] = lin_wgrad(c, c.at<bf16_t>(w.dqkv), 3 * bw.CA, c.at<bf16_t>(ba.xn1w), CP, T, bw.Wqkv, bw.bqkv, fl_qkv);
+        WgradMulti ridden;
+        const int nride = srk_attn_bwd_ride_option(2) ? 3 : 2;
+        int rc_ride = SRK_NOT_COVERED;
+        if (w.attn_recompute && srk_wgrad_ride_applies(wq, 4))
+          rc_ride = srk_launch_qkv_attn_bwd_ride(c.at<bf16_t>(ba.xn1w), CP, c.packed + bw.Wqkv, c.side + bw.bqkv, bw.scale,
+                                                 c.at<bf16_t>(w.gxbw), CP, c.packed + bw.WprojT, c.side + bw.biasd, c.at<bf16_t>(w.dqkv),
+                                                 c.at<float>(w.slab), T / 64, bw.nH, bw.CA, CP, geom, wq, nride, c.at<float>(w.ridepart),
+                                                 RIDE_WORKSPACE_BYTES, &ridden, st);
+        if (rc_ride != SRK_NOT_COVERED) {
+          RUN(rc_ride);
+          nslab = srk_qkv_attn_bwd_ride_slabs(T / 64, bw.nH, bw.CA, CP);
+        } else if (w.attn_recompute) {
           const int rc_abf = srk_launch_qkv_attn_bwd(c.at<bf16_t>(ba.xn1w), CP, c.packed + bw.Wqkv, c.side + bw.bqkv, bw.scale,
                                                      c.at<bf16_t>(w.gxbw), CP, c.packed + bw.WprojT, c.side + bw.biasd,
                                                      c.at<bf16_t>(w.dqkv), c.at<float>(w.slab), T / 64, bw.nH, bw.CA, CP, geom, st);
@@ -1278,8 +1291,8 @@
           nslab = srk_attn_bwd_slabs(T / 64, bw.nH, nullptr);
         }
         const RpbJob rpb = {c.at<float>(w.slab), grads + bw.rpb, nslab, bw.nH};
-        wq[3] = lin_wgrad(c, c.at<bf16_t>(w.dqkv), 3 * bw.CA, c.at<bf16_t>(ba.xn1w), CP, T, bw.Wqkv, bw.bqkv, fl_qkv);
-        RUN(srk_launch_wgrad_multi_rpb(wq, 4, &rpb, st));
+        if (rc_ride != SRK_NOT_COVERED) RUN(srk_launch_wgrad_multi_ridden(wq + nride, 4 - nride, ridden, &rpb, st));
+        else RUN(srk_launch_wgrad_multi_rpb(wq, 4, &rpb, st));
         {
           GemmParams g = {};
           g.A = c.at<bf16_t>(w.dqkv); g.lda = 3 * bw.CA; g.Wt = c.packed + bw.WqkvT; g.M = T; g.N = CP; g.K = 3 * bw.CA;
diff --git a/tpu_superresolution_amd/csrc/wgrad.h b/tpu_superresolution_amd/csrc/wgrad.h
--- a/tpu_superresolution_amd/csrc/wgrad.h
+++ b/tpu_superresolution_amd/csrc/wgrad.h
@@ -32,6 +32,10 @@
   int nsplit;
   int w8;
   RpbJob rpb;
+  float* ppart[4];
+  int pnsplit[4];
+  int ptile0[4];
+  int pw8[4];
   WgradParams p[4];
 };
 
@@ -58,6 +62,7 @@
 
 constexpr int WS_SLAB_VEC = 9216;
 constexpr size_t WS_WORKSPACE_BYTES = (size_t)256 * WS_SLAB_VEC * 16;
+constexpr size_t RIDE_WORKSPACE_BYTES = (size_t)128 * WS_SLAB_VEC * 16;
 float* srk_wgrad_scratch(hipStream_t stream, size_t bytes);
 void srk_wgrad_bind_workspace(void* ptr, size_t bytes, void** prev_ptr, size_t* prev_bytes);
 void srk_wgrad_partials_enable(int on);
@@ -83,4 +88,7 @@
 void srk_wgrad_stream_enable(int on);
 int srk_launch_wgrad_multi(const WgradParams* ps, int nprob, hipStream_t stream);
 int srk_launch_wgrad_multi_rpb(const WgradParams* ps, int nprob, const RpbJob* rpb, hipStream_t stream);
+bool srk_wgrad_ride_applies(const WgradParams* ps, int nprob);
+size_t srk_wgrad_ride_plan(const WgradParams* ridden, int nridden, int riders, WgradMulti* mp);
+int srk_launch_wgrad_multi_ridden(const WgradParams* rest, int nrest, const WgradMulti& ridden, const RpbJob* rpb, hipStream_t stream);
 int srk_launch_rpb_reduce(const float* slab, float* dtable, int nslab, int nH, hipStream_t stream);
diff --git a/tpu_superresolution_amd/csrc/wgrad.hip b/tpu_superresolution_amd/csrc/wgrad.hip
--- a/tpu_superresolution_amd/csrc/wgrad.hip
+++ b/tpu_superresolution_amd/csrc/wgrad.hip
@@ -1,4 +1,4 @@
-#include "wgrad.h"
+#include "wgrad_stream.h"
 
 namespace {
 
@@ -160,140 +160,10 @@
   }
 }
 
-constexpr int WS_LDS_BYTES = 147456;
-
-__device__ __forceinline__ const bf16_t* tr_addr_swz(const bf16_t* tile, int rbase, int c0, int lane) {
-  const int ll = lane & 15;
-  const int row = rbase + (ll >> 2);
-  return tile + row * 192 + (((c0 >> 4) ^ ((row >> 1) & 3)) << 4) + ((ll & 3) << 2);
-}
-
 template <int ROWS, bool NT, bool W8>
 __global__ __launch_bounds__(W8 ? 512 : 256) void wgrad_stream_kernel(const WgradMulti mp) {
-  constexpr int FI = W8 ? 3 : 6;
-  constexpr int STAGE_ELEMS = 2 * ROWS * 192;
-  constexpr int RING = WS_LDS_BYTES / (STAGE_ELEMS * 2);
-  constexpr int NI = ROWS * 24 / 256;
-  constexpr int AHEAD = RING - 1;
-  const int ntiles = mp.tile_begin[mp.nprob];
-  const int logical = xcd_remap(blockIdx.x, gridDim.x);
-  const int bsplit = logical / ntiles, btile = logical - bsplit * ntiles;
-  int pi = 0;
-  while (pi + 1 < mp.nprob && btile >= mp.tile_begin[pi + 1]) ++pi;
-  const WgradParams& p = mp.p[pi];
   extern __shared__ __attribute__((aligned(16))) unsigned char smem[];
-  bf16_t* ring = reinterpret_cast<bf16_t*>(smem);
-  const unsigned ring_base = (unsigned)(size_t)smem;
-
-  const int tid = threadIdx.x, lane = tid & 63;
-  const int wave = __builtin_amdgcn_readfirstlane(tid >> 6);
-  const int r16 = lane & 15, g = lane >> 4;
-  const int wn = wave >> 1, wk = wave & 1;
-  const bool loader = wave < 4;
-  const int ntn = p.N / 192;
-  const int bx = btile - mp.tile_begin[pi];
-  const int tn = bx % ntn, tk = bx / ntn;
-  const int n0 = tn * 192, k0 = tk * 192;
-  const int m_begin = bsplit * mp.m_per;
-  const int m_end = min(p.M, m_begin + mp.m_per);
-  const int nchunk = (m_end - m_begin) / ROWS;
-  if (nchunk <= 0) return;
-
-  int yoff[NI], xoff[NI];
-#pragma unroll
-  for (int i = 0; i < NI; ++i) {
-    const int q = (wave & 3) * (NI * 64) + i * 64 + lane;
-    const int row = q / 24, pos = q - row * 24;
-    const int c = (((pos >> 1) ^ ((row >> 1) & 3)) << 1) | (pos & 1);
-    yoff[i] = row * p.ldy + n0 + c * 8;
-    xoff[i] = row * p.ldx + k0 + c * 8;
-  }
-  auto issue = [&](int ch) {
-    if (!loader) return;
-    const int m0 = m_begin + ch * ROWS;
-    const bf16_t* yb = p.Y + (long long)m0 * p.ldy;
-    const bf16_t* xb = p.X + (long long)m0 * p.ldx;
-    const unsigned dst = ring_base + (unsigned)((ch % RING) * STAGE_ELEMS * 2);
-#pragma unroll
-    for (int i = 0; i < NI; ++i)
-      srk_glds16<NT>(yb + yoff[i], __builtin_amdgcn_readfirstlane(dst + (wave * (NI * 64) + i * 64) * 16));
-#pragma unroll
-    for (int i = 0; i < NI; ++i)
-      srk_glds16<NT>(xb + xoff[i], __builtin_amdgcn_readfirstlane(dst + ROWS * 192 * 2 + (wave * (NI * 64) + i * 64) * 16));
-  };
-
-  f32x4_t acc[FI][6], accb[FI];
-#pragma unroll
-  for (int i = 0; i < FI; ++i) {
-    accb[i] = f32x4_t{0.f, 0.f, 0.f, 0.f};
-#pragma unroll
-    for (int j = 0; j < 6; ++j) acc[i][j] = f32x4_t{0.f, 0.f, 0.f, 0.f};
-  }
-  const bool do_bias = p.db != nullptr && tk == 0 && wk == 0;
-  const bf16x8_t ones = bf16x8_t{0x3F80, 0x3F80, 0x3F80, 0x3F80, 0x3F80, 0x3F80, 0x3F80, 0x3F80};
-
-  for (int c = 0; c < AHEAD && c < nchunk; ++c) issue(c);
-  for (int ch = 0; ch < nchunk; ++ch) {
-    if (ch + AHEAD - 1 < nchunk) {
-      srk_wait_vmcnt<2 * NI * (AHEAD - 1)>();
-    } else {
-      srk_wait_vmcnt<0>();
-    }
-    srk_lds_barrier();
-    if (ch + AHEAD < nchunk) issue(ch + AHEAD);
-    const bf16_t* ys = ring + (ch % RING) * STAGE_ELEMS;
-    const bf16_t* xs = ys + ROWS * 192;
-#pragma unroll
-    for (int ks = 0; ks < ROWS / 32; ++ks) {
-      bf16x8_t yf[FI], xf[6];
-#pragma unroll
-      for (int i = 0; i < FI; ++i) {
-        const int c0 = wn * (16 * FI) + 16 * i;
-        const bf16x4_t lo = lds_tr_read(tr_addr_swz(ys, 32 * ks + 4 * g, c0, lane));
-        const bf16x4_t hi = lds_tr_read(tr_addr_swz(ys, 32 * ks + 16 + 4 * g, c0, lane));
-        yf[i] = bf16x8_t{lo[0], lo[1], lo[2], lo[3], hi[0], hi[1], hi[2], hi[3]};
-      }
-#pragma unroll
-      for (int j = 0; j < 6; ++j) {
-        const int c0 = wk * 96 + 16 * j;
-        const bf16x4_t lo = lds_tr_read(tr_addr_swz(xs, 32 * ks + 4 * g, c0, lane));
-        const bf16x4_t hi = lds_tr_read(tr_addr_swz(xs, 32 * ks + 16 + 4 * g, c0, lane));
-        xf[j] = bf16x8_t{lo[0], lo[1], lo[2], lo[3], hi[0], hi[1], hi[2], hi[3]};
-      }
-#pragma unroll
-      for (int i = 0; i < FI; ++i)
-#pragma unroll
-        for (int j = 0; j < 6; ++j) acc[i][j] = __builtin_amdgcn_mfma_f32_16x16x32_bf16(yf[i], xf[j], acc[i][j], 0, 0, 0);
-      if (do_bias) {
-#pragma unroll
-        for (int i = 0; i < FI; ++i) accb[i] = __builtin_amdgcn_mfma_f32_16x16x32_bf16(yf[i], ones, accb[i], 0, 0, 0);
-      }
-    }
-  }
-
-  if (mp.partial != nullptr) {
-    f32x4_t* slab = reinterpret_cast<f32x4_t*>(mp.partial) + (((size_t)btile * 144 + wave * (FI * 6)) * mp.nsplit + bsplit) * 64 + lane;
-#pragma unroll
-    for (int i = 0; i < FI; ++i)
-#pragma unroll
-      for (int j = 0; j < 6; ++j) slab[(size_t)(i * 6 + j) * mp.nsplit * 64] = acc[i][j];
-  }
-#pragma unroll
-  for (int i = 0; i < FI; ++i) {
-    const int n = n0 + wn * (16 * FI) + 16 * i + 4 * g;
-    if (mp.partial == nullptr) {
-#pragma unroll
-      for (int j = 0; j < 6; ++j) {
-        const int k = k0 + wk * 96 + 16 * j + r16;
-#pragma unroll
-        for (int e = 0; e < 4; ++e) atomicAdd(p.dW + (long long)(n + e) * p.ldw + k, acc[i][j][e]);
-      }
-    }
-    if (do_bias && r16 == 0) {
-#pragma unroll
-      for (int e = 0; e < 4; ++e) atomicAdd(p.db + n + e, accb[i][e]);
-    }
-  }
+  wgrad_stream_role<ROWS, NT, W8>(mp, blockIdx.x, gridDim.x, smem);
 }
 
 __global__ __launch_bounds__(256) void wgrad_reduce_kernel(const WgradMulti mp) {
@@ -311,19 +181,20 @@
   const int ntn = p.N / 192;
   const int bx = btile - mp.tile_begin[pi];
   const int tn = bx % ntn, tk = bx / ntn;
-  const f32x4_t* src = reinterpret_cast<const f32x4_t*>(mp.partial) + ((size_t)btile * 144 + (q >> 6)) * mp.nsplit * 64 + (q & 63);
+  const int nsplit = mp.pnsplit[pi];
+  const f32x4_t* src = reinterpret_cast<const f32x4_t*>(mp.ppart[pi]) + ((size_t)(mp.ptile0[pi] + bx) * 144 + (q >> 6)) * nsplit * 64 + (q & 63);
   f32x4_t sum = f32x4_t{0.f, 0.f, 0.f, 0.f};
   int s = 0;
-  for (; s + 8 <= mp.nsplit; s += 8) {
+  for (; s + 8 <= nsplit; s += 8) {
     f32x4_t v[8];
 #pragma unroll
     for (int u = 0; u < 8; ++u) v[u] = src[(s + u) * 64];
 #pragma unroll
     for (int u = 0; u < 8; ++u) sum += v[u];
   }
-  for (; s < mp.nsplit; ++s) sum += src[s * 64];
+  for (; s < nsplit; ++s) sum += src[s * 64];
   const int lane = q & 63, t = q >> 6;
-  const int fi = mp.w8 ? 3 : 6;
+  const int fi = mp.pw8[pi] ? 3 : 6;
   const int j = t % 6, i = (t / 6) % fi, wave = t / (6 * fi);
   const int wn = wave >> 1, wk = wave & 1, r16 = lane & 15, g = lane >> 4;
   const int n = tn * 192 + wn * (16 * fi) + 16 * i + 4 * g;
@@ -343,6 +214,24 @@
 #endif
 SrkOpt g_wgrad_w8{OPT_WGRAD_W8, SRK_WGRAD_W8_DEFAULT};
 SrkOpt g_wgrad_partials{OPT_WGRAD_PARTIALS, 1};
+
+using StreamFn = void (*)(const WgradMulti);
+StreamFn stream_fn() {
+  static const StreamFn fns[8] = {&wgrad_stream_kernel<64, false, false>, &wgrad_stream_kernel<64, true, false>,
+                                  &wgrad_stream_kernel<32, false, false>, &wgrad_stream_kernel<32, true, false>,
+                                  &wgrad_stream_kernel<64, false, true>,  &wgrad_stream_kernel<64, true, true>,
+                                  &wgrad_stream_kernel<32, false, true>,  &wgrad_stream_kernel<32, true, true>};
+  static SrkPerDevice<bool> sconf_pd; bool& sconf = sconf_pd.here();
+  if (!sconf) {
+    for (StreamFn f : fns)
+      if (hipFuncSetAttribute(reinterpret_cast<const void*>(f), hipFuncAttributeMaxDynamicSharedMemorySize, WS_LDS_BYTES) != hipSuccess) {
+        srk_set_error("wgrad(stream): cannot reserve %d bytes of LDS", WS_LDS_BYTES);
+        return nullptr;
+      }
+    sconf = true;
+  }
+  return fns[(g_wgrad_w8 ? 4 : 0) + (g_wgrad_rows == 32 ? 2 : 0) + (g_wgrad_nt ? 1 : 0)];
+}
 
 template <int TA, int TB, bool CONV>
 int launch(const WgradParams* ps, int nprob, hipStream_t stream) {
@@ -385,24 +274,14 @@
     for (int i = 0; i < nprob; ++i) ok = ok && ps[i].ldy % 8 == 0 && ps[i].ldx % 8 == 0;
     if (ok) {
       constexpr int slds = WS_LDS_BYTES;
-      using KernelFn = void (*)(const WgradMulti);
-      static const KernelFn fns[8] = {&wgrad_stream_kernel<64, false, false>, &wgrad_stream_kernel<64, true, false>,
-                                      &wgrad_stream_kernel<32, false, false>, &wgrad_stream_kernel<32, true, false>,
-                                      &wgrad_stream_kernel<64, false, true>,  &wgrad_stream_kernel<64, true, true>,
-                                      &wgrad_stream_kernel<32, false, true>,  &wgrad_stream_kernel<32, true, true>};
-      static SrkPerDevice<bool> sconf_pd; bool& sconf = sconf_pd.here();
-      if (!sconf) {
-        for (KernelFn f : fns)
-          if (hipFuncSetAttribute(reinterpret_cast<const void*>(f), hipFuncAttributeMaxDynamicSharedMemorySize, slds) != hipSuccess) {
-            srk_set_error("wgrad(stream): cannot reserve %d bytes of LDS", slds);
-            return SRK_E_LAUNCH;
-          }
-        sconf = true;
-      }
-      const KernelFn fn = fns[(g_wgrad_w8 ? 4 : 0) + (g_wgrad_rows == 32 ? 2 : 0) + (g_wgrad_nt ? 1 : 0)];
+      const StreamFn fn = stream_fn();
+      if (!fn) return SRK_E_LAUNCH;
       mp.nsplit = splits;
       mp.w8 = g_wgrad_w8;
       mp.partial = g_wgrad_partials && splits > 1 ? srk_wgrad_scratch(stream, (size_t)tiles * splits * WS_SLAB_VEC * 16) : nullptr;
+      for (int i = 0; i < nprob; ++i) {
+        mp.ppart[i] = mp.partial; mp.pnsplit[i] = splits; mp.ptile0[i] = mp.tile_begin[i]; mp.pw8[i] = mp.w8;
+      }
       srk_probe_pre(fam, stream, flops, bytes);
       hipLaunchKernelGGL(fn, dim3(tiles * splits), dim3(g_wgrad_w8 ? 512 : 256), slds, stream, mp);
       if (mp.partial) {
@@ -515,3 +394,86 @@
   }
   return SRK_OK;
 }
+
+bool srk_wgrad_ride_applies(const WgradParams* ps, int nprob) {
+  if (!g_wgrad_stream || !g_wgrad_partials || nprob < 1 || nprob > 4) return false;
+  for (int i = 0; i < nprob; ++i) {
+    const WgradParams& q = ps[i];
+    if (q.conv || !q.Y || !q.X || !q.dW || q.M <= 0 || q.M != ps[0].M || q.M % 64 != 0 || q.N <= 0 || q.K <= 0 || q.N % 192 != 0 ||
+        q.K % 192 != 0 || q.ldy % 8 != 0 || q.ldx % 8 != 0)
+      return false;
+  }
+  return true;
+}
+
+static int fill_tiles(WgradMulti& mp, const WgradParams* ps, int nprob, int first) {
+  int tiles = mp.tile_begin[first];
+  for (int i = 0; i < nprob; ++i) {
+    mp.p[first + i] = ps[i];
+    mp.tile_begin[first + i] = tiles;
+    tiles += (ps[i].N / 192) * (ps[i].K / 192);
+  }
+  mp.tile_begin[first + nprob] = tiles;
+  return tiles;
+}
+
+size_t srk_wgrad_ride_plan(const WgradParams* ridden, int nridden, int riders, WgradMulti* out) {
+  WgradMulti& mp = *out;
+  mp = WgradMulti{};
+  mp.nprob = nridden;
+  const int tiles = fill_tiles(mp, ridden, nridden, 0);
+  int splits = riders / tiles;
+  if (splits < 1) return 0;
+  int m_per = round_up(cdiv(ridden[0].M, splits), 64);
+  if (m_per < 256) m_per = 256;
+  mp.m_per = m_per;
+  mp.nsplit = cdiv(ridden[0].M, m_per);
+  mp.w8 = 1;
+  return (size_t)tiles * mp.nsplit * WS_SLAB_VEC * 16;
+}
+
+int srk_launch_wgrad_multi_ridden(const WgradParams* rest, int nrest, const WgradMulti& ridden, const RpbJob* rpb, hipStream_t stream) {
+  SRK_REQUIRE(nrest >= 1 && ridden.nprob >= 1 && nrest + ridden.nprob <= 4 && ridden.partial, SRK_E_SHAPE,
+              "wgrad_multi_ridden: %d + %d problems", nrest, ridden.nprob);
+  SRK_REQUIRE(srk_wgrad_ride_applies(rest, nrest) && rest[0].M == ridden.p[0].M, SRK_E_STATE,
+              "wgrad_multi_ridden: the streaming weight-gradient kernel does not cover the remaining problems");
+  const StreamFn fn = stream_fn();
+  if (!fn) return SRK_E_LAUNCH;
+  WgradMulti mp = {};
+  mp.nprob = nrest;
+  const int tiles = fill_tiles(mp, rest, nrest, 0);
+  double flops = 0.0, bytes = 0.0;
+  for (int i = 0; i < nrest; ++i) flops += rest[i].flops, bytes += rest[i].bytes;
+  for (int i = 0; i < ridden.nprob; ++i) flops += ridden.p[i].flops, bytes += ridden.p[i].bytes;
+  const int M = rest[0].M;
+  int splits = 256 / tiles;
+  if (splits < 1) splits = 1;
+  int m_per = round_up(cdiv(M, splits), 64);
+  if (m_per < 256) m_per = 256;
+  mp.m_per = m_per;
+  splits = cdiv(M, m_per);
+  mp.nsplit = splits;
+  mp.w8 = g_wgrad_w8;
+  mp.partial = srk_wgrad_scratch(stream, (size_t)tiles * splits * WS_SLAB_VEC * 16);
+  SRK_REQUIRE(mp.partial, SRK_E_STATE, "wgrad_multi_ridden: no weight-gradient workspace is bound (srk_set_wgrad_workspace)");
+  srk_probe_pre(FAM_WGRAD_LINEAR, stream, flops, bytes);
+  hipLaunchKernelGGL(fn, dim3(tiles * splits), dim3(g_wgrad_w8 ? 512 : 256), WS_LDS_BYTES, stream, mp);
+  WgradMulti rp = ridden;
+  for (int i = 0; i < ridden.nprob; ++i) {
+    rp.ppart[i] = ridden.partial; rp.pnsplit[i] = ridden.nsplit; rp.ptile0[i] = ridden.tile_begin[i]; rp.pw8[i] = ridden.w8;
+  }
+  const int all = fill_tiles(rp, rest, nrest, ridden.nprob);
+  for (int i = 0; i < nrest; ++i) {
+    const int k = ridden.nprob + i;
+    rp.ppart[k] = mp.partial; rp.pnsplit[k] = splits; rp.ptile0[k] = mp.tile_begin[i]; rp.pw8[k] = mp.w8;
+  }
+  rp.nprob = ridden.nprob + nrest;
+  int extra = 0;
+  if (rpb && rpb->slab) {
+    rp.rpb = *rpb;
+    extra = 64 * rpb->nH;
+  }
+  hipLaunchKernelGGL(wgrad_reduce_kernel, dim3(all * 36 + extra), dim3(256), 0, stream, rp);
+  srk_probe_post(FAM_WGRAD_LINEAR, stream);
+  return srk_check_launch("wgrad(stream, ridden)");
+}
diff --git a/tpu_superresolution_amd/csrc/wgrad_stream.h b/tpu_superresolution_amd/csrc/wgrad_stream.h
--- /dev/null
+++ b/tpu_superresolution_amd/csrc/wgrad_stream.h
@@ -0,0 +1,137 @@
+#pragma once
+#include "wgrad.h"
+
+constexpr int WS_LDS_BYTES = 147456;
+
+__device__ __forceinline__ const bf16_t* tr_addr_swz(const bf16_t* tile, int rbase, int c0, int lane) {
+  const int ll = lane & 15;
+  const int row = rbase + (ll >> 2);
+  return tile + row * 192 + (((c0 >> 4) ^ ((row >> 1) & 3)) << 4) + ((ll & 3) << 2);
+}
+
+template <int ROWS, bool NT, bool W8>
+__device__ __forceinline__ void wgrad_stream_role(const WgradMulti& mp, int wg, int nwg, unsigned char* smem) {
+  constexpr int FI = W8 ? 3 : 6;
+  constexpr int STAGE_ELEMS = 2 * ROWS * 192;
+  constexpr int RING = WS_LDS_BYTES / (STAGE_ELEMS * 2);
+  constexpr int NI = ROWS * 24 / 256;
+  constexpr int AHEAD = RING - 1;
+  const int ntiles = mp.tile_begin[mp.nprob];
+  const int logical = xcd_remap(wg, nwg);
+  const int bsplit = logical / ntiles, btile = logical - bsplit * ntiles;
+  int pi = 0;
+  while (pi + 1 < mp.nprob && btile >= mp.tile_begin[pi + 1]) ++pi;
+  const WgradParams& p = mp.p[pi];
+  bf16_t* ring = reinterpret_cast<bf16_t*>(smem);
+  const unsigned ring_base = (unsigned)(size_t)smem;
+
+  const int tid = threadIdx.x, lane = tid & 63;
+  const int wave = __builtin_amdgcn_readfirstlane(tid >> 6);
+  const int r16 = lane & 15, g = lane >> 4;
+  const int wn = wave >> 1, wk = wave & 1;
+  const bool loader = wave < 4;
+  const int ntn = p.N / 192;
+  const int bx = btile - mp.tile_begin[pi];
+  const int tn = bx % ntn, tk = bx / ntn;
+  const int n0 = tn * 192, k0 = tk * 192;
+  const int m_begin = bsplit * mp.m_per;
+  const int m_end = min(p.M, m_begin + mp.m_per);
+  const int nchunk = (m_end - m_begin) / ROWS;
+  if (nchunk <= 0) return;
+
+  int yoff[NI], xoff[NI];
+#pragma unroll
+  for (int i = 0; i < NI; ++i) {
+    const int q = (wave & 3) * (NI * 64) + i * 64 + lane;
+    const int row = q / 24, pos = q - row * 24;
+    const int c = (((pos >> 1) ^ ((row >> 1) & 3)) << 1) | (pos & 1);
+    yoff[i] = row * p.ldy + n0 + c * 8;
+    xoff[i] = row * p.ldx + k0 + c * 8;
+  }
+  auto issue = [&](int ch) {
+    if (!loader) return;
+    const int m0 = m_begin + ch * ROWS;
+    const bf16_t* yb = p.Y + (long long)m0 * p.ldy;
+    const bf16_t* xb = p.X + (long long)m0 * p.ldx;
+    const unsigned dst = ring_base + (unsigned)((ch % RING) * STAGE_ELEMS * 2);
+#pragma unroll
+    for (int i = 0; i < NI; ++i)
+      srk_glds16<NT>(yb + yoff[i], __builtin_amdgcn_readfirstlane(dst + (wave * (NI * 64) + i * 64) * 16));
+#pragma unroll
+    for (int i = 0; i < NI; ++i)
+      srk_glds16<NT>(xb + xoff[i], __builtin_amdgcn_readfirstlane(dst + ROWS * 192 * 2 + (wave * (NI * 64) + i * 64) * 16));
+  };
+
+  f32x4_t acc[FI][6], accb[FI];
+#pragma unroll
+  for (int i = 0; i < FI; ++i) {
+    accb[i] = f32x4_t{0.f, 0.f, 0.f, 0.f};
+#pragma unroll
+    for (int j = 0; j < 6; ++j) acc[i][j] = f32x4_t{0.f, 0.f, 0.f, 0.f};
+  }
+  const bool do_bias = p.db != nullptr && tk == 0 && wk == 0;
+  const bf16x8_t ones = bf16x8_t{0x3F80, 0x3F80, 0x3F80, 0x3F80, 0x3F80, 0x3F80, 0x3F80, 0x3F80};
+
+  for (int c = 0; c < AHEAD && c < nchunk; ++c) issue(c);
+  for (int ch = 0; ch < nchunk; ++ch) {
+    if (ch + AHEAD - 1 < nchunk) {
+      srk_wait_vmcnt<2 * NI * (AHEAD - 1)>();
+    } else {
+      srk_wait_vmcnt<0>();
+    }
+    srk_lds_barrier();
+    if (ch + AHEAD < nchunk) issue(ch + AHEAD);
+    const bf16_t* ys = ring + (ch % RING) * STAGE_ELEMS;
+    const bf16_t* xs = ys + ROWS * 192;
+#pragma unroll
+    for (int ks = 0; ks < ROWS / 32; ++ks) {
+      bf16x8_t yf[FI], xf[6];
+#pragma unroll
+      for (int i = 0; i < FI; ++i) {
+        const int c0 = wn * (16 * FI) + 16 * i;
+        const bf16x4_t lo = lds_tr_read(tr_addr_swz(ys, 32 * ks + 4 * g, c0, lane));
+        const bf16x4_t hi = lds_tr_read(tr_addr_swz(ys, 32 * ks + 16 + 4 * g, c0, lane));
+        yf[i] = bf16x8_t{lo[0], lo[1], lo[2], lo[3], hi[0], hi[1], hi[2], hi[3]};
+      }
+#pragma unroll
+      for (int j = 0; j < 6; ++j) {
+        const int c0 = wk * 96 + 16 * j;
+        const bf16x4_t lo = lds_tr_read(tr_addr_swz(xs, 32 * ks + 4 * g, c0, lane));
+        const bf16x4_t hi = lds_tr_read(tr_addr_swz(xs, 32 * ks + 16 + 4 * g, c0, lane));
+        xf[j] = bf16x8_t{lo[0], lo[1], lo[2], lo[3], hi[0], hi[1], hi[2], hi[3]};
+      }
+#pragma unroll
+      for (int i = 0; i < FI; ++i)
+#pragma unroll
+        for (int j = 0; j < 6; ++j) acc[i][j] = __builtin_amdgcn_mfma_f32_16x16x32_bf16(yf[i], xf[j], acc[i][j], 0, 0, 0);
+      if (do_bias) {
+#pragma unroll
+        for (int i = 0; i < FI; ++i) accb[i] = __builtin_amdgcn_mfma_f32_16x16x32_bf16(yf[i], ones, accb[i], 0, 0, 0);
+      }
+    }
+  }
+
+  if (mp.partial != nullptr) {
+    f32x4_t* slab = reinterpret_cast<f32x4_t*>(mp.partial) + (((size_t)btile * 144 + wave * (FI * 6)) * mp.nsplit + bsplit) * 64 + lane;
+#pragma unroll
+    for (int i = 0; i < FI; ++i)
+#pragma unroll
+      for (int j = 0; j < 6; ++j) slab[(size_t)(i * 6 + j) * mp.nsplit * 64] = acc[i][j];
+  }
+#pragma unroll
+  for (int i = 0; i < FI; ++i) {
+    const int n = n0 + wn * (16 * FI) + 16 * i + 4 * g;
+    if (mp.partial == nullptr) {
+#pragma unroll
+      for (int j = 0; j < 6; ++j) {
+        const int k = k0 + wk * 96 + 16 * j + r16;
+#pragma unroll
+        for (int e = 0; e < 4; ++e) atomicAdd(p.dW + (long long)(n + e) * p.ldw + k, acc[i][j][e]);
+      }
+    }
+    if (do_bias && r16 == 0) {
+#pragma unroll
+      for (int e = 0; e < 4; ++e) atomicAdd(p.db + n + e, accb[i][e]);
+    }
+  }
+}
diff --git a/tpu_superresolution_amd/ops.py b/tpu_superresolution_amd/ops.py
--- a/tpu_superresolution_amd/ops.py
+++ b/tpu_superresolution_amd/ops.py
@@ -248,9 +248,9 @@
         return False
 
 
-def linear_wgrad_multi_bf16(pairs):
+def _wgrad_problems(pairs, out):
     from ._lib import WgradProblem
-    assert 1 <= len(pairs) <= 4
+    assert 1 <= len(pairs) <= 4 and (out is None or len(out) == len(pairs))
     M = pairs[0][0].shape[0]
     dev = pairs[0][0].device
     arr = (WgradProblem * len(pairs))()
@@ -258,14 +258,38 @@
     for i, (y, x) in enumerate(pairs):
         assert y.shape[0] == M and x.shape[0] == M and y.stride(1) == 1 and x.stride(1) == 1
         N, K = y.shape[1], x.shape[1]
-        dw = zeros_f32((N, K), dev)
-        db = zeros_f32((N,), dev)
+        dw, db = out[i] if out is not None else (zeros_f32((N, K), dev), zeros_f32((N,), dev))
+        assert dw.dtype == torch.float32 and db.dtype == torch.float32 and dw.is_contiguous() and tuple(dw.shape) == (N, K) and db.numel() == N
         arr[i].y, arr[i].ldy, arr[i].x, arr[i].ldx = y.data_ptr(), y.stride(0), x.data_ptr(), x.stride(0)
         arr[i].dw, arr[i].db, arr[i].N, arr[i].K = dw.data_ptr(), db.data_ptr(), N, K
         outs.append((dw, db))
+    return arr, outs, M, dev
+
+
+def linear_wgrad_multi_bf16(pairs, out=None):
+    arr, outs, M, dev = _wgrad_problems(pairs, out)
     _bind_wgrad_workspace(dev)
     check(lib().srk_linear_wgrad_multi_bf16(arr, len(pairs), M, _stream()))
     return outs
+
+
+def window_attention_bwd_ride(xn: torch.Tensor, w_qkv: torch.Tensor, b_qkv: Optional[torch.Tensor], scale: float, d_x1: torch.Tensor,
+                              w_proj_t: torch.Tensor, bias_dense: torch.Tensor, H: int, W: int, shift: int, pairs, nride: int, out=None,
+                              phases: int = 3, state=None):
+    B_ = xn.shape[0] // 64
+    nH = bias_dense.shape[0]
+    arr, outs, M, dev = _wgrad_problems(pairs, out)
+    if state is None:
+        state = {"d_qkv": torch.empty((B_ * 64, 3 * nH * 32), dtype=torch.bfloat16, device=dev),
+                 "d_table": torch.zeros((225, nH), dtype=torch.float32, device=dev),
+                 "slab": torch.empty(max(16, lib().srk_window_attention_bwd_ride_scratch(B_, nH)), dtype=torch.uint8, device=dev),
+                 "ride_ws": torch.empty(int(lib().srk_window_attention_bwd_ride_workspace_bytes()), dtype=torch.uint8, device=dev)}
+    _bind_wgrad_workspace(dev)
+    check(lib().srk_window_attention_bwd_ride(_p(xn), xn.stride(0), _p(w_qkv), _p(b_qkv), float(scale), _p(d_x1), d_x1.stride(0),
+                                              _p(w_proj_t), _p(bias_dense), _p(state["d_qkv"]), _p(state["d_table"]), _p(state["slab"]),
+                                              B_, nH, _geom(H, W, shift), arr, len(pairs), nride, M, _p(state["ride_ws"]),
+                                              state["ride_ws"].numel(), phases, _stream()))
+    return state["d_qkv"], state["d_table"], outs, state
 
 
 def conv3x3_bf16(x: torch.Tensor, w: torch.Tensor, bias: Optional[torch.Tensor]) -> torch.Tensor:
```
